# asharakeh/bayes-od-rc

Hardware: AMD Instinct MI355X
Metric: images/sec at N=10 MC samples, 512x512; per-anchor covariance latency (higher is better)
Workload: dtype bf16; 1 GPU; ResNet-50 RetinaNet + covar head, N=10 MC-dropout, 512x512, full BayesOD pipeline (forward+posterior+soft-NMS+cluster-fuse); global_batch=512, mc_samples=10, anchors=49104, parallelism=one GPU (no exchange; N > 1: image-sharded, one RCCL gather/step), visible_gpus=1, gpu_max_hw_queues=4

## Files before the change

### bayes-od-rc_amd/_lib.py

```python
import ctypes as C
import os

import numpy as np


_HERE = os.path.dirname(os.path.abspath(__file__))
LIB_PATH = os.path.join(_HERE, "lib", "libbayesod_hip.so")
if os.environ.get("BOD_LIB_OVERRIDE"):
    LIB_PATH = os.path.abspath(os.environ["BOD_LIB_OVERRIDE"])

BOD_OK, BOD_ERR_INVALID_ARG, BOD_ERR_HIP, BOD_ERR_OOM, BOD_ERR_NOT_READY, BOD_ERR_NO_DEVICE = range(6)
BOD_PARTS_COVARIANCE, BOD_PARTS_CLASS = 1, 2
BOD_VIEW_IDENTITY, BOD_VIEW_HFLIP = 0, 1


class BodConfig(C.Structure):
    _fields_ = [
        ("device", C.c_int32), ("image_h", C.c_int32), ("image_w", C.c_int32), ("batch", C.c_int32),
        ("mc_samples", C.c_int32), ("num_classes", C.c_int32), ("anchors_per_location", C.c_int32),
        ("min_level", C.c_int32), ("max_level", C.c_int32), ("dropout_rate", C.c_float),
        ("use_full_covar", C.c_int32), ("dirichlet_non_informative", C.c_int32),
        ("gaussian_isotropic", C.c_int32), ("isotropic_variance", C.c_float),
        ("ranking_method", C.c_int32), ("nms_max_output_size", C.c_int32),
        ("nms_iou_threshold", C.c_float), ("nms_soft_sigma", C.c_float), ("nms_variant", C.c_int32),
# ... 58 lines not shown
    "bod_get_raw": (C.c_int, [_H, _F, _F, _F]),
    "bod_set_raw": (C.c_int, [_H, _F, _F, _F]),
    "bod_get_pyramid": (C.c_int, [_H, C.c_int32, _F]),
    "bod_posterior": (C.c_int, [_H, C.c_uint64, C.c_uint32]),
    "bod_validation_post": (C.c_int, [_H]),
    "bod_get_num_kept": (C.c_int, [_H, _I]),
    "bod_get_posterior": (C.c_int, [_H, C.c_int32, _F, _F, _F, _F, _F, _I]),
    "bod_set_posterior": (C.c_int, [_H, C.c_int32, C.c_int32, _F, _F, _F, _F]),
    "bod_nms": (C.c_int, [_H]),
    "bod_get_nms": (C.c_int, [_H, C.c_int32, _I, _I]),
    "bod_set_nms": (C.c_int, [_H, C.c_int32, _I, C.c_int32]),
    "bod_get_iou_matrix": (C.c_int, [_H, C.c_int32, _F]),
    "bod_cluster_fuse": (C.c_int, [_H]),
    "bod_set_affinity": (C.c_int, [_H, C.c_int32, _F, C.c_int32, C.c_int32]),
    "bod_get_detections": (C.c_int, [_H, C.c_int32, _I, _F, _F, _F, _F]),
    "bod_get_detections_batch": (C.c_int, [_H, _I, _F, _F, _F, _F]),
    "bod_device_detections": (C.c_int, [_H, C.c_int32, C.POINTER(C.c_void_p)]),
    "bod_device_raw": (C.c_int, [_H, C.POINTER(C.c_void_p), C.c_int32]),
    "bod_infer": (C.c_int, [_H, C.c_void_p, C.c_int32, C.c_uint64, C.c_uint32]),
    "bod_infer_async": (C.c_int, [_H, C.c_void_p, C.c_int32, C.c_uint64, C.c_uint32, _I]),
    "bod_collect": (C.c_int, [_H, C.c_int32, _I, _F, _F, _F, _F]),
    "bod_upload_images": (C.c_int, [_H, _F]),
    "bod_upload_frames_u8": (C.c_int, [_H, C.POINTER(C.c_uint8), C.c_int32, C.c_int32, _F, C.c_int32]),
    "bod_upload_frames_u8_async": (C.c_int, [_H, C.POINTER(C.c_uint8), C.c_int32, C.c_int32, _F, C.c_int32, C.c_int32]),
    "bod_upload_frames_u8_ragged": (C.c_int, [_H, C.POINTER(C.c_uint8), _I, _F, C.c_int32]),
    "bod_upload_frames_u8_ragged_async": (C.c_int, [_H, C.POINTER(C.c_uint8), _I, _F, C.c_int32, C.c_int32]),
    "bod_upload_frames_u8_augmented": (C.c_int, [_H, C.POINTER(C.c_uint8), _I, _F, C.c_int32, C.POINTER(BodAugment)]),
    "bod_upload_frames_u8_augmented_async": (C.c_int, [_H, C.POINTER(C.c_uint8), _I, _F, C.c_int32, C.POINTER(BodAugment), C.c_int32]),
    "bod_augment_boxes": (C.c_int, [C.c_int32, _I, C.c_int32, C.c_int32, C.c_int32, C.POINTER(BodAugment), _I, _F, _F, C.c_int32,
                                    C.c_float, _I, _F, _F]),
    "bod_jpeg_info": (C.c_int, [C.c_char_p, C.c_int64, C.POINTER(BodJpegInfo)]),
    "bod_jpeg_entropy_decode": (C.c_int, [C.c_char_p, C.c_int64, C.POINTER(C.c_int16), C.c_int64, C.POINTER(C.c_uint16)]),
    "bod_jpeg_decode_rgb": (C.c_int, [C.c_int32, C.c_int32, C.POINTER(C.c_char_p), C.POINTER(C.c_int64), C.c_int32,
                                      C.POINTER(C.c_uint8), C.c_int64, _I]),
    "bod_upload_frames_jpeg": (C.c_int, [_H, C.POINTER(C.c_char_p), C.POINTER(C.c_int64), _F, C.c_int32, C.POINTER(BodAugment),
                                         C.c_int32, _I]),
    "bod_upload_frames_jpeg_async": (C.c_int, [_H, C.POINTER(C.c_char_p), C.POINTER(C.c_int64), _F, C.c_int32, C.POINTER(BodAugment),
                                               C.c_int32, _I, C.c_int32]),
    "bod_device_images_buffer": (C.c_void_p, [_H, C.c_int32]),
    "bod_device_images": (C.c_void_p, [_H]),
    "bod_synchronize": (C.c_int, [_H]),
    "bod_stage_conv_wgrad": (C.c_int, [C.c_int32, _F, C.c_int32, C.c_int32, C.c_int32, C.c_int32, _F, C.c_int32, C.c_int32,
                                       C.c_int32, C.c_int32, C.c_int32, C.c_int32, _F, _F]),
    "bod_stage_conv": (C.c_int, [C.c_int32, _F, C.c_int32, C.c_int32, C.c_int32, C.c_int32, _F, _F,
                                 C.c_int32, C.c_int32, C.c_int32, C.c_int32, C.c_int32, C.c_int32, _F,
                                 C.c_float, C.c_uint64, C.c_int32, C.c_uint32, C.c_int32, C.c_int32, _F]),
    "bod_loss_forward": (C.c_int, [C.c_int32, C.c_int32, C.c_int32, C.c_int32, _F, _F, _F, _F, _F, _F,
                                   C.POINTER(C.c_uint8), C.POINTER(C.c_uint8), C.c_int32, C.c_int32, C.c_float,
                                   C.POINTER(C.c_double)]),
    "bod_loss_forward_ex": (C.c_int, [C.c_int32, C.c_int32, C.c_int32, C.c_int32, _F, _F, _F, _F, _F, _F,
                                      C.POINTER(C.c_uint8), C.POINTER(C.c_uint8), C.c_int32, C.c_int32, C.c_float,
                                      C.POINTER(C.c_double), C.POINTER(BodLossOptions)]),
    "bod_set_loss_options": (C.c_int, [_H, C.POINTER(BodLossOptions)]),
    "bod_train_step": (C.c_int, [_H, C.c_void_p, C.c_int32, _F, _F, C.POINTER(C.c_uint8), C.POINTER(C.c_uint8), C.c_uint64, C.c_uint32,
                                 C.c_int32, C.c_float, C.c_float, C.c_float, C.c_float, C.c_float, C.c_int32, C.POINTER(C.c_double)]),
    "bod_train_step_boxes": (C.c_int, [_H, C.c_void_p, C.c_int32, _I, _F, _F, C.c_float, C.c_float, C.c_uint64, C.c_uint32,
                                       C.c_int32, C.c_float, C.c_float, C.c_float, C.c_float, C.c_float, C.c_int32, C.POINTER(C.c_double)]),
    "bod_train_get_targets": (C.c_int, [_H, _F, _F, C.POINTER(C.c_uint8), C.POINTER(C.c_uint8)]),
    "bod_train_gradients": (C.c_int, [_H, C.POINTER(C.c_void_p), C.POINTER(C.c_int64)]),
    "bod_train_apply": (C.c_int, [_H, C.c_float, C.POINTER(C.c_double)]),
    "bod_train_get": (C.c_int, [_H, C.c_char_p, C.c_int32, C.c_int32, _F, C.c_int64]),
    "bod_train_set": (C.c_int, [_H, C.c_char_p, C.c_int32, C.c_int32, _F, C.c_int64]),
    "bod_train_step_count": (C.c_int, [_H, C.POINTER(C.c_int64), C.c_int64]),
    "bod_loss_backward": (C.c_int, [C.c_int32, C.c_int32, C.c_int32, C.c_int32, _F, _F, _F, _F, _F, _F,
                                    C.POINTER(C.c_uint8), C.POINTER(C.c_uint8), C.c_int32, C.c_int32, C.c_float,
                                    C.c_float, C.c_float, C.POINTER(C.c_double), _F, _F, _F]),
    "bod_loss_backward_ex": (C.c_int, [C.c_int32, C.c_int32, C.c_int32, C.c_int32, _F, _F, _F, _F, _F, _F,
                                       C.POINTER(C.c_uint8), C.POINTER(C.c_uint8), C.c_int32, C.c_int32, C.c_float,
                                       C.c_float, C.c_float, C.POINTER(C.c_double), _F, _F, _F, C.POINTER(BodLossOptions)]),
    "bod_anchor_targets": (C.c_int, [C.c_int32, C.c_int32, _F, C.c_int32, _I, _F, _F, C.c_int32, C.c_float, C.c_float, _F, _F,
                                     C.POINTER(C.c_uint8), C.POINTER(C.c_uint8), _I, _F]),
    "bod_validation_losses_boxes": (C.c_int, [_H, _I, _F, _F, C.c_float, C.c_float, C.c_int32, C.c_int32, C.c_float, _D]),
    "bod_get_validation_detections_batch": (C.c_int, [_H, _I, _F, _F]),
    "bod_validate_boxes": (C.c_int, [_H, C.c_void_p, C.c_int32, _I, _F, _F, C.c_float, C.c_float, C.c_int32, C.c_int32, C.c_float, _D,
                                     _I, _F, _F]),
    "bod_pdq_corner_heatmaps": (C.c_int, [C.c_int32, C.c_int32, C.c_int32, C.c_int32, _D, _D, _I, _F]),
    "bod_pdq_frames": (C.c_int, [C.c_int32, C.c_int32, C.c_int32, C.c_int32, _I, _I, _I, _I, _D, _D, _D, _D, _F]),
    "bod_score_pairs": (C.c_int, [C.c_int32, C.c_int64, _D, _D, _D, C.c_int32, C.c_uint64, C.c_uint64, _D, _I]),
    "bod_bench_head_conv": (C.c_int, [_H, C.c_int32, C.c_int32, C.c_int32, C.POINTER(C.c_double), C.POINTER(C.c_double)]),
    "bod_profile_begin": (C.c_int, [_H]),
    "bod_profile_select": (C.c_int, [_H, C.c_int32]),
    "bod_plan_info": (C.c_int, [_H, C.POINTER(C.c_int32)]),
    "bod_plan_info_n": (C.c_int, [_H, C.POINTER(C.c_int32), C.c_int32]),
    "bod_stat_reset": (C.c_int, [_H]),
    "bod_stat_forward": (C.c_int, [_H, C.c_void_p, C.c_int32, C.c_uint64, C.c_uint32, C.c_int32]),
    "bod_stat_merge_from": (C.c_int, [_H, _H]),
    "bod_stat_merge": (C.c_int, [_H, C.POINTER(C.c_void_p), C.c_int32]),
    "bod_stat_device": (C.c_int, [_H, C.POINTER(C.c_void_p), _I]),
    "bod_stat_get": (C.c_int, [_H, _F, _F, _F, _I]),
    "bod_stat_set": (C.c_int, [_H, _F, _F, _F, C.c_int32]),
    "bod_stat_posterior": (C.c_int, [_H, C.c_uint64, C.c_uint32]),
    "bod_stat_forward_view": (C.c_int, [_H, C.c_void_p, C.c_int32, C.c_uint64, C.c_uint32, C.c_int32, C.c_int32]),
    "bod_stat_merge_view": (C.c_int, [_H, C.POINTER(C.c_void_p), C.c_int32, C.c_int32]),
    "bod_record_width": (C.c_int32, [_H]),
    "bod_get_posterior_parts": (C.c_int, [_H, C.c_int32, _F]),
    "bod_set_posterior_parts": (C.c_int, [_H, C.c_int32, C.c_int32, _F]),
    "bod_get_detection_parts": (C.c_int, [_H, C.c_int32, _F]),
    "bod_get_detection_parts_batch": (C.c_int, [_H, _F]),
    "bod_collect_parts": (C.c_int, [_H, C.c_int32, _F]),
    "bod_device_detection_parts": (C.c_int, [_H, C.c_int32, C.POINTER(C.c_void_p)]),
    "bod_get_posterior_class_parts": (C.c_int, [_H, C.c_int32, _F]),
    "bod_get_posterior_mean_probs": (C.c_int, [_H, C.c_int32, _F]),
    "bod_set_posterior_class_parts": (C.c_int, [_H, C.c_int32, C.c_int32, _F, _F]),
    "bod_get_detection_class_parts": (C.c_int, [_H, C.c_int32, _F]),
    "bod_get_detection_class_parts_batch": (C.c_int, [_H, _F]),
    "bod_collect_class_parts": (C.c_int, [_H, C.c_int32, _F]),
    "bod_device_detection_class_parts": (C.c_int, [_H, C.c_int32, C.POINTER(C.c_void_p)]),
    "bod_stat_get_entropy": (C.c_int, [_H, _F]),
    "bod_stat_set_entropy": (C.c_int, [_H, _F]),
    "bod_stat_device_entropy": (C.c_int, [_H, C.POINTER(C.c_void_p)]),
    "bod_stat_merge_entropy": (C.c_int, [_H, C.c_void_p, C.c_int32]),
    "bod_gather_detections": (C.c_int, [_H, C.c_int32, C.c_void_p, C.c_int32, C.c_int32, C.c_int32, C.c_void_p, C.POINTER(C.c_void_p)]),
    "bod_profile_end": (C.c_int, [_H, C.POINTER(C.c_double), C.POINTER(C.c_int64),
                                  C.POINTER(C.c_double), C.POINTER(C.c_double), C.POINTER(C.c_int64)]),
}

_lib = None


def load():
    global _lib
    if _lib is not None:
        return _lib
    if not os.path.exists(LIB_PATH):
        raise RuntimeError(
            "libbayesod_hip.so not found at %s -- build it with `python -c 'import __graft_entry__ as g; "
            "g.build()'` (there is no CPU fallback)" % LIB_PATH)
    lib = C.CDLL(LIB_PATH)
    for name, (res, args) in SIGNATURES.items():
        fn = getattr(lib, name)
        fn.restype = res
        fn.argtypes = args
    _lib = lib
    return lib


def fptr(a):
    return None if a is None else a.ctypes.data_as(_F)


def dptr(a):
    return None if a is None else a.ctypes.data_as(_D)


def iptr(a):
    return None if a is None else a.ctypes.data_as(_I)


def check(lib, handle, status):
    if status == BOD_OK:
        return
    msg = lib.bod_last_error(handle)
    msg = msg.decode() if msg else "status %d" % status
    if status in (BOD_ERR_INVALID_ARG, BOD_ERR_NOT_READY):
        raise ValueError(msg)
    if status == BOD_ERR_OOM:
        raise MemoryError(msg)
    raise RuntimeError(msg)


def as_f32(a):
    return np.ascontiguousarray(a, dtype=np.float32)
```

### bayes-od-rc_amd/csrc/engine.hip

```cpp
#include "../../include/bayesod.h"
#include "kernels.h"
#include "jpeg_entropy.h"

#include <algorithm>
#include <array>
#include <atomic>
#include <cmath>
#include <condition_variable>
#include <deque>
#include <functional>
#include <mutex>
#include <thread>
#include <tuple>
#include <type_traits>
#include <cstdarg>
#include <cstdio>
#include <cstring>
#include <map>
#include <memory>
#include <string>
#include <system_error>
#include <vector>
#include <dlfcn.h>

// ... 186 lines not shown
            }
}

}

struct JpegSlot {
    char* pinned = nullptr; size_t pinned_cap = 0;
    char* dev = nullptr; size_t dev_cap = 0;
    uint8_t* planes = nullptr; size_t planes_cap = 0;
    hipEvent_t copied = nullptr;
    int32_t n = 0;
    size_t stage_bytes = 0, coef_base = 0, plane_bytes = 0;
    int64_t rgb_bytes = 0;
    int32_t idct_wgs_per_frame = 0, color_wgs_per_frame = 0;
    void release() {
        if (pinned) hipHostFree(pinned);
        if (dev) hipFree(dev);
        if (planes) hipFree(planes);
        if (copied) hipEventDestroy(copied);
        *this = JpegSlot();
    }
};

struct bod_context {
    bod_config cfg{};
    std::string err;
    hipStream_t stream = nullptr;
    std::vector<void*> allocs;
    std::map<const void*, size_t> alloc_bytes;
    int64_t device_bytes = 0;
    struct TrainState* train = nullptr;
    struct ValState* val = nullptr;
    int32_t energy_samples = BOD_ENERGY_DEFAULT_SAMPLES;
    uint64_t loss_seed = 0; uint32_t loss_first_image_id = 0; int32_t loss_id_stride = 1;
    int32_t* energy_list = nullptr; float* energy_term = nullptr;

    int sh = 0, sw = 0, ph = 0, pw = 0;
    int ch[6] = {0}, cw[6] = {0};
    int nlev = 0; int lh[8] = {0}, lw[8] = {0};
    int64_t lvl_off[8] = {0};
    int64_t lvl_p0[8] = {0};
    int64_t Ppad = 0; int P = 0, A = 0;

    std::map<std::string, HostTensor> host_w;
    std::map<std::string, PackedConv> packed;
    float* stem_w = nullptr; float* stem_b = nullptr;
    bool weights_ready = false, anchors_ready = false, forward_done = false, posterior_done = false,
         nms_done = false, cluster_done = false;

    float* d_images = nullptr;
    float* splitk_partial = nullptr; size_t splitk_elems = 0;
    uint8_t* d_frames_u8 = nullptr; size_t frames_u8_cap = 0;
    float* d_images_b[2] = {nullptr, nullptr}; uint8_t* d_u8_b[2] = {nullptr, nullptr}; size_t u8_cap_b[2] = {0, 0};
    hipStream_t copy = nullptr;
    hipEvent_t ev_img_ready[2] = {nullptr, nullptr}, ev_img_free[2] = {nullptr, nullptr};
    bool img_ready_pending[2] = {false, false}, img_free_pending[2] = {false, false};
    int cur_img_buf = -1;
    struct RaggedTable { std::vector<char> host; char* dev = nullptr; };
    RaggedTable rag_sync, rag_b[2];
    RaggedTable aug_sync, aug_b[2];
    JpegSlot jpeg_slot[3];
    hipEvent_t ev_tab[2] = {nullptr, nullptr};
    const float* kscale_src[2] = {nullptr, nullptr};
    float* kscale_cur[2] = {nullptr, nullptr}; int kscale_i = 0;
    const float* kscale_now = nullptr;
    char* stem_out = nullptr;
    int es = 2;
    bool split = false;
    char* pyr_hx = nullptr;
    int pyr_fmt = 1;
    int plan_mx = 0;
    int mx = 0;
    Plane pyramid;
    char* head_act[3][2] = {{nullptr}};
    char* head_act_t[3][4] = {{nullptr}};
    float* raw[3] = {nullptr};
    float* agg[3] = {nullptr};
    bool agg_plan = false;
    bool plan_fused_out = false, plan_xreuse = false, plan_xreuse0 = false;
    bool raw_valid = false, agg_valid = false;
    bool plan_sparse = false;
    bool plan_halo = false;
    SparseTailArgs sparse{};
    int plan_tail_rows = 0;
    bool agg_sparse = false;
    float* stat_acc[3] = {nullptr};
    int stat_k = 0;
    hipEvent_t ev_stat = nullptr;
    float* d_mirror = nullptr;
    int mirror_sym = -1, mirror_bad_level = 0;
    bool keep_ready = false;
    uint64_t keep_seed = 0; uint32_t keep_first = 0;
    uint64_t last_seed = 0; uint32_t last_first_image = 0;
    int32_t last_sample_base = 0;
    std::map<std::string, RowEnt*> tables;
    struct XrTable { RowEnt* rows = nullptr; int2* ext = nullptr; int m = 0; };
    std::map<std::string, XrTable> xr_tables;
    std::vector<Op> ops;
    const float* cur_images = nullptr;

    float* d_anchors = nullptr;
    PostBuffers pb{};
    float* nms_scores = nullptr; int32_t* nms_begin = nullptr;
    int32_t* nms_sel_s[2] = {nullptr, nullptr}; int32_t* nms_nsel_s[2] = {nullptr, nullptr};
    float* out_scores_s[2] = {nullptr, nullptr}; float* out_means_s[2] = {nullptr, nullptr};
    float* out_covs_s[2] = {nullptr, nullptr}; float* out_counts_s[2] = {nullptr, nullptr};
    int32_t* nms_sel = nullptr; int32_t* nms_nsel = nullptr;
    float* out_scores = nullptr; float* out_means = nullptr; float* out_covs = nullptr; float* out_counts = nullptr;
    int slot = 0;
    float* parts = nullptr;
    float* out_parts_s[2] = {nullptr, nullptr}; float* out_parts = nullptr;
    std::vector<char> parts_ok, det_parts_ok[2];
    bool parts_staged[2] = {false, false};
    bool class_parts = false;
    float* ent = nullptr; float* stat_ent = nullptr; int stat_ent_k = 0;
    float* cparts = nullptr;
    float* out_cparts_s[2] = {nullptr, nullptr}; float* out_cparts = nullptr;
    std::vector<char> cparts_ok, det_cparts_ok[2];
    bool cparts_staged[2] = {false, false};
    hipStream_t side = nullptr;
    int overlap_mode = 0;
    int ov_front_slots = 0, ov_slots = 0;
    hipStream_t full = nullptr, front = nullptr, back = nullptr;
    hipEvent_t ev_front_done[2] = {nullptr, nullptr}, ev_l0_done[2] = {nullptr, nullptr}, ev_join = nullptr;
    bool l0_pending[2] = {false, false};
    bool ov_dirty = false;
    char* pyr_d[2] = {nullptr, nullptr};
    int fwd_parity = 0, pyr_last = 0;
    int first_head_op = 0;
    bool in_overlap_call = false;
    int n_cu = 256;
    hipEvent_t ev_posterior = nullptr; hipEvent_t ev_done[2] = {nullptr, nullptr};
    int dev_op_lo = 0, dev_op_hi = 1 << 30;
    hipStream_t done_stream[2] = {nullptr, nullptr};
    bool side_pending[2] = {false, false};
    char* host_stage[2] = {nullptr, nullptr};
    float* rec_send = nullptr; float* rec_recv = nullptr; size_t rec_recv_elems = 0;
    hipEvent_t ev_gather = nullptr; hipStream_t gather_stream = nullptr;
    void select_slot(int sidx) {
        slot = sidx;
        nms_sel = nms_sel_s[sidx]; nms_nsel = nms_nsel_s[sidx];
        out_scores = out_scores_s[sidx]; out_means = out_means_s[sidx];
        out_covs = out_covs_s[sidx]; out_counts = out_counts_s[sidx];
        out_parts = out_parts_s[sidx]; out_cparts = out_cparts_s[sidx];
    }
    float* iou_scratch = nullptr; int64_t iou_cap = 0;
    float* affinity = nullptr; int affinity_img = -1;

    bool profiling = false; int prof_which = 0;
    std::vector<std::pair<hipEvent_t, hipEvent_t>> ev_head, ev_post;
    double prof_flops = 0;

    bod_status fail(bod_status s, const char* fmt, ...) {
        char buf[1024];
        va_list ap; va_start(ap, fmt); vsnprintf(buf, sizeof buf, fmt, ap); va_end(ap);
        err = buf;
        return s;
    }
    template <typename T> bod_status dalloc(T** p, size_t n_elems, bool zero = true) {
        void* q = nullptr;
        const size_t bytes = std::max<size_t>(n_elems * sizeof(T), 256);
        hipError_t e = hipMalloc(&q, bytes);
        if (e != hipSuccess) return fail(BOD_ERR_OOM, "hipMalloc(%zu) failed: %s", bytes, hipGetErrorString(e));
        if (zero) {
            e = hipMemsetAsync(q, 0, bytes, stream);
            if (e != hipSuccess) return fail(BOD_ERR_HIP, "hipMemset: %s", hipGetErrorString(e));
        }
        allocs.push_back(q);
        alloc_bytes[q] = bytes;
        device_bytes += (int64_t)bytes;
        *p = reinterpret_cast<T*>(q);
        return BOD_OK;
    }
};

#define HIPCHK(h, expr)                                                                         \
    do {                                                                                        \
        hipError_t _e = (expr);                                                                 \
        if (_e != hipSuccess)                                                                   \
            return (h)->fail(BOD_ERR_HIP, "%s failed: %s (%s:%d)", #expr, hipGetErrorString(_e), \
                             __FILE__, __LINE__);                                               \
    } while (0)
#define BODCHK(expr) do { bod_status _s = (expr); if (_s != BOD_OK) return _s; } while (0)

namespace {

const char* kHeadPrefix[3] = {"pyramid_classification", "pyramid_regression", "pyramid_cov"};
const int kHeadConvs[3] = {4, 3, 4};

// ... 546 lines not shown
    if (xreuse0) BODCHK(make_xr_tiles(t1, &d1x, &dext1, &m1x));

    const bool mc = train_mode || std::max(N, c.mc_ensemble_size) > 1;
    const uint32_t thr = (uint32_t)std::floor((double)c.dropout_rate * 65536.0);
    const float dscale = (float)(1.0 / (1.0 - (double)c.dropout_rate));
    const int nheads = c.has_covar_head ? 3 : 2;
    bool fuse_out = (h->es == 2 || (h->split && xreuse)) && !train_mode;
    if (const char* e = getenv("BOD_FUSE_HEAD_OUTPUT")) fuse_out = fuse_out && atoi(e) != 0;
    {
        ConvArgs probe{};
        probe.M = B * N * h->P; probe.cout_pad = 256; probe.fan_count = 1; probe.flags = CONV_RELU;
        fuse_out = fuse_out && (mx_plan || conv_igemm_uses_full_cout_tile(probe));
    }
    bool agg = xreuse && fuse_out && N >= 2 && 256 / N >= 1 && 320 / N - 2 >= 1 && (c.mc_ensemble_size <= N || c.mc_statistics);
    if (const char* e = getenv("BOD_FUSE_AGGREGATION")) agg = agg && atoi(e) != 0;
    RowEnt* d2a = nullptr; int2* dexta = nullptr; int m2a = 0;
    if (agg) {
        std::vector<RowEnt> tiled;
        std::vector<ExtRow> ext;
        const int rc = xr_tile_rows_aggregated(t2, B, N, h->P, tiled, ext);
        if (rc == 1) return h->fail(BOD_ERR_INVALID_ARG, "aggregated tiling: no pixel fits a tile (N = %d)", N);
        if (rc == 2) return h->fail(BOD_ERR_INVALID_ARG, "aggregated tiling: extended rows out of order");
        m2a = (int)tiled.size();
        BODCHK(h->dalloc(&d2a, tiled.size(), false));
        BODCHK(h->dalloc(&dexta, ext.size(), false));
        HIPCHK(h, hipMemcpyAsync(d2a, tiled.data(), tiled.size() * sizeof(RowEnt), hipMemcpyHostToDevice, h->stream));
        HIPCHK(h, hipMemcpyAsync(dexta, ext.data(), ext.size() * sizeof(int2), hipMemcpyHostToDevice, h->stream));
        HIPCHK(h, hipStreamSynchronize(h->stream));
        const size_t BA = (size_t)B * h->A;
        BODCHK(h->dalloc(&h->agg[0], BA * c.num_classes));
        BODCHK(h->dalloc(&h->agg[1], BA * 16));
        if (c.has_covar_head) BODCHK(h->dalloc(&h->agg[2], BA * 10));
        if (h->class_parts) BODCHK(h->dalloc(&h->ent, BA));
    } else {
        BODCHK(ensure_raw(h));
    }
    if (c.mc_statistics) {
        const size_t BA = (size_t)B * h->A;
        const size_t per[3] = {(size_t)c.num_classes, 16, 10};
        for (int k = 0; k < (c.has_covar_head ? 3 : 2); ++k)
            if (!h->agg[k]) BODCHK(h->dalloc(&h->agg[k], BA * per[k]));
        if (h->class_parts && !h->ent) BODCHK(h->dalloc(&h->ent, BA));
        BODCHK(ensure_stat(h));
    }
    bool sparse = agg && h->es == 2 && !h->split && !mx_plan && !c.pipeline_overlap && !c.mc_statistics &&
                  h->A == h->P * c.anchors_per_location && h->P <= 65536;
    if (const char* e = getenv("BOD_SPARSE_TAIL")) sparse = sparse && atoi(e) != 0;
    bool halo = sparse && !train_mode;
    if (const char* e = getenv("BOD_SPARSE_HALO")) halo = halo && atoi(e) != 0;
    if (sparse) {
        SparseTailArgs& sa = h->sparse;
        const int tables = halo ? 2 : 1;
        sa.B = B; sa.N = N; sa.P = h->P; sa.apl = c.anchors_per_location; sa.Ppad = h->Ppad;
        sa.cap_tiles = B * (h->P / st_min_pixels(N) + 1);
        sa.tail_rows = 192;
        if (const char* e = getenv("BOD_SPARSE_TAIL_ROWS")) { if (atoi(e) == 256) sa.tail_rows = 256; }
        {
            ConvArgs probe{};
            probe.M = sa.cap_tiles * sa.tail_rows; probe.cout_pad = 256; probe.fan_count = 1; probe.flags = CONV_RELU;
            if (!conv_igemm_uses_full_cout_tile(probe)) sa.tail_rows = 256;
        }
        if (st_min_pixels(N, sa.tail_rows) != st_min_pixels(N))
            return h->fail(BOD_ERR_INVALID_ARG, "sparse tail: %d-row tiles change the tile bound at N = %d", sa.tail_rows, N);
        sa.lv.n = 5;
        {
            const PyramidGeometry pg = pyramid_geometry(h->lh, h->lw);
            for (int l = 0; l < 5; ++l) { sa.lv.lw[l] = pg.lw[l]; sa.lv.lh[l] = pg.lh[l]; sa.lv.p0[l] = (int32_t)pg.lvl_p0[l]; }
        }
        RowEnt* pix = nullptr;
        BODCHK(h->dalloc(&pix, (size_t)h->P, false));
        HIPCHK(h, hipMemcpyAsync(pix, t2.data(), (size_t)h->P * sizeof(RowEnt), hipMemcpyHostToDevice, h->stream));
        HIPCHK(h, hipStreamSynchronize(h->stream));
        sa.pix = pix;
        BODCHK(h->dalloc(&sa.rows, (size_t)sa.cap_tiles * sa.tail_rows, false));
        BODCHK(h->dalloc(&sa.ext, (size_t)sa.cap_tiles * XR_EXT_ROWS, false));
        if (halo) {
            BODCHK(h->dalloc(&sa.halo_rows, (size_t)sa.cap_tiles * 256, false));
            BODCHK(h->dalloc(&sa.halo_ext, (size_t)sa.cap_tiles * XR_EXT_ROWS, false));
        }
        BODCHK(h->dalloc(&sa.tile_count, 2));
        BODCHK(h->dalloc(&sa.runs, (size_t)tables * B * h->P, false));
        BODCHK(h->dalloc(&sa.chunks, (size_t)tables * B * h->P, false));
        BODCHK(h->dalloc(&sa.tiles, (size_t)tables * B * h->P, false));
    }
    h->plan_sparse = sparse;
    h->plan_halo = halo;
    h->plan_tail_rows = sparse ? h->sparse.tail_rows : 0;
    Op sparse_op; sparse_op.kind = Op::CONV; sparse_op.is_head3x3 = true; sparse_op.flavour = FLAVOUR_AGG;
    int sparse_groups = 0; PackedConv sparse_pc{};
    Op halo_op = sparse_op;
    int halo_groups = 0; PackedConv halo_pc{};
    h->agg_plan = agg; h->plan_fused_out = fuse_out; h->plan_xreuse = xreuse; h->plan_xreuse0 = xreuse0; h->plan_mx = mx_plan ? mxf : 0;
    int hfmt[3] = {mxf, mxf, mxf};
    if (mxf == 2) { const char* e = getenv("BOD_MX4_BOX_HX"); if (e && atoi(e) != 0) hfmt[1] = 1; }
    if (mxf == 1) { static const bool cls_h4 = [] { const char* e = getenv("BOD_MX_CLS_H4"); return !e || atoi(e) != 0; }(); if (cls_h4) hfmt[0] = 2; }
    const bool mixed = mx_plan && hfmt[0] != hfmt[1];
    const int pyr_fmt = mixed ? 1 : mxf;
    h->pyr_fmt = pyr_fmt;
    for (int layer = 0; layer < 4; ++layer)
    for (int fpass = 0; fpass < 2; ++fpass)
    for (int part = 0; part < 2; ++part)
    for (int flav = (agg && layer >= 2) ? FLAVOUR_RAW : FLAVOUR_BOTH; flav <= ((agg && layer >= 2) ? FLAVOUR_AGG : FLAVOUR_BOTH); ++flav) {
        const bool split_launch = agg && layer >= 2;
        if (fpass == 1 && (!mixed || layer == 0)) continue;
        const int lfmt = !mx_plan ? 0 : layer == 0 ? pyr_fmt : mixed ? (fpass == 0 ? 2 : 1) : mxf;
        if (!split_launch && part == 1) continue;
        if (split_launch && part == 0 && flav == FLAVOUR_AGG) continue;
        const bool both = split_launch && part == 0;
        Op op; op.kind = Op::CONV; op.is_head3x3 = true; op.flavour = both ? FLAVOUR_BOTH : flav;
        int g = 0; PackedConv pc0{};
        double fused_flops = 0;
        const bool both_flav = op.flavour == FLAVOUR_BOTH;
        ConvGroup raw_cg{}; PackedConv raw_pc{}; std::string raw_wname; bool has_raw = false;
        ConvGroup full_cg[3]{}; std::string full_wname[3]; PackedConv full_pc{}; int nfull = 0;
        for (int hd = 0; hd < nheads; ++hd) {
            if (layer >= kHeadConvs[hd]) continue;
            if (split_launch && (part == 1) != (layer == kHeadConvs[hd] - 1)) continue;
            if (mixed && layer > 0 && hfmt[hd] != lfmt) continue;
            PackedConv pc;
            BODCHK(pack_conv(h, std::string(kHeadPrefix[hd]) + "_" + std::to_string(layer), "", 128, &pc, (mx_plan && (layer > 0 || mx_l0)) ? lfmt : 0));
            if (pc.cin != 256 || pc.cout != 256 || pc.taps != 9)
                return h->fail(BOD_ERR_INVALID_ARG, "head conv %s_%d must be 3x3 256->256", kHeadPrefix[hd], layer);
            op.wname[g] = std::string(kHeadPrefix[hd]) + "_" + std::to_string(layer);
            ConvGroup cg{};
            cg.in = layer == 0 ? (mx_l0 ? h->pyr_hx : h->pyramid.d) : (train_mode ? h->head_act_t[hd][layer - 1] : h->head_act[hd][(layer + 1) & 1]);
            cg.w = pc.w; cg.bias = pc.bias;
            cg.out = train_mode ? h->head_act_t[hd][layer] : h->head_act[hd][layer & 1];
            cg.layer_id = hd * 4 + layer;
            cg.out_hx = (mx_plan && layer < kHeadConvs[hd] - 1) ? hfmt[hd] : 0;
            if (fuse_out && layer == kHeadConvs[hd] - 1) {
                PackedConv po;
                BODCHK(pack_conv(h, kHeadPrefix[hd], "", 32, &po));
                if (po.cin != 256 || po.cout != out_ch[hd] || po.taps != 1)
                    return h->fail(BOD_ERR_INVALID_ARG, "head output conv %s must be 1x1 256->%d (got %d->%d)", kHeadPrefix[hd], out_ch[hd], po.cin, po.cout);
                cg.w2 = po.w; cg.bias2 = po.bias; cg.out2 = h->raw[hd]; cg.cout2 = po.cout; cg.out2_cstride = out_ch[hd];
                op.head[g] = hd;
                if (flav == FLAVOUR_AGG) {
                    cg.out2 = nullptr;
                    cg.agg_kind = hd == 0 ? AGG_CLS : hd == 1 ? AGG_BOX : AGG_COV;
                    cg.agg_n = N; cg.agg_P = h->P; cg.agg_C = c.num_classes; cg.agg_out = h->agg[hd]; cg.anchors = h->d_anchors;
                    if (hd == 0 && h->class_parts) { cg.agg_kind = AGG_CLS_ENT; cg.out2 = h->ent; }
                }
                fused_flops += 2.0 * ((double)B * N * h->P) * 256.0 * out_ch[hd];
            }
            if (halo && both_flav && ((layer == 1 && hd == 1) || (layer == 2 && hd == 2))) {
                halo_op.conv.g[halo_groups] = cg;
                halo_op.wname[halo_groups] = op.wname[g];
                if (halo_groups++ == 0) halo_pc = pc;
                halo_op.flops += 2.0 * ((double)B * N * h->P) * 256.0 * 2304.0;
                raw_cg = cg; raw_pc = pc; raw_wname = op.wname[g]; has_raw = true;
                if (nfull == 0) full_pc = pc;
                full_cg[nfull] = cg; full_wname[nfull++] = op.wname[g];
                op.wname[g].clear();
                continue;
            }
            if (sparse && flav == FLAVOUR_AGG && hd != 0) {
                sparse_op.conv.g[sparse_groups] = cg;
                sparse_op.wname[sparse_groups] = op.wname[g];
                sparse_op.head[sparse_groups] = hd;
                if (sparse_groups++ == 0) sparse_pc = pc;
                sparse_op.flops += 2.0 * ((double)B * N * h->P) * 256.0 * 2304.0 + 2.0 * ((double)B * N * h->P) * 256.0 * out_ch[hd];
                fused_flops -= 2.0 * ((double)B * N * h->P) * 256.0 * out_ch[hd];
                op.head[g] = -1; op.wname[g].clear();
                continue;
            }
            op.conv.g[g] = cg;
// ... 60 lines not shown
        ConvArgs a = base_args(sparse_pc, sa.rows, sa.cap_tiles * sa.tail_rows, 256, 256);
        a.tile_rows = sa.tail_rows;
        for (int q = 0; q < sparse_groups; ++q) a.g[q] = sparse_op.conv.g[q];
        a.groups = sparse_groups;
        a.flags = CONV_RELU | (mc ? CONV_DROPOUT : 0);
        a.fan_count = 1; a.fan_stride = (int32_t)h->Ppad;
        a.drop_threshold = thr; a.drop_scale = dscale;
        a.ext = sa.ext; a.xreuse = 2; a.tile_count = sa.tile_count;
        sparse_op.conv = a;
        sparse_op.name = "head_tower_layer_3(sparse)";
        h->ops.push_back(sparse_op);
    }
    for (int hd = 0; hd < nheads && !fuse_out; ++hd) {
        PackedConv pc;
        BODCHK(pack_conv(h, kHeadPrefix[hd], "", 64, &pc));
        if (pc.cin != 256 || pc.cout != out_ch[hd] || pc.taps != 1)
            return h->fail(BOD_ERR_INVALID_ARG, "head output conv %s must be 1x1 256->%d (got %d->%d)", kHeadPrefix[hd], out_ch[hd], pc.cin, pc.cout);
        Op op; op.kind = Op::CONV;
        ConvArgs a = base_args(pc, d3, B * N * h->P, 256, out_ch[hd]);
        a.g[0] = ConvGroup{train_mode ? h->head_act_t[hd][kHeadConvs[hd] - 1] : h->head_act[hd][(kHeadConvs[hd] - 1) & 1], pc.w, pc.bias, h->raw[hd], nullptr, nullptr, 0, 0, nullptr, nullptr, nullptr, 0, 0};
        a.flags = CONV_OUT_F32;
        op.conv = a;
        op.flops = 2.0 * a.M * pc.cout * 256.0;
        op.name = kHeadPrefix[hd]; op.wname[0] = kHeadPrefix[hd];
        h->ops.push_back(op);
    }
    if (h->splitk_elems) {
        BODCHK(h->dalloc(&h->splitk_partial, h->splitk_elems));
        for (Op& o : h->ops) if (o.kind == Op::CONV && o.conv.ksplit > 1) o.conv.partial = h->splitk_partial;
    }
    if (h->split) for (Op& o : h->ops) if (o.kind == Op::CONV) to_split_args(&o.conv);
    h->first_head_op = (int)h->ops.size();
    for (size_t i = 0; i < h->ops.size(); ++i) if (h->ops[i].is_head3x3) { h->first_head_op = (int)i; break; }
    h->pyr_d[0] = h->pyramid.d;
    if (const char* e = getenv("BOD_DUMP_OPS")) if (atoi(e) != 0) {
        fprintf(stderr, "# ops: index name kind flavour M taps cin cout groups fan has_res fused_next flops bytes\n");
        for (size_t i = 0; i < h->ops.size(); ++i) {
            const Op& o = h->ops[i];
            const ConvArgs& a = o.conv;
            double bytes = 0;
            if (o.kind == Op::STEM)
                bytes = (double)B * c.image_h * c.image_w * 3 * 4 + (double)B * h->ph * h->pw * 64 * h->es;
            if (o.kind == Op::CONV) {
                const double es = (a.flags & CONV_OUT_F32) ? 4.0 : (double)h->es;
                for (int g = 0; g < a.groups; ++g) {
                    bytes += (double)a.M * a.cin * h->es;
                    bytes += (double)a.M * std::max(1, a.fan_count) * a.cout_valid * es;
                    if (a.g[g].res) bytes += (double)a.M * a.cout_valid * h->es;
                    if (a.g[g].ch_w3) bytes += (double)a.M * (a.cin == 128 ? 128 : 64) * h->es;
                    bytes += (double)a.taps * a.cin * a.cout_pad * h->es;
                }
            }
            fprintf(stderr, "# op %zu %s %d %d %d %d %d %d %d %d %d %d %.6g %.6g\n", i, o.name.c_str(), (int)o.kind, o.flavour, a.M, a.taps, a.cin,
                    a.cout_valid, a.groups, a.fan_count, o.kind == Op::CONV && a.g[0].res ? 1 : 0, o.kind == Op::CONV && a.g[0].ch_w3 ? 1 : 0, o.flops, bytes);
        }
    }
    if (h->overlap_mode) BODCHK(h->dalloc(&h->pyr_d[1], (size_t)B * h->Ppad * 256 * h->es));
    return BOD_OK;
}

bod_status alloc_post(bod_context* h) {
    const bod_config& c = h->cfg;
    const size_t BA = (size_t)c.batch * h->A;
    const int nblocks = (h->A + 255) / 256;
    PostBuffers& p = h->pb;
    BODCHK(h->dalloc(&p.keep, BA));
    BODCHK(h->dalloc(&p.d_counts, BA * c.num_classes));
    BODCHK(h->dalloc(&p.block_counts, (size_t)c.batch * nblocks));
    BODCHK(h->dalloc(&p.num_kept, (size_t)c.batch));
    BODCHK(h->dalloc(&p.counts, BA * c.num_classes));
    BODCHK(h->dalloc(&p.score, BA * c.num_classes));
    BODCHK(h->dalloc(&p.means, BA * 4));
    BODCHK(h->dalloc(&p.covs, BA * 16));
    BODCHK(h->dalloc(&p.ranking, BA));
    BODCHK(h->dalloc(&p.corners, BA * 4));
    BODCHK(h->dalloc(&p.anchor_index, BA));
    BODCHK(h->dalloc(&h->d_anchors, (size_t)h->A * 4));
    const size_t BApad = (size_t)h->cfg.batch * ((h->A + 511) & ~(size_t)511);
    BODCHK(h->dalloc(&h->nms_scores, BApad));
    BODCHK(h->dalloc(&h->nms_begin, BApad));
    const size_t BK = (size_t)c.batch * c.nms_max_output_size;
    for (int sidx = 0; sidx < 2; ++sidx) {
        BODCHK(h->dalloc(&h->nms_sel_s[sidx], BK));
        BODCHK(h->dalloc(&h->nms_nsel_s[sidx], (size_t)c.batch));
        BODCHK(h->dalloc(&h->out_scores_s[sidx], BK * c.num_classes));
        BODCHK(h->dalloc(&h->out_means_s[sidx], BK * 4));
        BODCHK(h->dalloc(&h->out_covs_s[sidx], BK * 16));
        BODCHK(h->dalloc(&h->out_counts_s[sidx], BK * c.num_classes));
        if (c.covariance_parts & BOD_PARTS_COVARIANCE) BODCHK(h->dalloc(&h->out_parts_s[sidx], BK * 48));
        if (h->class_parts) BODCHK(h->dalloc(&h->out_cparts_s[sidx], BK * 4));
        const size_t stage_bytes = ((size_t)c.batch + BK * (2 * (size_t)c.num_classes + 20 + ((c.covariance_parts & BOD_PARTS_COVARIANCE) ? 48 : 0) +
                                                            (h->class_parts ? 4 : 0))) * 4;
        if (hipHostMalloc(reinterpret_cast<void**>(&h->host_stage[sidx]), stage_bytes, hipHostMallocDefault) != hipSuccess)
            return h->fail(BOD_ERR_OOM, "pinned host staging buffer (%zu bytes)", stage_bytes);
    }
    if (c.covariance_parts & BOD_PARTS_COVARIANCE) {
        BODCHK(h->dalloc(&h->parts, BA * BOD_PARTS_TRI));
        h->parts_ok.assign((size_t)c.batch, 0);
        for (int sidx = 0; sidx < 2; ++sidx) h->det_parts_ok[sidx].assign((size_t)c.batch, 0);
    }
    if (h->class_parts) {
        BODCHK(h->dalloc(&h->cparts, BA * (3 + (size_t)c.num_classes)));
        h->cparts_ok.assign((size_t)c.batch, 0);
        for (int sidx = 0; sidx < 2; ++sidx) h->det_cparts_ok[sidx].assign((size_t)c.batch, 0);
    }
    h->select_slot(0);
    BODCHK(h->dalloc(&h->d_images, (size_t)c.batch * c.image_h * c.image_w * 3));
    h->d_images_b[0] = h->d_images;
    return BOD_OK;
}

PostCfg post_cfg(bod_context* h, uint64_t seed, uint32_t first_image) {
    const bod_config& c = h->cfg;
    PostCfg p{};
    p.B = c.batch; p.N = c.mc_samples; p.A = h->A; p.C = c.num_classes; p.draws = c.num_categorical_draws;
    p.use_full_covar = c.use_full_covar; p.has_covar = c.has_covar_head; p.dirichlet = c.dirichlet_non_informative;
    p.gaussian_iso = c.gaussian_isotropic; p.ranking_method = c.ranking_method; p.iso_var = c.isotropic_variance;
    p.kitti_sh = c.kitti_scale_h; p.kitti_sw = c.kitti_scale_w;
    p.kitti_frame = c.kitti_scale_h > 0.f ? h->kscale_now : nullptr;
    p.seed_lo = (uint32_t)seed; p.seed_hi = (uint32_t)(seed >> 32); p.image_base = first_image;
    return p;
}

struct Markers {
    bool on = false;
    int (*push)(const char*) = nullptr;
    int (*pop)() = nullptr;
    Markers() {
        const char* e = getenv("BOD_ROCTX");
        if (!e || !atoi(e)) return;
        void* lib = dlopen("librocprofiler-sdk-roctx.so", RTLD_NOW | RTLD_GLOBAL);
        if (!lib) lib = dlopen("libroctx64.so", RTLD_NOW | RTLD_GLOBAL);
        if (!lib) { fprintf(stderr, "bayesod: BOD_ROCTX=1 but no roctx library could be opened (%s)\n", dlerror()); return; }
        push = reinterpret_cast<int (*)(const char*)>(dlsym(lib, "roctxRangePushA"));
        pop = reinterpret_cast<int (*)()>(dlsym(lib, "roctxRangePop"));
        on = push && pop;
    }
};
static Markers& markers() { static Markers m; return m; }
struct MarkerRange {
    bool on;
    explicit MarkerRange(const char* name) : on(markers().on) { if (on) markers().push(name); }
    ~MarkerRange() { if (on) markers().pop(); }
    MarkerRange(const MarkerRange&) = delete;
    MarkerRange& operator=(const MarkerRange&) = delete;
};
static std::string op_stage(const std::string& name) {
    if (name.rfind("conv1", 0) == 0 || name.rfind("pool1", 0) == 0) return "bod:stem";
    if (name.rfind("res", 0) == 0 && name.size() > 3) return "bod:" + name.substr(0, 4);
    if (name.rfind("head_tower_layer_", 0) == 0) return "bod:" + name.substr(0, name.find('(') == std::string::npos ? name.size() : name.find('('));
    if (name.rfind("pyramid_", 0) == 0) return "bod:head_outputs";
    return "bod:fpn";
}

bod_status mark_images_consumed(bod_context* h, hipStream_t st = nullptr) {
    if (h->cur_img_buf >= 0 && h->copy) {
        HIPCHK(h, hipEventRecord(h->ev_img_free[h->cur_img_buf], st ? st : h->stream));
        h->img_free_pending[h->cur_img_buf] = true;
    }
    return BOD_OK;
}

bod_status join_overlap(bod_context* h) {
    if (!h->ov_dirty) return BOD_OK;
    HIPCHK(h, hipStreamSynchronize(h->front));
    HIPCHK(h, hipStreamSynchronize(h->back));
    h->ov_dirty = false;
    return BOD_OK;
}

bod_status run_forward(bod_context* h, const float* dev_images, uint64_t seed, uint32_t first_image, int flavour = FLAVOUR_RAW,
                       bool only_flavoured = false, bool overlapped = false) {
    const bod_config& c = h->cfg;
    if (flavour == FLAVOUR_RAW && !only_flavoured) BODCHK(ensure_raw(h));
    const bool ov = overlapped && h->overlap_mode != 0 && !only_flavoured;
    hipStream_t fs = ov ? h->front : h->stream;
    int par = 0;
    if (ov) {
        par = h->fwd_parity; h->fwd_parity ^= 1;
        if (h->l0_pending[par]) { HIPCHK(h, hipStreamWaitEvent(fs, h->ev_l0_done[par], 0)); h->l0_pending[par] = false; }
    }
    if (!only_flavoured) { h->pyr_last = par; h->keep_ready = false; }
    const int cus_front = h->n_cu;
    const int cus_back = h->n_cu;
    static const int trace_call = getenv("BOD_TRACE_OPS") ? atoi(getenv("BOD_TRACE_OPS")) : 0;
    static int call_no = 0;
    const bool trace = trace_call > 0 && ++call_no == trace_call && !ov;
    std::vector<hipEvent_t> tev;
    if (trace) {
        tev.resize(h->ops.size() + 1);
        for (hipEvent_t& e : tev) HIPCHK(h, hipEventCreate(&e));
        HIPCHK(h, hipEventRecord(tev[0], h->stream));
    }
    size_t op_i = 0;
    bool stem_pool_fused = false;
    std::string cur_stage;
    struct StageCloser { std::string& s; ~StageCloser() { if (!s.empty()) markers().pop(); } } stage_closer{cur_stage};
    for (Op& op : h->ops) {
        if (trace && op_i > 0) HIPCHK(h, hipEventRecord(tev[op_i], h->stream));
        const bool is_front = (int)op_i < h->first_head_op;
        const bool first_back = (int)op_i == h->first_head_op;
        hipStream_t st = is_front ? fs : h->stream;
        ++op_i;
        if ((op.flavour != FLAVOUR_BOTH && op.flavour != flavour) || (only_flavoured && op.flavour == FLAVOUR_BOTH)) continue;
        if (op.raw_use == (only_flavoured ? Op::RAW_FORWARD : Op::RAW_RERUN)) continue;
        if ((int)op_i - 1 < h->dev_op_lo || (int)op_i - 1 >= h->dev_op_hi) continue;
        if (ov && first_back) {
            HIPCHK(h, hipEventRecord(h->ev_front_done[par], fs));
            HIPCHK(h, hipStreamWaitEvent(h->stream, h->ev_front_done[par], 0));
        }
        if (markers().on) {
            std::string st = op_stage(op.name);
            if (st != cur_stage) {
                if (!cur_stage.empty()) markers().pop();
                markers().push(st.c_str());
                cur_stage.swap(st);
            }
        }
        switch (op.kind) {
            case Op::STEM: {
                const Op* pool = op_i < h->ops.size() && h->ops[op_i].kind == Op::POOL ? &h->ops[op_i] : nullptr;
                static const bool split_fused = [] { const char* e = getenv("BOD_STEM_SPLIT_FUSED"); return !e || atoi(e) != 0; }();
                stem_pool_fused = pool && !h->train && (h->split ? split_fused : h->es == 2) && !trace &&
                                  stem_pool_fused_applies(dev_images, c.batch, c.image_w, h->sw, is_front ? cus_front : cus_back);
                if (stem_pool_fused)
                    HIPCHK(h, launch_stem_pool_fused(dev_images, h->stem_w, h->stem_b, pool->conv.g[0].out, h->split ? 1 : 0, c.batch, c.image_h,
                                                     c.image_w, h->sh, h->sw, h->ph, h->pw, h->pw + 2, (h->ph + 2) * (h->pw + 2), st));
                else
                HIPCHK(h, launch_stem_conv(dev_images, h->stem_w, h->stem_b, h->stem_out, h->es == 4, c.batch, c.image_h,
                                           c.image_w, h->sh, h->sw, st));
                if (!h->train) BODCHK(mark_images_consumed(h, st));
                break;
            }
            case Op::KEEP: {
                for (int sidx = 0; sidx < 2; ++sidx)
                    if (h->side_pending[sidx]) HIPCHK(h, hipStreamWaitEvent(st, h->ev_done[sidx], 0));
                PostCfg pc = post_cfg(h, seed, first_image);
                pc.aggregated = 1;
                PostBuffers pb = h->pb;
                pb.agg_cls = h->agg[0];
                HIPCHK(h, launch_posterior_keep(pc, pb, st));
                SparseTailArgs sa = h->sparse;
                sa.keep = h->pb.keep;
                HIPCHK(h, launch_sparse_tail_rows(sa, st));
                static const bool sparse_stats = [] { const char* e = getenv("BOD_SPARSE_STATS"); return e && atoi(e) != 0; }();
                if (sparse_stats) {
                    HIPCHK(h, hipStreamSynchronize(st));
                    int32_t cnt[2] = {0, 0};
                    HIPCHK(h, hipMemcpy(cnt, sa.tile_count, sizeof cnt, hipMemcpyDeviceToHost));
                    const int R = sa.tail_rows;
                    long valid = 0, full = 0;
                    if (cnt[0] > 0 && cnt[0] <= sa.cap_tiles) {
                        std::vector<int32_t> off((size_t)cnt[0] * R);
                        HIPCHK(h, hipMemcpy2D(off.data(), sizeof(int32_t), &sa.rows[0].out_off, sizeof(RowEnt), sizeof(int32_t), off.size(), hipMemcpyDeviceToHost));
                        for (int t = 0; t < cnt[0]; ++t) {
                            int v = 0;
                            for (int r = 0; r < R; ++r) v += off[(size_t)t * R + r] >= 0 ? 1 : 0;
                            valid += v;
                            full += v == R ? 1 : 0;
                        }
                    }
                    const long dense = ((long)sa.B * sa.N * sa.P + 255) / 256;
                    std::fprintf(stderr, "BOD_SPARSE_STATS: tail %d tiles of %d rows, %.1f valid rows per tile (%ld rows = %.3f of the dense launch's), %ld tiles with all %d rows valid; "
                                 "halo %d tiles of 256 rows; dense plain tiles %ld; capacity %d tiles\n", (int)cnt[0], R,
                                 cnt[0] > 0 ? (double)valid / cnt[0] : 0.0, valid, (double)valid / ((double)sa.B * sa.N * sa.P), full, R, (int)cnt[1], dense, (int)sa.cap_tiles);
                }
                h->keep_ready = true; h->keep_seed = seed; h->keep_first = first_image;
                break;
            }
            case Op::POOL:
                if (stem_pool_fused) break;
                HIPCHK(h, launch_stem_pool(h->stem_out, op.conv.g[0].out, h->split ? 2 : (h->es == 4 ? 1 : 0), c.batch,
                                           h->sh, h->sw, h->ph, h->pw, h->pw + 2, (h->ph + 2) * (h->pw + 2), st));
                break;
            case Op::CONV: {
                if (op.hx_pyramid) HIPCHK(h, launch_pairs_to_hx(h->pyramid.d, h->pyr_hx, (long)c.batch * h->Ppad, 256, st, h->pyr_fmt));
                op.conv.seed_lo = (uint32_t)seed; op.conv.seed_hi = (uint32_t)(seed >> 32);
                op.conv.image_base = first_image;
                op.conv.sample_base = (uint32_t)c.mc_sample_base;
                op.conv.dyn_rng = train_dyn_rng(h);
                const bool is_tower = op.conv.xreuse != 0 && op.conv.fan_count <= 1;
                const bool timed = h->profiling && op.is_head3x3 && (h->prof_which == 0 || (h->prof_which == 1) == is_tower);
                hipEvent_t e0 = nullptr, e1 = nullptr;
                if (timed) {
                    HIPCHK(h, hipEventCreate(&e0)); HIPCHK(h, hipEventCreate(&e1));
                    HIPCHK(h, hipEventRecord(e0, st));
                }
                op.conv.n_cu = is_front ? cus_front : cus_back;
                if (par != 0) {
                    ConvArgs a = op.conv;
                    for (int g = 0; g < a.groups; ++g) {
                        if (a.g[g].in == h->pyr_d[0]) a.g[g].in = h->pyr_d[1];
                        if (a.g[g].out == h->pyr_d[0]) a.g[g].out = h->pyr_d[1];
                    }
                    HIPCHK(h, (h->es == 4 && !h->split) ? launch_conv_igemm_f32(a, st) : launch_conv_igemm(a, st));
                } else
                HIPCHK(h, (h->es == 4 && !h->split) ? launch_conv_igemm_f32(op.conv, st) : launch_conv_igemm(op.conv, st));
                if (timed) {
                    HIPCHK(h, hipEventRecord(e1, st));
                    h->ev_head.emplace_back(e0, e1);
                    h->prof_flops += op.flops;
                }
                if (ov && first_back) {
                    HIPCHK(h, hipEventRecord(h->ev_l0_done[par], h->stream));
                    h->l0_pending[par] = true;
                }
                break;
            }
        }
    }
    if (trace) {
        HIPCHK(h, hipEventRecord(tev[h->ops.size()], h->stream));
        HIPCHK(h, hipStreamSynchronize(h->stream));
        fprintf(stderr, "# op trace: name kind M taps cin cout_pad groups fan ms TFLOP/s\n");
        for (size_t i = 0; i < h->ops.size(); ++i) {
            float ms = 0.f;
            HIPCHK(h, hipEventElapsedTime(&ms, tev[i], tev[i + 1]));
            const Op& o = h->ops[i];
            fprintf(stderr, "%-28s %d %8d %2d %5d %5d %d %2d %9.4f %8.1f\n", o.name.c_str(), (int)o.kind, o.conv.M, o.conv.taps,
                    o.conv.cin, o.conv.cout_pad, o.conv.groups, o.conv.fan_count, ms, o.flops / (ms * 1e-3) / 1e12);
        }
        for (hipEvent_t& e : tev) hipEventDestroy(e);
    }
    h->forward_done = true; h->posterior_done = h->nms_done = h->cluster_done = false; h->affinity_img = -1;
    h->last_seed = seed; h->last_first_image = first_image;
    if (!only_flavoured) h->last_sample_base = c.mc_sample_base;
    if (flavour == FLAVOUR_AGG) { h->agg_valid = true; h->raw_valid = false; h->agg_sparse = h->plan_sparse; }
// ... 1375 lines not shown
        if (!h->det_cparts_ok[h->slot][img]) return h->fail(BOD_ERR_NOT_READY, "bod_get_detection_class_parts_batch: image %d was fused without its posterior's class parts (bod_set_posterior_class_parts)", img);
    const size_t B = (size_t)h->cfg.batch, K = (size_t)h->cfg.nms_max_output_size;
    std::vector<int32_t> num(B);
    HIPCHK(h, hipMemcpyAsync(num.data(), h->nms_nsel, B * 4, hipMemcpyDeviceToHost, h->stream));
    BODCHK(d2h(h, rows, h->out_cparts, B * K * 4));
    HIPCHK(h, hipStreamSynchronize(h->stream));
    for (size_t b = 0; rows && b < B; ++b)
        for (size_t k = (size_t)std::max(num[b], 0); k < K; ++k)
            for (int q = 0; q < 4; ++q) rows[(b * K + k) * 4 + q] = 0.f;
    return BOD_OK;
}

bod_status bod_device_detection_class_parts(bod_handle h, int32_t sidx, void** p) {
    BODCHK(class_parts_handle(h, "bod_device_detection_class_parts"));
    if (!p || sidx < 0 || sidx > 1) return h->fail(BOD_ERR_INVALID_ARG, "bod_device_detection_class_parts: slot %d / NULL", sidx);
    *p = h->out_cparts_s[sidx];
    return BOD_OK;
}

bod_status bod_device_raw(bod_handle h, void** p, int32_t mark_ready) {
    if (!h || !p) return BOD_ERR_INVALID_ARG;
    BODCHK(join_overlap(h));
    HIPCHK(h, hipSetDevice(h->cfg.device));
    if (mark_ready) BODCHK(ensure_raw(h)); else BODCHK(materialise_raw(h));
    p[0] = h->raw[0]; p[1] = h->raw[1]; p[2] = h->cfg.has_covar_head ? h->raw[2] : nullptr;
    if (mark_ready) { h->kscale_now = nullptr; h->forward_done = true; h->posterior_done = h->nms_done = h->cluster_done = false; h->affinity_img = -1; h->raw_valid = true; h->agg_valid = false; }
    return BOD_OK;
}

bod_status bod_device_detections(bod_handle h, int32_t sidx, void** p) {
    if (!h || !p || sidx < 0 || sidx > 1) return BOD_ERR_INVALID_ARG;
    p[0] = h->nms_nsel_s[sidx]; p[1] = h->out_scores_s[sidx]; p[2] = h->out_means_s[sidx];
    p[3] = h->out_covs_s[sidx]; p[4] = h->out_counts_s[sidx];
    return BOD_OK;
}

bod_status bod_infer(bod_handle h, const float* images, int32_t on_device, uint64_t seed, uint32_t first_image_id) {
    MarkerRange mr_api("bod:infer");
    if (!h) return BOD_ERR_INVALID_ARG;
    BODCHK(join_overlap(h));
    if (!h->weights_ready) return h->fail(BOD_ERR_NOT_READY, "weights not finalized");
    if (h->cfg.mc_samples < 2) return h->fail(BOD_ERR_INVALID_ARG, "bayes_od needs mc_samples >= 2 (sample covariance divides by N-1)");
    HIPCHK(h, hipSetDevice(h->cfg.device));
    const float* dev = nullptr;
    BODCHK(stage_images(h, images, on_device, &dev));
    h->cur_images = dev;
    BODCHK(run_forward(h, dev, seed, first_image_id, infer_flavour(h)));
    BODCHK(run_posterior(h, seed, first_image_id));
    BODCHK(run_nms(h, h->stream));
    return run_cluster(h, h->stream);
}

bod_status bod_infer_async(bod_handle h, const float* images, int32_t on_device, uint64_t seed, uint32_t first_image_id, int32_t* slot_out) {
    MarkerRange mr_api("bod:infer_async");
    if (!h || !slot_out) return BOD_ERR_INVALID_ARG;
    if (!h->weights_ready) return h->fail(BOD_ERR_NOT_READY, "weights not finalized");
    if (h->cfg.mc_samples < 2) return h->fail(BOD_ERR_INVALID_ARG, "bayes_od needs mc_samples >= 2 (sample covariance divides by N-1)");
    HIPCHK(h, hipSetDevice(h->cfg.device));
    const int sidx = h->slot ^ 1;
    if (h->side_pending[sidx])
        return h->fail(BOD_ERR_NOT_READY, "slot %d still holds uncollected detections: call bod_collect first", sidx);
    const bool ov = h->overlap_mode != 0;
    struct MainStream { bod_context* h; ~MainStream() { h->stream = h->full; h->in_overlap_call = false; } } restore_main{h};
    if (ov) {
        HIPCHK(h, hipEventRecord(h->ev_join, h->full));
        HIPCHK(h, hipStreamWaitEvent(h->front, h->ev_join, 0));
        HIPCHK(h, hipStreamWaitEvent(h->back, h->ev_join, 0));
        h->stream = h->back; h->in_overlap_call = true; h->ov_dirty = true;
    }
    const float* dev = nullptr;
    BODCHK(stage_images(h, images, on_device, &dev, ov ? h->front : h->stream));
    h->cur_images = dev;
    BODCHK(run_forward(h, dev, seed, first_image_id, infer_flavour(h), false, ov));
    BODCHK(run_posterior(h, seed, first_image_id));
    HIPCHK(h, hipEventRecord(h->ev_posterior, h->stream));
    h->select_slot(sidx);
    static const bool side_on = [] { const char* e = getenv("BOD_SIDE_STREAM"); return e && atoi(e) != 0; }();
    hipStream_t sd = side_on ? h->side : h->stream;
    if (side_on) HIPCHK(h, hipStreamWaitEvent(h->side, h->ev_posterior, 0));
    BODCHK(run_nms(h, sd));
    BODCHK(run_cluster(h, sd));
    {
        const size_t B = (size_t)h->cfg.batch, BK = B * h->cfg.nms_max_output_size, C = h->cfg.num_classes;
        char* hs = h->host_stage[sidx];
        HIPCHK(h, hipMemcpyAsync(hs, h->nms_nsel_s[sidx], B * 4, hipMemcpyDeviceToHost, sd)); hs += B * 4;
        HIPCHK(h, hipMemcpyAsync(hs, h->out_scores_s[sidx], BK * C * 4, hipMemcpyDeviceToHost, sd)); hs += BK * C * 4;
        HIPCHK(h, hipMemcpyAsync(hs, h->out_means_s[sidx], BK * 16, hipMemcpyDeviceToHost, sd)); hs += BK * 16;
        HIPCHK(h, hipMemcpyAsync(hs, h->out_covs_s[sidx], BK * 64, hipMemcpyDeviceToHost, sd)); hs += BK * 64;
        HIPCHK(h, hipMemcpyAsync(hs, h->out_counts_s[sidx], BK * C * 4, hipMemcpyDeviceToHost, sd)); hs += BK * C * 4;
        if (h->parts) { HIPCHK(h, hipMemcpyAsync(hs, h->out_parts_s[sidx], BK * 48 * 4, hipMemcpyDeviceToHost, sd)); h->parts_staged[sidx] = true; hs += BK * 48 * 4; }
        if (h->cparts) { HIPCHK(h, hipMemcpyAsync(hs, h->out_cparts_s[sidx], BK * 4 * 4, hipMemcpyDeviceToHost, sd)); h->cparts_staged[sidx] = true; }
    }
    HIPCHK(h, hipEventRecord(h->ev_done[sidx], sd));
    h->done_stream[sidx] = sd;
    h->side_pending[sidx] = true;
    *slot_out = sidx;
    return BOD_OK;
}

bod_status bod_collect(bod_handle h, int32_t sidx, int32_t* num, float* scores, float* means, float* covs, float* counts) {
    MarkerRange mr_api("bod:collect");
    if (!h) return BOD_ERR_INVALID_ARG;
    if (sidx < 0 || sidx > 1 || !h->side_pending[sidx]) return h->fail(BOD_ERR_NOT_READY, "slot %d has no pending batch", sidx);
    const size_t B = (size_t)h->cfg.batch, BK = B * h->cfg.nms_max_output_size, C = h->cfg.num_classes;
    HIPCHK(h, hipEventSynchronize(h->ev_done[sidx]));
    const char* hs = h->host_stage[sidx];
    if (num) std::memcpy(num, hs, B * 4);
    hs += B * 4;
    if (scores) std::memcpy(scores, hs, BK * C * 4);
    hs += BK * C * 4;
    if (means) std::memcpy(means, hs, BK * 16);
    hs += BK * 16;
    if (covs) std::memcpy(covs, hs, BK * 64);
    hs += BK * 64;
    if (counts) std::memcpy(counts, hs, BK * C * 4);
    h->side_pending[sidx] = false;
    return BOD_OK;
}

bod_status bod_collect_parts(bod_handle h, int32_t sidx, float* parts) {
    BODCHK(parts_handle(h, "bod_collect_parts"));
    if (sidx < 0 || sidx > 1 || !h->parts_staged[sidx]) return h->fail(BOD_ERR_NOT_READY, "bod_collect_parts: slot %d holds no batch of bod_infer_async", sidx);
    const size_t B = (size_t)h->cfg.batch, BK = B * h->cfg.nms_max_output_size, C = h->cfg.num_classes;
    HIPCHK(h, hipEventSynchronize(h->ev_done[sidx]));
    if (parts) std::memcpy(parts, h->host_stage[sidx] + (B + BK * (2 * C + 20)) * 4, BK * 48 * 4);
    return BOD_OK;
}

bod_status bod_collect_class_parts(bod_handle h, int32_t sidx, float* rows) {
    BODCHK(class_parts_handle(h, "bod_collect_class_parts"));
    if (sidx < 0 || sidx > 1 || !h->cparts_staged[sidx]) return h->fail(BOD_ERR_NOT_READY, "bod_collect_class_parts: slot %d holds no batch of bod_infer_async", sidx);
    const size_t B = (size_t)h->cfg.batch, K = (size_t)h->cfg.nms_max_output_size, BK = B * K, C = h->cfg.num_classes;
    HIPCHK(h, hipEventSynchronize(h->ev_done[sidx]));
    if (!rows) return BOD_OK;
    std::memcpy(rows, h->host_stage[sidx] + (B + BK * (2 * C + 20 + (h->parts ? 48 : 0))) * 4, BK * 4 * 4);
    const int32_t* num = reinterpret_cast<const int32_t*>(h->host_stage[sidx]);
    for (size_t b = 0; b < B; ++b)
        for (size_t k = (size_t)std::max(num[b], 0); k < K; ++k)
            for (int q = 0; q < 4; ++q) rows[(b * K + k) * 4 + q] = 0.f;
    return BOD_OK;
}

bod_status bod_stage_conv(int32_t device, const float* x, int32_t B, int32_t H, int32_t W, int32_t Cin,
                          const float* w, const float* bias, int32_t KH, int32_t KW, int32_t Cout,
                          int32_t stride, int32_t same_padding, int32_t relu, const float* residual,
                          float dropout_rate, uint64_t seed, int32_t layer_id, uint32_t image_id,
                          int32_t round_output_bf16, int32_t precision, float* out) {
    bod_context ctx;
    bod_context* h = &ctx;
    const int mxfmt = precision == BOD_PRECISION_F16MX ? 1 : precision == BOD_PRECISION_F16MX4 ? 2 : 0;
    const bool mxp = mxfmt != 0;
    const int mx_mode = mxp ? round_output_bf16 : 0;
    const bool f32 = precision == BOD_PRECISION_FP32, x3 = precision == BOD_PRECISION_BF16X3 || mxp;
    if (mxp) round_output_bf16 = 1;
    h->es = (f32 || x3) ? 4 : 2;
    h->split = x3; h->mx = mxfmt;
    auto done = [&](bod_status s) {
        if (s != BOD_OK) g_create_error = h->err;
        if (h->stream) hipStreamSynchronize(h->stream);
        for (void* p : h->allocs) hipFree(p);
        if (h->stream) hipStreamDestroy(h->stream);
        h->allocs.clear(); h->stream = nullptr;
        return s;
    };
    if (!x || !w || !out || B < 1 || H < 1 || W < 1 || KH < 1 || KW < 1 || stride < 1 || stride > 2)
        return done(h->fail(BOD_ERR_INVALID_ARG, "bod_stage_conv: bad argument"));
    if (precision != BOD_PRECISION_BF16 && !f32 && !x3) return done(h->fail(BOD_ERR_INVALID_ARG, "bod_stage_conv: bad precision"));
    if (mxp && (KH != 3 || KW != 3 || stride != 1 || !same_padding || Cin != 256 || Cout != 256 || residual || mx_mode < 0 || mx_mode > 2))
        return done(h->fail(BOD_ERR_INVALID_ARG, "bod_stage_conv: BOD_PRECISION_F16MX / F16MX4 run a head-tower layer (3x3, stride 1, SAME, 256 -> 256, no residual), round_output_bf16 in 0..2"));
    if (f32 && round_output_bf16) return done(h->fail(BOD_ERR_INVALID_ARG, "bod_stage_conv: round_output_bf16 is meaningless in fp32 precision"));
    if (Cin % 64 != 0 || ((round_output_bf16 || (dropout_rate > 0.f && !f32)) && Cout % 4 != 0))
        return done(h->fail(BOD_ERR_INVALID_ARG, "bod_stage_conv: Cin must be a multiple of 64 (and Cout of 4 for bf16 output); got %d, %d", Cin, Cout));
    if (KH > 3 || KW > 3) return done(h->fail(BOD_ERR_INVALID_ARG, "bod_stage_conv: kernel larger than 3x3 needs a wider zero border"));
    int ndev = 0;
    if (hipGetDeviceCount(&ndev) != hipSuccess || device < 0 || device >= ndev)
        return done(h->fail(BOD_ERR_NO_DEVICE, "no HIP device %d: libbayesod_hip has no CPU fallback", device));
    if (hipSetDevice(device) != hipSuccess || hipStreamCreateWithFlags(&h->stream, hipStreamNonBlocking) != hipSuccess)
        return done(h->fail(BOD_ERR_HIP, "cannot set up device %d", device));
    h->cfg.batch = B;
    int OH, OW, oy = 1, ox = 1;
    if (same_padding) {
        OH = (H + stride - 1) / stride; OW = (W + stride - 1) / stride;
        oy = 1 - same_pad_before(H, KH, stride); ox = 1 - same_pad_before(W, KW, stride);
    } else {
        OH = (H - KH) / stride + 1; OW = (W - KW) / stride + 1;
    }
    if (OH < 1 || OW < 1) return done(h->fail(BOD_ERR_INVALID_ARG, "bod_stage_conv: empty output"));
    auto run = [&]() -> bod_status {
        Plane in, res;
        BODCHK(new_plane(h, &in, B, H, W, Cin));
        auto put_split = [](std::vector<uint16_t>& dst, size_t pix_slot0, int c, float v) {
            const uint16_t hi = f2bf(v);
            const size_t slot = pix_slot0 + (size_t)(c >> 5) * 64 + (c & 31);
            dst[slot] = hi; dst[slot + 32] = f2bf(v - bf2f(hi));
        };
        std::vector<uint16_t> hx(f32 ? 0 : (size_t)B * in.bstride * Cin * (x3 ? 2 : 1), 0);
        std::vector<float> hx32(f32 ? (size_t)B * in.bstride * Cin : 0, 0.f);
        const bool hx_in = mxp && mx_mode != 2;
        for (int b = 0; b < B && hx_in; ++b)
            for (int y = 0; y < H; ++y)
                for (int xx = 0; xx < W; ++xx) {
                    const size_t pix = (size_t)b * in.bstride + (size_t)(y + 1) * in.pitch + (xx + 1);
                    (mxfmt == 2 ? pack_h4_row : pack_hx_row)(x + (((size_t)b * H + y) * W + xx) * Cin, Cin, reinterpret_cast<uint8_t*>(hx.data()) + pix * Cin * 4, false);
                }
        for (int b = 0; b < B && !hx_in; ++b)
            for (int y = 0; y < H; ++y)
                for (int xx = 0; xx < W; ++xx)
                    for (int c = 0; c < Cin; ++c) {
                        const size_t pix = (size_t)b * in.bstride + (size_t)(y + 1) * in.pitch + (xx + 1);
                        const size_t di = pix * Cin + c;
                        const float v = x[(((size_t)b * H + y) * W + xx) * Cin + c];
                        if (f32) hx32[di] = v; else if (x3) put_split(hx, pix * 2 * Cin, c, v); else hx[di] = f2bf(v);
                    }
        HIPCHK(h, hipMemcpyAsync(in.d, f32 ? (const void*)hx32.data() : (const void*)hx.data(),
                                 (size_t)B * in.bstride * Cin * h->es, hipMemcpyHostToDevice, h->stream));
        HIPCHK(h, hipStreamSynchronize(h->stream));
        if (residual) {
            BODCHK(new_plane(h, &res, B, OH, OW, Cout));
// ... 578 lines not shown
    static const bool side_on = [] { const char* e = getenv("BOD_SIDE_STREAM"); return e && atoi(e) != 0; }();
    hipStream_t st = (slot >= 0 && slot <= 1 && !side_on && h->done_stream[slot]) ? h->done_stream[slot] : h->side;
    if (slot < 0) {
        if (!h->cluster_done) return h->fail(BOD_ERR_NOT_READY, "bod_gather_detections: bod_cluster_fuse has not run");
        BODCHK(join_overlap(h));
        sidx = h->slot;
        st = h->stream;
    } else if (slot > 1 || !h->side_pending[slot]) {
        return h->fail(BOD_ERR_NOT_READY, "bod_gather_detections: slot %d has no pending batch", slot);
    }
    for (int img = 0; h->parts && img < B; ++img)
        if (!h->det_parts_ok[sidx][img]) return h->fail(BOD_ERR_NOT_READY, "bod_gather_detections: image %d was fused without its posterior's parts (bod_set_posterior_parts)", img);
    for (int img = 0; h->cparts && img < B; ++img)
        if (!h->det_cparts_ok[sidx][img]) return h->fail(BOD_ERR_NOT_READY, "bod_gather_detections: image %d was fused without its posterior's class parts (bod_set_posterior_class_parts)", img);
    if (!h->rec_send && hipMalloc(reinterpret_cast<void**>(&h->rec_send), block * 4) != hipSuccess)
        return h->fail(BOD_ERR_OOM, "bod_gather_detections: %zu bytes", block * 4);
    if (h->ev_gather && h->gather_stream && h->gather_stream != st) HIPCHK(h, hipStreamWaitEvent(st, h->ev_gather, 0));
    if (slot >= 0) HIPCHK(h, hipStreamWaitEvent(st, h->ev_done[slot], 0));
    if (h->cparts)
        HIPCHK(h, launch_pack_records_class(h->nms_nsel_s[sidx], h->out_scores_s[sidx], h->out_means_s[sidx], h->out_covs_s[sidx],
                                            h->out_counts_s[sidx], h->out_parts_s[sidx], h->out_cparts_s[sidx], h->rec_send, B, K, C, st));
    else if (h->parts)
        HIPCHK(h, launch_pack_records_parts(h->nms_nsel_s[sidx], h->out_scores_s[sidx], h->out_means_s[sidx], h->out_covs_s[sidx],
                                            h->out_counts_s[sidx], h->out_parts_s[sidx], h->rec_send, B, K, C, st));
    else
        HIPCHK(h, launch_pack_records(h->nms_nsel_s[sidx], h->out_scores_s[sidx], h->out_means_s[sidx], h->out_covs_s[sidx],
                                      h->out_counts_s[sidx], h->rec_send, B, K, C, st));
    float* recv = nullptr;
    if (rank == root) {
        if (world == 1 && !nccl_comm) recv = h->rec_send;
        else {
            if (h->rec_recv_elems < block * world) {
                if (h->rec_recv && h->rec_recv != h->rec_send) hipFree(h->rec_recv);
                h->rec_recv = nullptr; h->rec_recv_elems = 0;
                if (hipMalloc(reinterpret_cast<void**>(&h->rec_recv), block * world * 4) != hipSuccess)
                    return h->fail(BOD_ERR_OOM, "bod_gather_detections: %zu bytes", block * world * 4);
                h->rec_recv_elems = block * world;
            }
            recv = h->rec_recv;
        }
    }
    if (nccl_comm) {
        if (!rccl().load()) return h->fail(BOD_ERR_NOT_READY, "bod_gather_detections: librccl.so (ncclGather) could not be opened");
        const int rc = rccl().gather(h->rec_send, recv, block,  7, root, nccl_comm, st);
        if (rc != 0) return h->fail(BOD_ERR_HIP, "ncclGather: %s", rccl().errstr ? rccl().errstr(rc) : "error");
    }
    if (!h->ev_gather) HIPCHK(h, hipEventCreateWithFlags(&h->ev_gather, hipEventDisableTiming));
    if (rank == root && gathered_host) {
        HIPCHK(h, hipMemcpyAsync(gathered_host, recv, block * world * 4, hipMemcpyDeviceToHost, st));
        HIPCHK(h, hipEventRecord(h->ev_gather, st)); h->gather_stream = st;
        HIPCHK(h, hipEventSynchronize(h->ev_gather));
    } else {
        HIPCHK(h, hipEventRecord(h->ev_gather, st)); h->gather_stream = st;
    }
    if (!(rank == root && gathered_host) && slot >= 0) {
        HIPCHK(h, hipEventRecord(h->ev_done[slot], st));
    }
    if (gathered_device) *gathered_device = recv;
    return BOD_OK;
}

bod_status bod_plan_info(bod_handle h, int32_t* info8) {
    if (!h || !info8) return BOD_ERR_INVALID_ARG;
    if (!h->weights_ready) return h->fail(BOD_ERR_NOT_READY, "bod_plan_info: the plan is built by bod_finalize_weights");
    for (int i = 0; i < 8; ++i) info8[i] = 0;
    info8[0] = h->agg_plan; info8[1] = h->plan_fused_out; info8[2] = h->plan_xreuse; info8[3] = h->plan_xreuse0;
    info8[4] = (int32_t)h->ops.size();
    for (const Op& o : h->ops) if (o.kind == Op::CONV && !o.is_head3x3 && o.conv.xreuse) ++info8[5];
    info8[6] = h->plan_mx;
    info8[7] = h->plan_sparse;
    return BOD_OK;
}

bod_status bod_plan_info_n(bod_handle h, int32_t* info, int32_t n) {
    if (!h || !info || n < 0) return BOD_ERR_INVALID_ARG;
    int32_t all[10];
    BODCHK(bod_plan_info(h, all));
    all[8] = h->plan_halo;
    all[9] = h->plan_tail_rows;
    for (int i = 0; i < n && i < 10; ++i) info[i] = all[i];
    return BOD_OK;
}

static bod_status stat_handle(bod_handle h, const char* who) {
    if (!h->cfg.mc_statistics) return h->fail(BOD_ERR_INVALID_ARG, "%s: the handle was not created with mc_statistics = 1", who);
    BODCHK(join_overlap(h));
    HIPCHK(h, hipSetDevice(h->cfg.device));
    return ensure_stat(h);
}

static bod_status stat_view_ready(bod_handle h, const char* who, int32_t view) {
    if (view != BOD_VIEW_IDENTITY && view != BOD_VIEW_HFLIP)
        return h->fail(BOD_ERR_INVALID_ARG, "%s: view must be BOD_VIEW_IDENTITY (0) or BOD_VIEW_HFLIP (1), got %d", who, view);
    if (view == BOD_VIEW_IDENTITY) return BOD_OK;
    if (!h->anchors_ready) return h->fail(BOD_ERR_NOT_READY, "%s: bod_set_anchors has not been called (a mirrored view maps every anchor to its partner)", who);
    const bod_config& c = h->cfg;
    const int K = c.anchors_per_location;
    if (h->mirror_sym < 0) {
        std::vector<float> an((size_t)h->A * 4);
        HIPCHK(h, hipMemcpyAsync(an.data(), h->d_anchors, an.size() * 4, hipMemcpyDeviceToHost, h->stream));
        HIPCHK(h, hipStreamSynchronize(h->stream));
        const float fw = (float)c.image_w;
        int bad = -1;
        for (int l = 0; l < h->nlev && bad < 0; ++l) {
            const size_t off = (size_t)h->lvl_p0[l] * K;
            const int W = h->lw[l];
            for (int y = 0; y < h->lh[l] && bad < 0; ++y)
                for (int x = 0; x < W && bad < 0; ++x)
                    for (int k = 0; k < K; ++k) {
                        const float* s = &an[(off + ((size_t)y * W + x) * K + k) * 4];
                        const float* p = &an[(off + ((size_t)y * W + (W - 1 - x)) * K + k) * 4];
                        const float want[4] = {s[0], fw - s[1], s[2], s[3]};
                        if (memcmp(p, want, 16) != 0) { bad = l; break; }
                    }
        }
        h->mirror_sym = bad < 0; h->mirror_bad_level = bad < 0 ? 0 : c.min_level + bad;
    }
    if (!h->mirror_sym)
        return h->fail(BOD_ERR_INVALID_ARG, "%s: the anchors of pyramid level %d are not mirror-symmetric about image_w / 2 for a %dx%d image "
                       "(BOD_VIEW_HFLIP needs image_w to be a multiple of 2^max_level = %d)", who, h->mirror_bad_level, c.image_h, c.image_w,
                       1 << c.max_level);
    return BOD_OK;
}

static bod_status stat_fold(bod_handle h, const char* who, const float* cls, const float* box, const float* cov, int kb, int32_t view = BOD_VIEW_IDENTITY) {
    if (kb < 1) return h->fail(BOD_ERR_INVALID_ARG, "%s: a record of %d samples", who, kb);
    if (h->stat_k > (1 << 24) - kb) return h->fail(BOD_ERR_INVALID_ARG, "%s: more than 2^24 samples in one accumulator", who);
    if (h->class_parts && h->stat_ent_k != h->stat_k)
        return h->fail(BOD_ERR_NOT_READY, "%s: ent_sum holds %d of the record's %d samples (bod_stat_merge_entropy / bod_stat_set_entropy has not followed)", who, h->stat_ent_k, h->stat_k);
    StatMergeArgs m{};
    m.BA = (int64_t)h->cfg.batch * h->A; m.C = h->cfg.num_classes; m.ka = h->stat_k; m.kb = kb;
    m.acc_cls = h->stat_acc[0]; m.acc_box = h->stat_acc[1]; m.acc_cov = h->stat_acc[2];
    m.src_cls = cls; m.src_box = box; m.src_cov = h->cfg.has_covar_head ? cov : nullptr;
    if (!cls || !box || (h->cfg.has_covar_head && !cov)) return h->fail(BOD_ERR_INVALID_ARG, "%s: NULL statistics array", who);
    if (cls == m.acc_cls || box == m.acc_box) return h->fail(BOD_ERR_INVALID_ARG, "%s: the source is the accumulator itself", who);
    if (((uintptr_t)cls | (uintptr_t)box | (uintptr_t)m.src_cov) & 15u) return h->fail(BOD_ERR_INVALID_ARG, "%s: statistics arrays must be 16-byte aligned", who);
    if (view == BOD_VIEW_HFLIP) {
        StatMirrorArgs mm{};
        mm.m = m; mm.A = h->A; mm.K = h->cfg.anchors_per_location; mm.nlev = h->nlev;
        for (int l = 0; l < h->nlev; ++l) { mm.lvl_off[l] = (int32_t)h->lvl_p0[l] * mm.K; mm.lvl_w[l] = h->lw[l]; }
        mm.lvl_off[h->nlev] = h->A;
        mm.u_flip = (float)(h->cfg.image_w - 1);
        HIPCHK(h, launch_stat_merge_mirror(mm, h->stream));
    } else {
        HIPCHK(h, launch_stat_merge(m, h->stream));
    }
    h->stat_k += kb;
    return BOD_OK;
}

static bod_status stat_fold_entropy(bod_handle h, const char* who, const float* ent, int32_t view = BOD_VIEW_IDENTITY) {
    if (!ent) return h->fail(BOD_ERR_INVALID_ARG, "%s: ent_sum is NULL", who);
    if (ent == h->stat_ent) return h->fail(BOD_ERR_INVALID_ARG, "%s: the source is the accumulator itself", who);
    if ((uintptr_t)ent & 15u) return h->fail(BOD_ERR_INVALID_ARG, "%s: ent_sum must be 16-byte aligned", who);
    if (h->stat_ent_k >= h->stat_k) return h->fail(BOD_ERR_NOT_READY, "%s: ent_sum already holds the record's %d samples (fold the three arrays first)", who, h->stat_k);
    const int64_t BA = (int64_t)h->cfg.batch * h->A;
    if (view == BOD_VIEW_HFLIP) {
        StatMirrorArgs mm{};
        mm.A = h->A; mm.K = h->cfg.anchors_per_location; mm.nlev = h->nlev;
        for (int l = 0; l < h->nlev; ++l) { mm.lvl_off[l] = (int32_t)h->lvl_p0[l] * mm.K; mm.lvl_w[l] = h->lw[l]; }
        mm.lvl_off[h->nlev] = h->A;
        HIPCHK(h, launch_stat_merge_entropy(h->stat_ent, ent, BA, h->stat_ent_k == 0, &mm, h->stream));
    } else {
        HIPCHK(h, launch_stat_merge_entropy(h->stat_ent, ent, BA, h->stat_ent_k == 0, nullptr, h->stream));
    }
    h->stat_ent_k = h->stat_k;
// ... 228 lines not shown
```

### bayes-od-rc_amd/csrc/kernels.h

```cpp
#pragma once
#include <hip/hip_runtime.h>
#include <stdint.h>
#include "plan_tables.h"
#include "sparse_tables.h"


struct ConvGroup {
    const void* in;
    const void* w;
    const float* bias;
    void* out;
    const void* res;
    void* out_relu;
    int32_t in_coff;
    int32_t layer_id;
    const void* w2;
    const float* bias2;
    float* out2;
    int32_t cout2;
    int32_t out2_cstride;
    int32_t agg_kind;
    int32_t agg_n;
    int32_t agg_P;
    int32_t agg_C;
// ... 41 lines not shown
    int32_t n_cu;
    int32_t stagger_ticks;
    int32_t fan_chunk;
    int32_t mx;
    int32_t mx_loader;
    int32_t tile_rows;
    const int32_t* tile_count;
};

struct PerDeviceOnce {
    bool done[64] = {false};
    bool* slot() { int d = 0; if (hipGetDevice(&d) != hipSuccess || d < 0 || d >= 64) d = 0; return &done[d]; }
};

int device_cu_count();
inline int launch_cus(const ConvArgs& a) { return a.n_cu > 0 ? a.n_cu : device_cu_count(); }
hipError_t launch_conv_igemm(const ConvArgs& a, hipStream_t s);
bool conv_igemm_uses_full_cout_tile(const ConvArgs& a);
bool conv_igemm_uses_big_tile(const ConvArgs& a);
void conv_igemm_phase_cycles(unsigned long long* out16, bool reset);
hipError_t launch_conv_igemm_f32(const ConvArgs& a, hipStream_t s);
hipError_t launch_pairs_to_hx(const void* in, void* out, long npix, int C, hipStream_t s, int fmt = 1);

hipError_t launch_stem_conv(const float* img, const float* w, const float* bias, void* out, int out_f32,
                            int B, int H, int W, int oh, int ow, hipStream_t s);
bool stem_pool_fused_applies(const float* img, int B, int W, int ow, int n_cu);
hipError_t launch_stem_pool_fused(const float* img, const float* w, const float* bias, void* pooled, int split, int B, int H, int W, int oh,
                                  int ow, int ph, int pw, int pool_pitch, int pool_plane, hipStream_t s);
hipError_t launch_stem_pool(const void* in, void* out, int mode, int B, int ih, int iw, int oh, int ow,
                            int out_pitch, int out_plane, hipStream_t s);

struct PostCfg {
    int32_t B, N, A, C, draws;
    int32_t use_full_covar, has_covar, dirichlet, gaussian_iso, ranking_method;
    float iso_var;
    float kitti_sh, kitti_sw;
    const float* kitti_frame;
    uint32_t seed_lo, seed_hi, image_base;
    int32_t aggregated;
};

struct PostBuffers {
    const float* cls;
    const float* box;
    const float* cov;
    const float* anchors;
    const float* agg_cls;
    const float* agg_box;
    const float* agg_cov;
    uint8_t* keep;
    float* d_counts;
    int32_t* block_counts;
    int32_t* num_kept;
    float* counts;
    float* score;
    float* means;
    float* covs;
    float* ranking;
    float* corners;
    int32_t* anchor_index;
};

hipError_t launch_posterior(const PostCfg& c, const PostBuffers& b, hipStream_t s);
hipError_t launch_posterior_keep(const PostCfg& c, const PostBuffers& b, hipStream_t s);
hipError_t launch_posterior_fuse(const PostCfg& c, const PostBuffers& b, hipStream_t s);

struct SparseTailArgs {
    const uint8_t* keep;
    const RowEnt* pix;
    RowEnt* rows;
    int2* ext;
    RowEnt* halo_rows;
    int2* halo_ext;
    int32_t* tile_count;
    int2* runs;
    StQuad* chunks;
    StQuad* tiles;
    int32_t B, N, P, apl, cap_tiles;
    int32_t tail_rows;
    int64_t Ppad;
    SparseLevels lv;
};
hipError_t launch_sparse_tail_rows(const SparseTailArgs& a, hipStream_t s);
hipError_t launch_joint_entropy_rank(const PostCfg& c, const PostBuffers& b, hipStream_t s);
hipError_t launch_validation_post(const PostCfg& c, const PostBuffers& b, hipStream_t s);

struct NmsArgs {
    int32_t B, A;
    const int32_t* num_kept;
    const float* corners;
    const float* ranking;
    float* work_scores;
    int32_t* work_begin;
    int32_t* selected;
    int32_t* num_selected;
    int32_t max_out;
    float iou_thr, sigma;
    int32_t variant;
};
hipError_t launch_nms(const NmsArgs& a, hipStream_t s);

struct ValGatherArgs {
    int32_t B, A, C, max_out;
    const int32_t* num_kept;
    const int32_t* selected;
    const int32_t* num_selected;
    const float* score;
    const float* corners;
    float* out_scores;
    float* out_corners;
    int32_t* out_num;
};
hipError_t launch_validation_gather(const ValGatherArgs& a, hipStream_t s);

struct ClusterArgs {
    int32_t B, A, C, max_out;
    const int32_t* num_kept;
    const int32_t* selected;
    const int32_t* num_selected;
    const float* corners;
    const float* counts;
    const float* means;
    const float* covs;
    float thr;
    const float* affinity; int32_t affinity_img;
    float* out_scores; float* out_means; float* out_covs; float* out_counts;
};
hipError_t launch_cluster_fuse(const ClusterArgs& a, hipStream_t s);
hipError_t launch_iou_matrix(const float* corners, int M, float* out, hipStream_t s);
#define BOD_PARTS_TRI 30
hipError_t launch_posterior_parts(const PostCfg& c, const PostBuffers& b, float* parts, hipStream_t s);
hipError_t launch_cluster_parts(const ClusterArgs& a, const float* parts, float* out_parts, hipStream_t s);
#define BOD_LOG_SDEN(x) (__builtin_amdgcn_logf(x) * 0.693147180559945f)
hipError_t launch_posterior_class_parts(const PostCfg& c, const PostBuffers& b, const float* ent_sum, float* cparts, hipStream_t s);
hipError_t launch_cluster_class_parts(const ClusterArgs& a, const float* cparts, float* out_cparts, hipStream_t s);
hipError_t launch_pack_records(const int32_t* num, const float* scores, const float* means, const float* covs, const float* counts,
                               float* rec, int B, int K, int C, hipStream_t s);
hipError_t launch_pack_records_parts(const int32_t* num, const float* scores, const float* means, const float* covs, const float* counts,
                                     const float* parts, float* rec, int B, int K, int C, hipStream_t s);
hipError_t launch_pack_records_class(const int32_t* num, const float* scores, const float* means, const float* covs, const float* counts,
                                     const float* parts, const float* cparts, float* rec, int B, int K, int C, hipStream_t s);

struct PreprocArgs {
    const uint8_t* src;
    float* dst;
    int32_t B, sh, sw;
    int32_t rh, rw;
    int32_t H, W;
    int32_t crop_y, crop_x, pad_y, pad_x, vis_h, vis_w;
    int32_t resize;
    float scale_y, scale_x;
    float mean[3];
};
hipError_t launch_preprocess(const PreprocArgs& a, hipStream_t s);

struct PreprocFrame {
    int64_t offset;
    int32_t sh, sw, rh, rw;
    float scale_y, scale_x;
    int32_t crop_y, crop_x, pad_y, pad_x, vis_h, vis_w;
};
struct PreprocRaggedArgs {
    const uint8_t* src;
    float* dst;
    const PreprocFrame* frames;
    int32_t B, H, W;
// ... 192 lines not shown
```

### bayes-od-rc_amd/csrc/post_kernels.hip

```cpp
#include "kernels.h"
#include "philox.h"
#include <algorithm>
#include <math.h>

#define POST_BLOCK 256
#define MAXC 16

struct Mat4 { float m[4][4]; };

__device__ __forceinline__ Mat4 inv_spd4_once(const Mat4& a) {
    float g[4][4];
#pragma unroll
    for (int i = 0; i < 4; ++i)
#pragma unroll
        for (int j = 0; j < 4; ++j) g[i][j] = 0.f;
#pragma unroll
    for (int j = 0; j < 4; ++j) {
        float d = a.m[j][j];
#pragma unroll
        for (int k = 0; k < j; ++k) d -= g[j][k] * g[j][k];
        const float dj = sqrtf(d);
        g[j][j] = dj;
        const float inv = 1.0f / dj;
#pragma unroll
        for (int i = j + 1; i < 4; ++i) {
            float s = a.m[i][j];
#pragma unroll
            for (int k = 0; k < j; ++k) s -= g[i][k] * g[j][k];
            g[i][j] = s * inv;
        }
    }
    float h[4][4];
#pragma unroll
    for (int i = 0; i < 4; ++i)
#pragma unroll
        for (int j = 0; j < 4; ++j) h[i][j] = 0.f;
#pragma unroll
    for (int j = 0; j < 4; ++j) {
        h[j][j] = 1.0f / g[j][j];
#pragma unroll
        for (int i = j + 1; i < 4; ++i) {
            float s = 0.f;
#pragma unroll
            for (int k = j; k < i; ++k) s += g[i][k] * h[k][j];
            h[i][j] = -s / g[i][i];
        }
    }
    Mat4 r;
#pragma unroll
    for (int i = 0; i < 4; ++i)
#pragma unroll
        for (int j = 0; j <= i; ++j) {
            float s = 0.f;
#pragma unroll
            for (int k = i; k < 4; ++k) s += h[k][i] * h[k][j];
            r.m[i][j] = s;
            r.m[j][i] = s;
        }
    return r;
}

__device__ __forceinline__ Mat4 inv_spd4(const Mat4& a) { return inv_spd4_once(a); }

__device__ __forceinline__ void decode_box(const float4 anc, const float4 t, float o[4]) {
    o[0] = anc.z * t.x / 10.0f + anc.x;
    o[1] = anc.w * t.y / 10.0f + anc.y;
    o[2] = anc.z * fminf(fmaxf(expf(t.z / 5.0f), 1e-4f), 1e4f);
    o[3] = anc.w * fminf(fmaxf(expf(t.w / 5.0f), 1e-4f), 1e4f);
}

template <int C>
__global__ __launch_bounds__(POST_BLOCK) void post_sample_kernel(PostCfg c, PostBuffers pb, int nblocks) {
    const int a = blockIdx.x * POST_BLOCK + threadIdx.x;
    const int b = blockIdx.y;
    bool keep = false;
    if (a < c.A) {
        float mp[C];
#pragma unroll
        for (int j = 0; j < C; ++j) mp[j] = 0.f;
        if (c.aggregated) {
            const float* l = pb.agg_cls + ((size_t)b * c.A + a) * C;
#pragma unroll
            for (int j = 0; j < C; ++j) mp[j] = l[j];
        }
        for (int n = 0; n < (c.aggregated ? 0 : c.N); ++n) {
            const float* l = pb.cls + (((size_t)b * c.N + n) * c.A + a) * C;
            float v[C];
            if (C % 4 == 0) {
#pragma unroll
                for (int q = 0; q < C / 4; ++q) {
                    const float4 t = reinterpret_cast<const float4*>(l)[q];
                    v[4 * q] = t.x; v[4 * q + 1] = t.y; v[4 * q + 2] = t.z; v[4 * q + 3] = t.w;
                }
            } else {
#pragma unroll
                for (int j = 0; j < C; ++j) v[j] = l[j];
            }
            float mx = v[0];
#pragma unroll
            for (int j = 1; j < C; ++j) mx = fmaxf(mx, v[j]);
            float s = 0.f;
#pragma unroll
            for (int j = 0; j < C; ++j) { v[j] = expf(v[j] - mx); s += v[j]; }
#pragma unroll
            for (int j = 0; j < C; ++j) mp[j] += v[j] / s;
        }
        float cdf[C];
        float accum = 0.f;
#pragma unroll
        for (int j = 0; j < C; ++j) { mp[j] = mp[j] / (float)c.N; accum += mp[j]; cdf[j] = accum; }
        const float total = cdf[C - 1];
        int cnt[C];
#pragma unroll
        for (int j = 0; j < C; ++j) cnt[j] = 0;
        const int groups = (c.draws + 3) / 4;
        for (int g = 0; g < groups; ++g) {
            const Philox4 r = philox4x32_10((uint32_t)a, (uint32_t)g, BOD_CAT_TAG, c.image_base + b,
                                            c.seed_lo, c.seed_hi);
            const uint32_t w[4] = {r.x, r.y, r.z, r.w};
#pragma unroll
            for (int q = 0; q < 4; ++q) {
                if (4 * g + q < c.draws) {
                    const float t = (float)(w[q] >> 8) * 5.9604644775390625e-8f * total;
                    int k = 0;
#pragma unroll
                    for (int j = 0; j < C; ++j) k += (cdf[j] <= t) ? 1 : 0;
                    k = k < C - 1 ? k : C - 1;
#pragma unroll
                    for (int j = 0; j < C; ++j) cnt[j] += (j == k) ? 1 : 0;
                }
            }
        }
        int best = 0, bestc = cnt[0];
#pragma unroll
        for (int j = 1; j < C; ++j)
            if (cnt[j] > bestc) { bestc = cnt[j]; best = j; }
        keep = best != C - 1;
        pb.keep[(size_t)b * c.A + a] = keep ? 1 : 0;
        float* dc = pb.d_counts + ((size_t)b * c.A + a) * C;
#pragma unroll
        for (int j = 0; j < C; ++j) dc[j] = (float)cnt[j];
    }
    const int n = __syncthreads_count(keep ? 1 : 0);
    if (threadIdx.x == 0) pb.block_counts[(size_t)b * nblocks + blockIdx.x] = n;
}

__global__ __launch_bounds__(POST_BLOCK) void post_scan_kernel(PostBuffers pb, int nblocks) {
    __shared__ int part[POST_BLOCK];
    const int b = blockIdx.x, tid = threadIdx.x;
    int* bc = pb.block_counts + (size_t)b * nblocks;
    const int per = (nblocks + POST_BLOCK - 1) / POST_BLOCK;
    int local = 0;
    for (int i = 0; i < per; ++i) {
        const int idx = tid * per + i;
        if (idx < nblocks) local += bc[idx];
    }
    part[tid] = local;
    __syncthreads();
    if (tid == 0) {
        int run = 0;
        for (int i = 0; i < POST_BLOCK; ++i) { const int t = part[i]; part[i] = run; run += t; }
        pb.num_kept[b] = run;
    }
    __syncthreads();
    int run = part[tid];
    for (int i = 0; i < per; ++i) {
        const int idx = tid * per + i;
        if (idx < nblocks) { const int t = bc[idx]; bc[idx] = run; run += t; }
    }
}

__global__ __launch_bounds__(POST_BLOCK) void post_compact_kernel(PostCfg c, PostBuffers pb, int nblocks) {
    __shared__ int wave_off[POST_BLOCK / 64 + 1];
    const int tid = threadIdx.x, lane = tid & 63, wave = tid >> 6;
    const int a = blockIdx.x * POST_BLOCK + tid;
    const int b = blockIdx.y;
    const bool keep = (a < c.A) && pb.keep[(size_t)b * c.A + a];
    const unsigned long long bal = __ballot(keep);
    const int before = __popcll(bal & ((1ull << lane) - 1ull));
    if (lane == 0) wave_off[wave + 1] = __popcll(bal);
    if (tid == 0) wave_off[0] = 0;
    __syncthreads();
    if (tid == 0)
        for (int w = 1; w <= POST_BLOCK / 64; ++w) wave_off[w] += wave_off[w - 1];
    __syncthreads();
    if (!keep) return;
    const int slot = pb.block_counts[(size_t)b * nblocks + blockIdx.x] + wave_off[wave] + before;
    pb.anchor_index[(size_t)b * c.A + slot] = a;
}

#if defined(BOD_POST_SELFCHECK)
#define POST_FUSE_INLINE __noinline__
#if BOD_POST_SELFCHECK == 2
struct FuseIn { float4 anc, ab[4]; float2 cv[5]; float dc[8]; };
#define POST_FUSE_OUT , float* __restrict__ out20, const FuseIn& fin
#else
#define POST_FUSE_OUT , float* __restrict__ out20
#endif
struct SelfcheckRec { uint32_t hw_id, xcc_id, image, slot, lane, elem; float first, second; };
__device__ unsigned int g_selfcheck_count;
__device__ unsigned long long g_selfcheck_waves;
__device__ SelfcheckRec g_selfcheck_recs[4096];
#else
#define POST_FUSE_INLINE __forceinline__
#define POST_FUSE_OUT
#endif
template <int C>
__device__ POST_FUSE_INLINE void post_fuse_anchor(const PostCfg& c, const PostBuffers& pb, const int b, const int slot POST_FUSE_OUT) {
    const size_t o = (size_t)b * c.A + slot;
#if defined(BOD_POST_SELFCHECK) && BOD_POST_SELFCHECK == 2
    const int a = 0; (void)a; (void)o;
    const float4 anc = fin.anc;
#else
    const int a = pb.anchor_index[o];

    const float4 anc = reinterpret_cast<const float4*>(pb.anchors)[a];
#endif
    float mu[4] = {0.f, 0.f, 0.f, 0.f};
    Mat4 epi;
#pragma unroll
    for (int i = 0; i < 4; ++i)
#pragma unroll
        for (int j = 0; j < 4; ++j) epi.m[i][j] = 0.f;
    const int n_raw = c.aggregated ? 0 : c.N;
// ... 181 lines not shown
    }
#endif
#if defined(BOD_POST_SELFCHECK)
#pragma unroll
    for (int i = 0; i < 4; ++i) {
        out20[i] = pm[i];
#pragma unroll
        for (int j = 0; j < 4; ++j) out20[4 + i * 4 + j] = pcov.m[i][j];
    }
#endif
#if defined(BOD_POST_SELFCHECK) && BOD_POST_SELFCHECK == 2
    out20[0] += best * 0.f;
    return;
#else
    pb.ranking[o] = best;
    pb.corners[o * 4 + 0] = pm[0] - pm[2] / 2.0f;
    pb.corners[o * 4 + 1] = pm[1] - pm[3] / 2.0f;
    pb.corners[o * 4 + 2] = pm[0] + pm[2] / 2.0f;
    pb.corners[o * 4 + 3] = pm[1] + pm[3] / 2.0f;
#endif
}

#define POST_FUSE_BLOCKS 8
template <int C>
__global__ __launch_bounds__(POST_BLOCK) void post_fuse_kernel(PostCfg c, PostBuffers pb, int nblocks) {
    const int b = blockIdx.y;
    const int m = pb.num_kept[b];
#if defined(BOD_POST_SELFCHECK)
    for (int slot = blockIdx.x * POST_BLOCK + threadIdx.x; slot < m; slot += gridDim.x * POST_BLOCK) {
        float r1[20], r2[20];
#if BOD_POST_SELFCHECK == 2
        FuseIn fin;
        {
            const size_t o = (size_t)b * c.A + slot;
            const int a = pb.anchor_index[o];
            fin.anc = reinterpret_cast<const float4*>(pb.anchors)[a];
            for (int q = 0; q < 4; ++q) fin.ab[q] = (reinterpret_cast<const float4*>(pb.agg_box) + ((size_t)b * c.A + a) * 4)[q];
            for (int q = 0; q < 5; ++q) fin.cv[q] = reinterpret_cast<const float2*>(pb.agg_cov + ((size_t)b * c.A + a) * 10)[q];
            for (int q = 0; q < 8; ++q) fin.dc[q] = q < C ? pb.d_counts[((size_t)b * c.A + a) * C + q] : 0.f;
        }
        asm volatile("s_waitcnt vmcnt(0) lgkmcnt(0)" ::: "memory");
        post_fuse_anchor<C>(c, pb, b, slot, r1, fin);
        post_fuse_anchor<C>(c, pb, b, slot, r2, fin);
#else
        post_fuse_anchor<C>(c, pb, b, slot, r1);
        post_fuse_anchor<C>(c, pb, b, slot, r2);
#endif
        if ((threadIdx.x & 63) == 0) atomicAdd(&g_selfcheck_waves, 1ull);
        int bad = -1;
        for (int i = 19; i >= 0; --i) if (__float_as_uint(r1[i]) != __float_as_uint(r2[i])) bad = i;
        if (bad >= 0) {
            const unsigned int k = atomicAdd(&g_selfcheck_count, 1u);
            if (k < 4096u) {
                SelfcheckRec r;
                r.hw_id = __builtin_amdgcn_s_getreg((31 << 11) | 4);
                r.xcc_id = __builtin_amdgcn_s_getreg((31 << 11) | 20);
                r.image = (uint32_t)b; r.slot = (uint32_t)slot; r.lane = threadIdx.x & 63; r.elem = (uint32_t)bad;
                r.first = r1[bad]; r.second = r2[bad];
                g_selfcheck_recs[k] = r;
            }
        }
    }
#else
    for (int slot = blockIdx.x * POST_BLOCK + threadIdx.x; slot < m; slot += gridDim.x * POST_BLOCK) post_fuse_anchor<C>(c, pb, b, slot);
#endif
}
#if defined(BOD_POST_SELFCHECK)
extern "C" int bod_debug_selfcheck_read(unsigned int* count, unsigned long long* waves, void* recs, int max) {
    unsigned int n = 0;
    if (hipMemcpyFromSymbol(&n, HIP_SYMBOL(g_selfcheck_count), 4) != hipSuccess) return 1;
    if (hipMemcpyFromSymbol(waves, HIP_SYMBOL(g_selfcheck_waves), 8) != hipSuccess) return 1;
    const unsigned int m = n < (unsigned)max ? n : (unsigned)max;
    if (m && hipMemcpyFromSymbol(recs, HIP_SYMBOL(g_selfcheck_recs), (size_t)(m < 4096u ? m : 4096u) * sizeof(SelfcheckRec)) != hipSuccess) return 1;
    const unsigned int z = 0; const unsigned long long z8 = 0;
    if (hipMemcpyToSymbol(HIP_SYMBOL(g_selfcheck_count), &z, 4) != hipSuccess || hipMemcpyToSymbol(HIP_SYMBOL(g_selfcheck_waves), &z8, 8) != hipSuccess) return 1;
    *count = n;
    return 0;
}
#endif

hipError_t launch_posterior_keep(const PostCfg& c, const PostBuffers& b, hipStream_t s) {
    const int nblocks = (c.A + POST_BLOCK - 1) / POST_BLOCK;
    dim3 grid(nblocks, c.B);
    if (c.C == 8) hipLaunchKernelGGL(post_sample_kernel<8>, grid, dim3(POST_BLOCK), 0, s, c, b, nblocks);
    else if (c.C == 4) hipLaunchKernelGGL(post_sample_kernel<4>, grid, dim3(POST_BLOCK), 0, s, c, b, nblocks);
    else return hipErrorInvalidValue;
    hipLaunchKernelGGL(post_scan_kernel, dim3(c.B), dim3(POST_BLOCK), 0, s, b, nblocks);
    return hipGetLastError();
}

hipError_t launch_posterior_fuse(const PostCfg& c, const PostBuffers& b, hipStream_t s) {
    const int nblocks = (c.A + POST_BLOCK - 1) / POST_BLOCK;
    dim3 grid(nblocks, c.B);
    if (c.C != 8 && c.C != 4) return hipErrorInvalidValue;
    hipLaunchKernelGGL(post_compact_kernel, grid, dim3(POST_BLOCK), 0, s, c, b, nblocks);
    if (c.C == 8) hipLaunchKernelGGL(post_fuse_kernel<8>, dim3(std::min(nblocks, POST_FUSE_BLOCKS), c.B), dim3(POST_BLOCK), 0, s, c, b, nblocks);
    else hipLaunchKernelGGL(post_fuse_kernel<4>, dim3(std::min(nblocks, POST_FUSE_BLOCKS), c.B), dim3(POST_BLOCK), 0, s, c, b, nblocks);
    return hipGetLastError();
}

hipError_t launch_posterior(const PostCfg& c, const PostBuffers& b, hipStream_t s) {
    const hipError_t e = launch_posterior_keep(c, b, s);
    return e != hipSuccess ? e : launch_posterior_fuse(c, b, s);
}

__device__ __forceinline__ void parts_congruence(const Mat4& g, const Mat4& x, const float sc[4], float* __restrict__ out) {
    Mat4 t;
#pragma unroll
    for (int i = 0; i < 4; ++i)
#pragma unroll
        for (int j = 0; j < 4; ++j) {
            float s = 0.f;
#pragma unroll
            for (int k = 0; k < 4; ++k) s += g.m[i][k] * x.m[k][j];
            t.m[i][j] = s;
        }
    int q = 0;
#pragma unroll
    for (int i = 0; i < 4; ++i)
#pragma unroll
        for (int j = 0; j <= i; ++j) {
            float s = 0.f;
#pragma unroll
            for (int k = 0; k < 4; ++k) s += t.m[i][k] * g.m[j][k];
            out[q++] = sc[i] * s * sc[j];
        }
}

__global__ __launch_bounds__(POST_BLOCK) void post_parts_kernel(PostCfg c, PostBuffers pb, float* __restrict__ parts) {
    const int b = blockIdx.y;
    const int m = pb.num_kept[b];
    for (int slot = blockIdx.x * POST_BLOCK + threadIdx.x; slot < m; slot += gridDim.x * POST_BLOCK) {
        const size_t o = (size_t)b * c.A + slot;
        const int a = pb.anchor_index[o];
        const float4 anc = reinterpret_cast<const float4*>(pb.anchors)[a];
        float mu[4] = {0.f, 0.f, 0.f, 0.f};
        Mat4 epi;
#pragma unroll
        for (int i = 0; i < 4; ++i)
#pragma unroll
            for (int j = 0; j < 4; ++j) epi.m[i][j] = 0.f;
        const int n_raw = c.aggregated ? 0 : c.N;
        if (c.aggregated) {
            const float4* ab = reinterpret_cast<const float4*>(pb.agg_box) + ((size_t)b * c.A + a) * 4;
            const float4 q0 = ab[1], q1 = ab[2], q2 = ab[3];
            epi.m[0][0] = q0.x; epi.m[1][0] = q0.y; epi.m[1][1] = q0.z; epi.m[2][0] = q0.w;
            epi.m[2][1] = q1.x; epi.m[2][2] = q1.y; epi.m[3][0] = q1.z; epi.m[3][1] = q1.w;
            epi.m[3][2] = q2.x; epi.m[3][3] = q2.y;
        }
        for (int n = 0; n < n_raw; ++n) {
            const float4 t = reinterpret_cast<const float4*>(pb.box)[((size_t)b * c.N + n) * c.A + a];
            float bx[4];
            decode_box(anc, t, bx);
#pragma unroll
            for (int i = 0; i < 4; ++i) mu[i] += bx[i];
        }
        if (!c.aggregated) {
#pragma unroll
            for (int i = 0; i < 4; ++i) mu[i] = mu[i] / (float)c.N;
        }
        for (int n = 0; n < n_raw; ++n) {
            const float4 t = reinterpret_cast<const float4*>(pb.box)[((size_t)b * c.N + n) * c.A + a];
            float bx[4];
            decode_box(anc, t, bx);
#pragma unroll
            for (int i = 0; i < 4; ++i) bx[i] -= mu[i];
#pragma unroll
            for (int i = 0; i < 4; ++i)
#pragma unroll
// ... 102 lines not shown
            parts_congruence(g, al, sc, out + 10);
        } else {
#pragma unroll
            for (int q = 0; q < 10; ++q) out[10 + q] = 0.f;
        }
        int q = 0;
#pragma unroll
        for (int i = 0; i < 4; ++i)
#pragma unroll
            for (int j = 0; j <= i; ++j) out[20 + q++] = sc[i] * pp.m[i][j] * sc[j];
    }
}

hipError_t launch_posterior_parts(const PostCfg& c, const PostBuffers& b, float* parts, hipStream_t s) {
    if (!parts) return hipErrorInvalidValue;
    const int nblocks = (c.A + POST_BLOCK - 1) / POST_BLOCK;
    hipLaunchKernelGGL(post_parts_kernel, dim3(std::min(nblocks, POST_FUSE_BLOCKS), c.B), dim3(POST_BLOCK), 0, s, c, b, parts);
    return hipGetLastError();
}

template <int C>
__global__ __launch_bounds__(POST_BLOCK) void post_class_parts_kernel(PostCfg c, PostBuffers pb, const float* __restrict__ ent_sum,
                                                                      float* __restrict__ cparts) {
    const int b = blockIdx.y;
    const int m = pb.num_kept[b];
    for (int slot = blockIdx.x * POST_BLOCK + threadIdx.x; slot < m; slot += gridDim.x * POST_BLOCK) {
        const size_t o = (size_t)b * c.A + slot;
        const int a = pb.anchor_index[o];
        float mp[C];
        float ent = 0.f;
#pragma unroll
        for (int j = 0; j < C; ++j) mp[j] = 0.f;
        if (c.aggregated) {
            const float4* l = reinterpret_cast<const float4*>(pb.agg_cls + ((size_t)b * c.A + a) * C);
#pragma unroll
            for (int k = 0; k < C / 4; ++k) {
                const float4 t = l[k];
                mp[4 * k] = t.x; mp[4 * k + 1] = t.y; mp[4 * k + 2] = t.z; mp[4 * k + 3] = t.w;
            }
            ent = ent_sum[(size_t)b * c.A + a];
        }
        for (int n = 0; n < (c.aggregated ? 0 : c.N); ++n) {
            const float* l = pb.cls + (((size_t)b * c.N + n) * c.A + a) * C;
            float v[C];
#pragma unroll
            for (int k = 0; k < C / 4; ++k) {
                const float4 t = reinterpret_cast<const float4*>(l)[k];
                v[4 * k] = t.x; v[4 * k + 1] = t.y; v[4 * k + 2] = t.z; v[4 * k + 3] = t.w;
            }
            float mx = v[0];
#pragma unroll
            for (int j = 1; j < C; ++j) mx = fmaxf(mx, v[j]);
            float sden = 0.f, dot = 0.f;
#pragma unroll
            for (int j = 0; j < C; ++j) { const float d = v[j] - mx; v[j] = expf(d); sden += v[j]; dot += v[j] * d; }
            ent += BOD_LOG_SDEN(sden) - dot / sden;
#pragma unroll
            for (int j = 0; j < C; ++j) mp[j] += v[j] / sden;
        }
        const float fk = (float)c.N;
        float total = 0.f;
#pragma unroll
        for (int j = 0; j < C; ++j) {
            mp[j] = mp[j] / fk;
            if (mp[j] > 0.f) total -= mp[j] * logf(mp[j]);
        }
        const float ale = ent / fk;
        float* out = cparts + o * (3 + C);
        out[0] = total; out[1] = ale; out[2] = fmaxf(total - ale, 0.f);
#pragma unroll
        for (int j = 0; j < C; ++j) out[3 + j] = mp[j];
    }
}

hipError_t launch_posterior_class_parts(const PostCfg& c, const PostBuffers& b, const float* ent_sum, float* cparts, hipStream_t s) {
    if (!cparts || (c.aggregated && !ent_sum) || (c.C != 4 && c.C != 8)) return hipErrorInvalidValue;
    const int nblocks = (c.A + POST_BLOCK - 1) / POST_BLOCK;
    const dim3 grid(std::min(nblocks, POST_FUSE_BLOCKS), c.B);
    if (c.C == 8) hipLaunchKernelGGL(post_class_parts_kernel<8>, grid, dim3(POST_BLOCK), 0, s, c, b, ent_sum, cparts);
    else hipLaunchKernelGGL(post_class_parts_kernel<4>, grid, dim3(POST_BLOCK), 0, s, c, b, ent_sum, cparts);
    return hipGetLastError();
}

__global__ __launch_bounds__(256) void sparse_tail_rows_kernel(SparseTailArgs a) {
    extern __shared__ uint8_t s_flag[];
    __shared__ int s_cnt[2][256];
    __shared__ int s_nrun[2], s_nchunk[2], s_ntile[2], s_base[2];
    const int b = blockIdx.x, tid = threadIdx.x, N = a.N, P = a.P, B = a.B;
    const int T = a.halo_rows ? 2 : 1;
    const SparseLevels& lv = a.lv;
    const uint8_t* keep = a.keep + (size_t)b * P * a.apl;
    for (int p = tid; p < P; p += blockDim.x) {
        uint8_t f = 0;
        for (int k = 0; k < a.apl; ++k) f |= keep[(size_t)p * a.apl + k];
        s_flag[p] = f ? ST_KEPT : 0;
    }
    __syncthreads();
    for (int p = tid; p < P; p += blockDim.x) if (st_member(s_flag, lv, p, ST_KEPT)) s_flag[p] |= ST_TAIL;
    if (T == 2) {
        __syncthreads();
        for (int p = tid; p < P; p += blockDim.x) if (st_dilated(s_flag, lv, p)) s_flag[p] |= ST_DIL;
        __syncthreads();
        for (int p = tid; p < P; p += blockDim.x) if (st_member(s_flag, lv, p, ST_DIL)) s_flag[p] |= ST_HALO;
    }
    __syncthreads();
    const int share = (P + 255) / 256, q0 = min(P, tid * share), q1 = min(P, q0 + share);
    int cnt[2] = {0, 0};
    for (int t = 0; t < T; ++t) {
        const uint8_t bit = t == 0 ? ST_TAIL : ST_HALO;
        for (int p = q0; p < q1; ++p) cnt[t] += st_run_edge(s_flag, lv, p, bit) & 1;
        s_cnt[t][tid] = cnt[t];
    }
    __syncthreads();
    for (int d = 1; d < 256; d <<= 1) {
        int v[2] = {0, 0};
        for (int t = 0; t < T; ++t) v[t] = tid >= d ? s_cnt[t][tid - d] : 0;
        __syncthreads();
        for (int t = 0; t < T; ++t) s_cnt[t][tid] += v[t];
        __syncthreads();
    }
    for (int t = 0; t < T; ++t) {
        const uint8_t bit = t == 0 ? ST_TAIL : ST_HALO;
        int2* runs = a.runs + ((size_t)t * B + b) * P;
        int r = s_cnt[t][tid] - cnt[t];
        for (int p = q0; p < q1; ++p) {
            const int edge = st_run_edge(s_flag, lv, p, bit);
            if (edge & 1) runs[r++].x = p;
            if (edge & 2) runs[r - 1].y = p;
        }
        if (tid == 255) s_nrun[t] = s_cnt[t][255];
    }
    __syncthreads();
    const int wave = tid >> 6, lane = tid & 63;
    if (wave < T) {
        const int t = wave;
        const int2* runs = a.runs + ((size_t)t * B + b) * P;
        StQuad* chunks = a.chunks + ((size_t)t * B + b) * P;
        StQuad* tiles = a.tiles + ((size_t)t * B + b) * P;
        const int nrun = s_nrun[t];
        const int R = t == 0 ? a.tail_rows : 256;
        StPack st{0, 0, 0, 0, 0, 0};
        for (int r0 = 0; r0 < nrun; r0 += 64) {
            const int2 mine = r0 + lane < nrun ? runs[r0 + lane] : make_int2(0, 0);
            const int n = min(64, nrun - r0);
            for (int j = 0; j < n; ++j) {
                const int p = __shfl(mine.x, j), q = __shfl(mine.y, j);
                st_pack_run(st, p, q - p + 1, N, chunks, tiles, lane == 0, R);
            }
        }
        st_pack_close(st, tiles, lane == 0);
        if (lane == 0) {
            s_nchunk[t] = st.nchunk; s_ntile[t] = st.ntile;
            s_base[t] = atomicAdd(a.tile_count + t, st.ntile);
        }
    }
    __syncthreads();
    const RowEnt invalid = st_invalid_row(a.pix[0]);
    for (int t = 0; t < T; ++t) {
        const int nchunk = s_nchunk[t], ntile = s_ntile[t], base = s_base[t];
        const int R = t == 0 ? a.tail_rows : 256;
        if (base + ntile > a.cap_tiles) continue;
        RowEnt* rows = t == 0 ? a.rows : a.halo_rows;
        ExtRow* ext = reinterpret_cast<ExtRow*>(t == 0 ? a.ext : a.halo_ext);
        const StQuad* chunks = a.chunks + ((size_t)t * B + b) * P;
        const StQuad* tiles = a.tiles + ((size_t)t * B + b) * P;
        for (int i = tid; i < nchunk * N; i += blockDim.x) {
            const int ci = i / N, n = i - ci * N;
            const StQuad c = chunks[ci];
            st_write_piece(c, n, b, base + c.y, a.pix, N, P, a.Ppad, rows, ext, R);
        }
        for (int i = tid; i < ntile * R; i += blockDim.x) {
            const int tt = i / R, r = i - tt * R;
            if (st_pad_row(tiles[tt], r, N)) rows[(size_t)(base + tt) * R + r] = invalid;
        }
        for (int i = tid; i < ntile * XR_EXT_ROWS; i += blockDim.x) {
            const int tt = i / XR_EXT_ROWS, r = i - tt * XR_EXT_ROWS;
            const StQuad ti = tiles[tt];
            if (r >= ti.z) ext[(size_t)(base + tt) * XR_EXT_ROWS + r] = st_pad_ext(ti, b, a.pix, N, P, a.Ppad);
        }
    }
}

hipError_t launch_sparse_tail_rows(const SparseTailArgs& a, hipStream_t s) {
    if (a.B <= 0 || a.P <= 0 || a.N < 1 || 256 / a.N < 1 || XR_EXT_ROWS / a.N - 2 < 1 || a.P > 65536 || a.lv.n < 1 || a.lv.n > 5)
        return hipErrorInvalidValue;
    if ((a.tail_rows != 192 && a.tail_rows != 256) || a.tail_rows / a.N < 1) return hipErrorInvalidValue;
    hipError_t e = hipMemsetAsync(a.tile_count, 0, 2 * sizeof(int32_t), s);
    if (e != hipSuccess) return e;
    hipLaunchKernelGGL(sparse_tail_rows_kernel, dim3(a.B), dim3(256), (size_t)a.P, s, a);
    return hipGetLastError();
}

template <int C>
__global__ __launch_bounds__(POST_BLOCK) void val_flag_kernel(PostCfg c, PostBuffers pb, int nblocks) {
    const int a = blockIdx.x * POST_BLOCK + threadIdx.x;
    const int b = blockIdx.y;
    bool keep = false;
    if (a < c.A) {
        const float* l = pb.cls + (((size_t)b * c.N) * c.A + a) * C;
        float v[C];
#pragma unroll
        for (int j = 0; j < C; ++j) v[j] = l[j];
        float mx = v[0];
#pragma unroll
        for (int j = 1; j < C; ++j) mx = fmaxf(mx, v[j]);
        float s = 0.f;
#pragma unroll
        for (int j = 0; j < C; ++j) { v[j] = expf(v[j] - mx); s += v[j]; }
        int best = 0; float bestp = v[0] / s;
        float* dc = pb.d_counts + ((size_t)b * c.A + a) * C;
#pragma unroll
        for (int j = 0; j < C; ++j) {
            const float pj = v[j] / s;
            dc[j] = pj;
            if (j > 0 && pj > bestp) { bestp = pj; best = j; }
        }
        keep = best != C - 1;
        pb.keep[(size_t)b * c.A + a] = keep ? 1 : 0;
    }
    const int n = __syncthreads_count(keep ? 1 : 0);
    if (threadIdx.x == 0) pb.block_counts[(size_t)b * nblocks + blockIdx.x] = n;
}

template <int C>
__global__ __launch_bounds__(POST_BLOCK) void val_fuse_kernel(PostCfg c, PostBuffers pb, int nblocks) {
    __shared__ int wave_off[POST_BLOCK / 64 + 1];
    const int tid = threadIdx.x, lane = tid & 63, wave = tid >> 6;
    const int a = blockIdx.x * POST_BLOCK + tid;
    const int b = blockIdx.y;
    const bool keep = (a < c.A) && pb.keep[(size_t)b * c.A + a];
    const unsigned long long bal = __ballot(keep);
    const int before = __popcll(bal & ((1ull << lane) - 1ull));
    if (lane == 0) wave_off[wave + 1] = __popcll(bal);
    if (tid == 0) wave_off[0] = 0;
    __syncthreads();
    if (tid == 0)
        for (int w = 1; w <= POST_BLOCK / 64; ++w) wave_off[w] += wave_off[w - 1];
    __syncthreads();
    if (!keep) return;
    const int slot = pb.block_counts[(size_t)b * nblocks + blockIdx.x] + wave_off[wave] + before;
    const size_t o = (size_t)b * c.A + slot;
    const float4 anc = reinterpret_cast<const float4*>(pb.anchors)[a];
    const float4 t = reinterpret_cast<const float4*>(pb.box)[((size_t)b * c.N) * c.A + a];
    float bx[4];
    decode_box(anc, t, bx);
    const float* dc = pb.d_counts + ((size_t)b * c.A + a) * C;
    float top = dc[0];
#pragma unroll
    for (int j = 0; j < C; ++j) { pb.counts[o * C + j] = dc[j]; pb.score[o * C + j] = dc[j]; top = fmaxf(top, dc[j]); }
#pragma unroll
    for (int i = 0; i < 4; ++i) pb.means[o * 4 + i] = bx[i];
#pragma unroll
    for (int i = 0; i < 16; ++i) pb.covs[o * 16 + i] = 0.f;
    pb.ranking[o] = top;
    reinterpret_cast<float4*>(pb.corners)[o] = make_float4(bx[0] - bx[2] / 2.0f, bx[1] - bx[3] / 2.0f, bx[0] + bx[2] / 2.0f, bx[1] + bx[3] / 2.0f);
    pb.anchor_index[o] = a;
}

hipError_t launch_validation_post(const PostCfg& c, const PostBuffers& b, hipStream_t s) {
    const int nblocks = (c.A + POST_BLOCK - 1) / POST_BLOCK;
    dim3 grid(nblocks, c.B);
    if (c.C == 8) {
        hipLaunchKernelGGL(val_flag_kernel<8>, grid, dim3(POST_BLOCK), 0, s, c, b, nblocks);
        hipLaunchKernelGGL(post_scan_kernel, dim3(c.B), dim3(POST_BLOCK), 0, s, b, nblocks);
        hipLaunchKernelGGL(val_fuse_kernel<8>, grid, dim3(POST_BLOCK), 0, s, c, b, nblocks);
    } else if (c.C == 4) {
        hipLaunchKernelGGL(val_flag_kernel<4>, grid, dim3(POST_BLOCK), 0, s, c, b, nblocks);
        hipLaunchKernelGGL(post_scan_kernel, dim3(c.B), dim3(POST_BLOCK), 0, s, b, nblocks);
        hipLaunchKernelGGL(val_fuse_kernel<4>, grid, dim3(POST_BLOCK), 0, s, c, b, nblocks);
    } else {
        return hipErrorInvalidValue;
    }
// ... 355 lines not shown
            for (int o = 32; o > 0; o >>= 1) {
                const float ok = __shfl_xor(bk, o, 64);
                const int oi = __shfl_xor(bi, o, 64);
                if (oi != 0x7fffffff && (bi == 0x7fffffff || ok < bk || (ok == bk && oi < bi))) { bk = ok; bi = oi; }
            }
            if (lane == 0) { top_kl[wave * 3 + r] = bk; top_ix[wave * 3 + r] = bi; }
            if (bi != 0x7fffffff && ci == bi) ++p;
        }
    }
    __syncthreads();
#pragma unroll
    for (int q = 0; q < 10; ++q) psum[q] = (red[q] + red[16 + q]) + (red[32 + q] + red[48 + q]);
#pragma unroll
    for (int q = 0; q < 4; ++q) pmsum[q] = (red[10 + q] + red[26 + q]) + (red[42 + q] + red[58 + q]);
    const int total = (int)((red[14] + red[30]) + (red[46] + red[62]));
    if (total <= 3) {
        __syncthreads();
#pragma unroll
        for (int j = 0; j < C; ++j) {
            const float r0 = wsum(ssum[j]), r1 = wsum(csum[j]);
            if (lane == 0) { red[wave * 16 + j] = r0; red[64 + wave * 16 + j] = r1; }
        }
        __syncthreads();
#pragma unroll
        for (int j = 0; j < C; ++j) {
            ssum[j] = (red[j] + red[16 + j]) + (red[32 + j] + red[48 + j]);
            csum[j] = (red[64 + j] + red[80 + j]) + (red[96 + j] + red[112 + j]);
        }
    }
    if (tid != 0) return;
    const size_t ob = (size_t)b * a.max_out + k;
    Mat4 ps;
    {
        int t = 0;
#pragma unroll
        for (int r = 0; r < 4; ++r)
#pragma unroll
            for (int q = 0; q <= r; ++q) { ps.m[r][q] = psum[t]; ps.m[q][r] = psum[t]; ++t; }
    }
    const Mat4 fc = inv_spd4(ps);
#pragma unroll
    for (int r = 0; r < 4; ++r) {
        float s = 0.f;
#pragma unroll
        for (int q = 0; q < 4; ++q) s += fc.m[r][q] * pmsum[q];
        a.out_means[ob * 4 + r] = s;
#pragma unroll
        for (int q = 0; q < 4; ++q) a.out_covs[ob * 16 + r * 4 + q] = fc.m[r][q] * 70.0f;
    }
    if (total > 3) {
        float bk[3] = {INFINITY, INFINITY, INFINITY};
        int bx[3] = {0x7fffffff, 0x7fffffff, 0x7fffffff};
        for (int t = 0; t < 4 * 3; ++t) {
            const float kl = top_kl[t]; const int ix = top_ix[t];
            if (ix == 0x7fffffff) continue;
            if (kl < bk[2] || (kl == bk[2] && ix < bx[2])) {
                bk[2] = kl; bx[2] = ix;
                if (bk[2] < bk[1] || (bk[2] == bk[1] && bx[2] < bx[1])) {
                    float f = bk[1]; bk[1] = bk[2]; bk[2] = f; int g = bx[1]; bx[1] = bx[2]; bx[2] = g;
                    if (bk[1] < bk[0] || (bk[1] == bk[0] && bx[1] < bx[0])) {
                        f = bk[0]; bk[0] = bk[1]; bk[1] = f; g = bx[0]; bx[0] = bx[1]; bx[1] = g;
                    }
                }
            }
        }
#pragma unroll
        for (int j = 0; j < C; ++j) { ssum[j] = 0.f; csum[j] = 0.f; }
        for (int t = 0; t < 3; ++t) {
            float row[C], rs = 0.f;
#pragma unroll
            for (int j = 0; j < C; ++j) { row[j] = a.counts[(base + bx[t]) * C + j]; rs += row[j]; }
#pragma unroll
            for (int j = 0; j < C; ++j) { ssum[j] += row[j] / rs; csum[j] += row[j]; }
        }
    }
    const float denom = (float)(total > 3 ? 3 : total);
#pragma unroll
    for (int j = 0; j < C; ++j) {
        a.out_scores[ob * C + j] = ssum[j] / denom;
        a.out_counts[ob * C + j] = csum[j];
    }
}

hipError_t launch_cluster_fuse(const ClusterArgs& a, hipStream_t s) {
    dim3 grid(a.max_out, a.B);
    if (a.C == 8) hipLaunchKernelGGL(cluster_fuse_kernel<8>, grid, dim3(CL_BLOCK), 0, s, a);
    else if (a.C == 4) hipLaunchKernelGGL(cluster_fuse_kernel<4>, grid, dim3(CL_BLOCK), 0, s, a);
    else return hipErrorInvalidValue;
    return hipGetLastError();
}

__global__ __launch_bounds__(CL_BLOCK) void cluster_parts_kernel(ClusterArgs a, const float* __restrict__ parts, float* __restrict__ out_parts) {
    __shared__ float red[4 * 40];
    const int k = blockIdx.x, b = blockIdx.y, tid = threadIdx.x;
    if (k >= a.num_selected[b]) return;
    const int M = a.num_kept[b];
    const int centre = a.selected[(size_t)b * a.max_out + k];
    const size_t base = (size_t)b * a.A;
    const float4* boxes = reinterpret_cast<const float4*>(a.corners) + base;
    const float4 cbox = boxes[centre];
    float acc[40];
#pragma unroll
    for (int q = 0; q < 40; ++q) acc[q] = 0.f;
    const float* aff = (a.affinity && b == a.affinity_img) ? a.affinity + (size_t)k * a.A : nullptr;
    for (int i = tid; i < M; i += CL_BLOCK) {
        if (!((aff ? aff[i] : iou_plus1(boxes[i], cbox)) > a.thr)) continue;
        Mat4 cv;
#pragma unroll
        for (int r = 0; r < 4; ++r)
#pragma unroll
            for (int q = 0; q < 4; ++q) cv.m[r][q] = a.covs[(base + i) * 16 + r * 4 + q];
        const Mat4 pr = inv_spd4(cv);
        {
            int t = 0;
#pragma unroll
            for (int r = 0; r < 4; ++r)
#pragma unroll
                for (int q = 0; q <= r; ++q) acc[30 + t++] += pr.m[r][q];
        }
        const float* x = parts + (base + i) * BOD_PARTS_TRI;
        const float one[4] = {1.f, 1.f, 1.f, 1.f};
#pragma unroll
        for (int part = 0; part < 3; ++part) {
            Mat4 xm;
            int t = 0;
#pragma unroll
            for (int r = 0; r < 4; ++r)
#pragma unroll
                for (int q = 0; q <= r; ++q) { xm.m[r][q] = x[part * 10 + t]; xm.m[q][r] = xm.m[r][q]; ++t; }
            float pxp[10];
            parts_congruence(pr, xm, one, pxp);
#pragma unroll
            for (int q = 0; q < 10; ++q) acc[part * 10 + q] += pxp[q];
        }
    }
    const int wave = tid >> 6, lane = tid & 63;
#pragma unroll
    for (int q = 0; q < 40; ++q) {
        float v = acc[q];
#pragma unroll
        for (int o = 32; o > 0; o >>= 1) v += __shfl_xor(v, o, 64);
        if (lane == 0) red[wave * 40 + q] = v;
    }
    __syncthreads();
    if (tid != 0) return;
#pragma unroll
    for (int q = 0; q < 40; ++q) acc[q] = (red[q] + red[40 + q]) + (red[80 + q] + red[120 + q]);
    Mat4 ps;
    {
        int t = 0;
#pragma unroll
        for (int r = 0; r < 4; ++r)
#pragma unroll
            for (int q = 0; q <= r; ++q) { ps.m[r][q] = acc[30 + t]; ps.m[q][r] = acc[30 + t]; ++t; }
    }
    const Mat4 fc = inv_spd4(ps);
    const float one[4] = {1.f, 1.f, 1.f, 1.f};
    float* out = out_parts + ((size_t)b * a.max_out + k) * 48;
#pragma unroll
    for (int part = 0; part < 3; ++part) {
        Mat4 sm;
        int t = 0;
#pragma unroll
        for (int r = 0; r < 4; ++r)
#pragma unroll
            for (int q = 0; q <= r; ++q) { sm.m[r][q] = acc[part * 10 + t]; sm.m[q][r] = sm.m[r][q]; ++t; }
        float fsf[10];
        parts_congruence(fc, sm, one, fsf);
        t = 0;
#pragma unroll
        for (int r = 0; r < 4; ++r)
// ... 263 lines not shown
```

### bayes-od-rc_amd/engine.py

```python
import ctypes as C

import numpy as np

from . import _lib
from ._lib import BodConfig, BodSizes, as_f32, fptr, iptr

_KINDS = {"kernel": 0, "bias": 1, "gamma": 2, "beta": 3, "mean": 4, "var": 5}
PRECISIONS = {"bf16": 0, "fp32": 1, "bf16x3": 2, "f16mx": 3, "f16mx4": 4}
VIEWS = {"identity": _lib.BOD_VIEW_IDENTITY, "hflip": _lib.BOD_VIEW_HFLIP}


def make_config(image_hw, batch=1, mc_samples=10, num_classes=8, anchors_per_location=9, device=0,
                dropout_rate=0.3, use_full_covar=True, bayes_od_config=None, nms_config=None,
                has_covar_head=True, dataset_name='bdd', orig_size=None, nms_variant='A',
                num_categorical_draws=30, layers=(3, 4, 5, 6, 7), precision='bf16', mc_sample_base=0,
                mc_ensemble_size=0, training=False, backbone_depth=50, pipeline_overlap=False, mc_statistics=False,
                covariance_parts=False, class_parts=False):
    bo = bayes_od_config or {'ranking_method': 'score', 'dirichlet_prior': {'type': 'non_informative'},
                             'gaussian_prior': {'type': 'isotropic', 'isotropic_variance': 100000.0}}
    nms = nms_config or {'max_output_size': 100, 'iou_threshold': 0.5, 'soft_nms_sigma': 0.5}
    cfg = BodConfig()
    cfg.device = int(device)
    cfg.image_h, cfg.image_w = int(image_hw[0]), int(image_hw[1])
    cfg.batch, cfg.mc_samples = int(batch), int(mc_samples)
# ... 593 lines not shown
            self._chk(self.lib.bod_stat_merge(self.h, p, int(samples)))
        else:
            self._chk(self.lib.bod_stat_merge_view(self.h, p, int(samples), v))
        if len(ptrs) > 3 and ptrs[3]:
            self.stat_merge_entropy(ptrs[3], view=v)

    def stat_merge_entropy(self, ptr, view=0):
        self._chk(self.lib.bod_stat_merge_entropy(self.h, C.c_void_p(int(ptr)), self._view(view)))

    def stat_device_entropy_pointer(self):
        p = C.c_void_p(0)
        self._chk(self.lib.bod_stat_device_entropy(self.h, C.byref(p)))
        return int(p.value or 0)

    def get_entropy(self):
        ent = np.empty((self.B, self.A), np.float32)
        self._chk(self.lib.bod_stat_get_entropy(self.h, fptr(ent)))
        return ent

    def set_entropy(self, ent_sum):
        ent = as_f32(ent_sum)
        if ent.shape != (self.B, self.A):
            raise ValueError("ent_sum of shape %s, expected %s" % (ent.shape, (self.B, self.A)))
        self._chk(self.lib.bod_stat_set_entropy(self.h, fptr(ent)))

    def stat_device_pointers(self):
        ptrs = (C.c_void_p * 3)()
        self._chk(self.lib.bod_stat_device(self.h, ptrs, None))
        return [ptrs[i] for i in range(3)]

    @property
    def stat_samples(self):
        k = C.c_int32(0)
        self._chk(self.lib.bod_stat_device(self.h, None, C.byref(k)))
        return int(k.value)

    def get_statistics(self):
        n = (self.B, self.A)
        cls = np.empty(n + (self.Ccls,), np.float32)
        box = np.empty(n + (16,), np.float32)
        cov = np.empty(n + (10,), np.float32) if self.cfg.has_covar_head else None
        k = C.c_int32(0)
        self._chk(self.lib.bod_stat_get(self.h, fptr(cls), fptr(box), fptr(cov), C.byref(k)))
        return cls, box, cov, int(k.value)

    def set_statistics(self, cls_sum, box_moments, cov_sum=None, samples=0):
        n = (self.B, self.A)
        arrs = []
        for a, w in ((cls_sum, self.Ccls), (box_moments, 16), (cov_sum, 10)):
            a = as_f32(a) if a is not None else None
            if a is not None and a.shape != n + (w,):
                raise ValueError("statistics array of shape %s, expected %s" % (a.shape, n + (w,)))
            arrs.append(a)
        self._chk(self.lib.bod_stat_set(self.h, fptr(arrs[0]), fptr(arrs[1]), fptr(arrs[2]), int(samples)))

    def stat_posterior(self, seed=0, first_image_id=0):
        self._chk(self.lib.bod_stat_posterior(self.h, seed, first_image_id))

    def bench_head_conv(self, layer=1, variant=0, iters=10):
        ms, fl = C.c_double(0), C.c_double(0)
        self._chk(self.lib.bod_bench_head_conv(self.h, layer, variant, iters, C.byref(ms), C.byref(fl)))
        return ms.value, fl.value

    def gather_detections(self, slot=-1, comm=None, world=1, rank=0, root=0, want_host=True):
        w = int(self.lib.bod_record_width(self.h))
        out = None
        dev = C.c_void_p(0)
        if rank == root and want_host:
            out = np.empty((world, self.B, self.K, w), np.float32)
        self._chk(self.lib.bod_gather_detections(self.h, int(slot), C.c_void_p(int(comm) if comm else 0), int(world), int(rank), int(root),
                                                 out.ctypes.data if out is not None else None,
                                                 C.byref(dev) if rank == root else None))
        if rank == root and not want_host:
            return int(dev.value or 0), (world, self.B, self.K, w)
        return out

    def plan_info(self):
        info = (C.c_int32 * 10)()
        self._chk(self.lib.bod_plan_info_n(self.h, info, 10))
        return {"aggregating": bool(info[0]), "fused_head_outputs": bool(info[1]), "row_reuse": bool(info[2]),
                "fan_out_row_reuse": bool(info[3]), "ops": int(info[4]), "plane_row_reuse_layers": int(info[5]), "tower_mx": bool(info[6]), "tower_mx_format": int(info[6]),
                "sparse_tail": bool(info[7]), "sparse_halo": bool(info[8]), "sparse_tail_rows": int(info[9])}

    @property
    def aggregating(self):
        return self.plan_info()["aggregating"]

    def profile_begin(self, which=None):
        if which is not None:
            self._chk(self.lib.bod_profile_select(self.h, int(which)))
        self._chk(self.lib.bod_profile_begin(self.h))

    def profile_end(self):
        hm, pm, fl = C.c_double(0), C.c_double(0), C.c_double(0)
        hl, pl = C.c_int64(0), C.c_int64(0)
        self._chk(self.lib.bod_profile_end(self.h, C.byref(hm), C.byref(hl), C.byref(fl), C.byref(pm), C.byref(pl)))
        return {"head_conv_ms": hm.value, "head_conv_launches": hl.value, "head_conv_flops": fl.value,
                "posterior_ms": pm.value, "posterior_launches": pl.value}


def pack_ragged(frames, batch=None):
    frames = list(frames)
    if batch is not None and len(frames) != int(batch):
        raise ValueError("expected %d frames, got %d" % (int(batch), len(frames)))
    if not frames:
        raise ValueError("no frames to pack")
    for i, f in enumerate(frames):
        if not isinstance(f, np.ndarray) or f.dtype != np.uint8 or f.ndim != 3 or f.shape[2] != 3 or f.shape[0] < 1 or f.shape[1] < 1:
            raise ValueError("frame %d: expected a uint8 array of shape (h, w, 3), got %s %s" %
                             (i, getattr(f, "dtype", type(f).__name__), getattr(f, "shape", "")))
    sizes = np.asarray([f.shape[:2] for f in frames], np.int32)
    buf = np.empty(3 * int(np.sum(sizes[:, 0].astype(np.int64) * sizes[:, 1])), np.uint8)
    off = 0
    for f in frames:
        buf[off:off + f.size] = f.reshape(-1)
        off += f.size
    return buf, sizes


AUGMENT_DTYPE = np.dtype([("flip", "<i4"), ("scale", "<f4"), ("off_y", "<f4"), ("off_x", "<f4"), ("gain", "<f4"), ("bias", "<f4")])
AUGMENT_IDENTITY = {"flip": 0, "scale": 1.0, "off_y": 0.5, "off_x": 0.5, "gain": 1.0, "bias": 0.0}
AUGMENT_DEFAULTS = {"flip_probability": 0.5, "scale_range": [0.8, 1.25], "random_placement": True, "gain_range": [0.8, 1.2],
                    "bias_range": [-20.0, 20.0], "min_visible": 0.25}


def augment_records(aug, batch=None):
    if isinstance(aug, np.ndarray):
        if aug.dtype != AUGMENT_DTYPE:
            raise ValueError("augmentation records must have dtype AUGMENT_DTYPE, got %s" % (aug.dtype,))
        rec = np.ascontiguousarray(aug).reshape(-1)
    else:
        rec = np.empty(len(aug), AUGMENT_DTYPE)
        for i, d in enumerate(aug):
            unknown = set(d) - set(AUGMENT_IDENTITY)
            if unknown:
                raise ValueError("frame %d: unknown augmentation field(s) %s" % (i, sorted(unknown)))
            rec[i] = tuple(d.get(k, v) for k, v in AUGMENT_IDENTITY.items())
    if batch is not None and rec.shape[0] != int(batch):
        raise ValueError("expected %d augmentation records, got %d" % (int(batch), rec.shape[0]))
    return rec


def augment_config(cfg=None):
    out = dict(AUGMENT_DEFAULTS)
    unknown = set(cfg or {}) - set(out)
    if unknown:
        raise ValueError("unknown augmentation setting(s) %s (known: %s)" % (sorted(unknown), sorted(out)))
    out.update(cfg or {})
    return out


def _f32_in(x, lo, hi):
    v = np.float32(x)
    if float(v) > hi:
        v = np.nextafter(v, np.float32(-np.inf))
    elif float(v) < lo:
        v = np.nextafter(v, np.float32(np.inf))
    return v


def draw_augmentation(cfg, seed, image_ids):
    cfg = augment_config(cfg)
    ids = [int(i) for i in np.asarray(image_ids).reshape(-1)]
    rec = np.empty(len(ids), AUGMENT_DTYPE)
    (s_lo, s_hi), (g_lo, g_hi), (b_lo, b_hi) = cfg["scale_range"], cfg["gain_range"], cfg["bias_range"]
    if not (0.0 < s_lo <= s_hi) or g_lo > g_hi or b_lo > b_hi or not (0.0 <= cfg["flip_probability"] <= 1.0):
# ... 235 lines not shown
```

### include/bayesod.h

```cpp
#ifndef BAYESOD_H
#define BAYESOD_H

#include <stdint.h>

#ifdef __cplusplus
extern "C" {
#endif

typedef struct bod_context* bod_handle;

typedef enum {
    BOD_OK = 0,
    BOD_ERR_INVALID_ARG = 1,
    BOD_ERR_HIP = 2,
    BOD_ERR_OOM = 3,
    BOD_ERR_NOT_READY = 4,
    BOD_ERR_NO_DEVICE = 5
} bod_status;

enum { BOD_RANK_SCORE = 0, BOD_RANK_JOINT_ENTROPY = 1 };
enum { BOD_NMS_VARIANT_A = 0, BOD_NMS_VARIANT_B = 1 };
enum { BOD_HEAD_CLS = 0, BOD_HEAD_REG = 1, BOD_HEAD_COV = 2 };
enum { BOD_PRECISION_BF16 = 0, BOD_PRECISION_FP32 = 1, BOD_PRECISION_BF16X3 = 2, BOD_PRECISION_F16MX = 3, BOD_PRECISION_F16MX4 = 4 };

// ... 171 lines not shown
                            const float* covar_params, const float* anchors, const uint8_t* positive_mask,
                            const uint8_t* negative_mask, int32_t do_classification, int32_t reg_kind,
                            float label_smoothing, double* out4);

#define BOD_LOSS_ONE_IMAGE_ID 1
typedef struct {
    int32_t energy_samples;
    uint64_t seed;
    uint32_t first_image_id;
    int32_t reserved[4];
} bod_loss_options;
bod_status bod_loss_forward_ex(int32_t device, int32_t B, int32_t A, int32_t C, const float* cls,
                               const float* cls_targets, const float* box, const float* box_targets,
                               const float* covar_params, const float* anchors, const uint8_t* positive_mask,
                               const uint8_t* negative_mask, int32_t do_classification, int32_t reg_kind,
                               float label_smoothing, double* out4, const bod_loss_options* options);
bod_status bod_set_loss_options(bod_handle h, const bod_loss_options* options);

bod_status bod_anchor_targets(int32_t device, int32_t A, const float* anchors_vuhw, int32_t B, const int32_t* num_gt,
                              const float* gt_boxes_vuvu, const float* gt_classes, int32_t C, float min_positive_iou,
                              float max_negative_iou, float* cls_targets, float* box_targets, uint8_t* positive_mask,
                              uint8_t* negative_mask, int32_t* best_gt, float* best_iou);

bod_status bod_validation_losses_boxes(bod_handle h, const int32_t* num_gt, const float* gt_boxes_vuvu, const float* gt_classes,
                                       float min_positive_iou, float max_negative_iou, int32_t do_classification,
                                       int32_t reg_kind, float label_smoothing, double* sums4);
bod_status bod_get_validation_detections_batch(bod_handle h, int32_t* num_detections, float* scores, float* corners);
bod_status bod_validate_boxes(bod_handle h, const float* images, int32_t images_on_device, const int32_t* num_gt,
                              const float* gt_boxes_vuvu, const float* gt_classes, float min_positive_iou,
                              float max_negative_iou, int32_t do_classification, int32_t reg_kind, float label_smoothing,
                              double* sums4, int32_t* num_detections, float* scores, float* corners);

bod_status bod_loss_backward(int32_t device, int32_t B, int32_t A, int32_t C, const float* cls,
                             const float* cls_targets, const float* box, const float* box_targets,
                             const float* covar_params, const float* anchors, const uint8_t* positive_mask,
                             const uint8_t* negative_mask, int32_t do_cls, int32_t reg_kind, float label_smoothing,
                             float w_cls, float w_reg, double* out4, float* dcls, float* dbox, float* dcov);
bod_status bod_loss_backward_ex(int32_t device, int32_t B, int32_t A, int32_t C, const float* cls,
                                const float* cls_targets, const float* box, const float* box_targets,
                                const float* covar_params, const float* anchors, const uint8_t* positive_mask,
                                const uint8_t* negative_mask, int32_t do_cls, int32_t reg_kind, float label_smoothing,
                                float w_cls, float w_reg, double* out4, float* dcls, float* dbox, float* dcov,
                                const bod_loss_options* options);

bod_status bod_pdq_corner_heatmaps(int32_t device, int32_t img_h, int32_t img_w, int32_t n, const double* means_yx,
                                   const double* covs_yx, int32_t* rois, float* heatmaps);
bod_status bod_pdq_frames(int32_t device, int32_t img_h, int32_t img_w, int32_t num_frames, const int32_t* num_gt,
                          const int32_t* gt_boxes, const int32_t* num_det, const int32_t* det_boxes,
                          const double* det_corner_covs, double* fg_loss, double* bg_loss, double* det_bg_loss,
                          float* heatmaps);

bod_status bod_score_pairs(int32_t device, int64_t n, const double* means, const double* covs, const double* targets,
                           int32_t num_samples, uint64_t seed, uint64_t first_row_id, double* out, int32_t* status);

bod_status bod_bench_head_conv(bod_handle h, int32_t layer, int32_t variant, int32_t iters,
                               double* mean_ms, double* flops_per_launch);

bod_status bod_profile_begin(bod_handle h);
bod_status bod_profile_select(bod_handle h, int32_t which);
bod_status bod_profile_end(bod_handle h, double* head_conv_ms, int64_t* head_conv_launches,
                           double* head_conv_flops, double* posterior_ms, int64_t* posterior_launches);

int32_t bod_record_width(bod_handle h);
bod_status bod_gather_detections(bod_handle h, int32_t slot, void* nccl_comm, int32_t world, int32_t rank, int32_t root,
                                 float* gathered_host, float** gathered_device);

bod_status bod_get_posterior_parts(bod_handle h, int32_t image_index, float* parts);
bod_status bod_set_posterior_parts(bod_handle h, int32_t image_index, int32_t m, const float* parts);
bod_status bod_get_detection_parts(bod_handle h, int32_t image_index, float* parts);
bod_status bod_get_detection_parts_batch(bod_handle h, float* parts);
bod_status bod_collect_parts(bod_handle h, int32_t slot, float* parts);
bod_status bod_device_detection_parts(bod_handle h, int32_t slot, void** ptr);

bod_status bod_get_posterior_class_parts(bod_handle h, int32_t image_index, float* rows);
bod_status bod_get_posterior_mean_probs(bod_handle h, int32_t image_index, float* mean_probs);
bod_status bod_set_posterior_class_parts(bod_handle h, int32_t image_index, int32_t m, const float* mean_probs, const float* rows);
bod_status bod_get_detection_class_parts(bod_handle h, int32_t image_index, float* rows);
bod_status bod_get_detection_class_parts_batch(bod_handle h, float* rows);
bod_status bod_collect_class_parts(bod_handle h, int32_t slot, float* rows);
bod_status bod_device_detection_class_parts(bod_handle h, int32_t slot, void** ptr);

bod_status bod_plan_info(bod_handle h, int32_t* info8);
bod_status bod_plan_info_n(bod_handle h, int32_t* info, int32_t n);

bod_status bod_stat_reset(bod_handle h);
bod_status bod_stat_forward(bod_handle h, const float* images, int32_t images_on_device, uint64_t seed, uint32_t first_image_id,
                            int32_t sample_base);
bod_status bod_stat_merge_from(bod_handle dst, bod_handle src);
bod_status bod_stat_merge(bod_handle h, const void* const* ptrs3, int32_t samples);
bod_status bod_stat_device(bod_handle h, void** ptrs3, int32_t* samples);
bod_status bod_stat_get(bod_handle h, float* cls_sum, float* box_moments, float* cov_sum, int32_t* samples);
bod_status bod_stat_set(bod_handle h, const float* cls_sum, const float* box_moments, const float* cov_sum, int32_t samples);
bod_status bod_stat_posterior(bod_handle h, uint64_t seed, uint32_t first_image_id);

enum { BOD_VIEW_IDENTITY = 0, BOD_VIEW_HFLIP = 1 };
bod_status bod_stat_forward_view(bod_handle h, const float* images, int32_t images_on_device, uint64_t seed, uint32_t first_image_id,
                                 int32_t sample_base, int32_t view);
bod_status bod_stat_merge_view(bod_handle h, const void* const* ptrs3, int32_t samples, int32_t view);

bod_status bod_stat_get_entropy(bod_handle h, float* ent_sum);
bod_status bod_stat_set_entropy(bod_handle h, const float* ent_sum);
bod_status bod_stat_device_entropy(bod_handle h, void** ptr);
bod_status bod_stat_merge_entropy(bod_handle h, const void* ent_sum, int32_t view);

#ifdef __cplusplus
}
#endif
#endif
```

### include/bayesod_cdef.h

```cpp
typedef struct bod_context* bod_handle;
typedef enum {
    BOD_OK = 0,
    BOD_ERR_INVALID_ARG = 1,
    BOD_ERR_HIP = 2,
    BOD_ERR_OOM = 3,
    BOD_ERR_NOT_READY = 4,
    BOD_ERR_NO_DEVICE = 5
} bod_status;
enum { BOD_RANK_SCORE = 0, BOD_RANK_JOINT_ENTROPY = 1 };
enum { BOD_NMS_VARIANT_A = 0, BOD_NMS_VARIANT_B = 1 };
enum { BOD_HEAD_CLS = 0, BOD_HEAD_REG = 1, BOD_HEAD_COV = 2 };
enum { BOD_PRECISION_BF16 = 0, BOD_PRECISION_FP32 = 1, BOD_PRECISION_BF16X3 = 2, BOD_PRECISION_F16MX = 3, BOD_PRECISION_F16MX4 = 4 };
typedef struct {
    int32_t device;
    int32_t image_h, image_w;
    int32_t batch;
    int32_t mc_samples;
    int32_t num_classes;
    int32_t anchors_per_location;
    int32_t min_level, max_level;
    float   dropout_rate;
    int32_t use_full_covar;
    int32_t dirichlet_non_informative;
    int32_t gaussian_isotropic;
// ... 129 lines not shown
                                const float* gt_boxes_vuvu, const float* gt_classes, float min_positive_iou,
                                float max_negative_iou, uint64_t seed, uint32_t first_image_id, int32_t reg_kind,
                                float label_smoothing, float w_cls, float w_reg, float l2_rate, float learning_rate,
                                int32_t apply_update, double* out6);
bod_status bod_train_get_targets(bod_handle h, float* cls_targets, float* box_targets, uint8_t* positive_mask,
                                 uint8_t* negative_mask);
bod_status bod_train_gradients(bod_handle h, void** device_ptr, int64_t* count);
bod_status bod_train_apply(bod_handle h, float learning_rate, double* grad_norm);
bod_status bod_train_get(bod_handle h, const char* layer, int32_t kind, int32_t what, float* out, int64_t n);
bod_status bod_train_set(bod_handle h, const char* layer, int32_t kind, int32_t what, const float* data, int64_t n);
bod_status bod_train_step_count(bod_handle h, int64_t* get, int64_t set);
bod_status bod_loss_forward(int32_t device, int32_t B, int32_t A, int32_t C, const float* cls,
                            const float* cls_targets, const float* box, const float* box_targets,
                            const float* covar_params, const float* anchors, const uint8_t* positive_mask,
                            const uint8_t* negative_mask, int32_t do_classification, int32_t reg_kind,
                            float label_smoothing, double* out4);
typedef struct {
    int32_t energy_samples;
    uint64_t seed;
    uint32_t first_image_id;
    int32_t reserved[4];
} bod_loss_options;
bod_status bod_loss_forward_ex(int32_t device, int32_t B, int32_t A, int32_t C, const float* cls,
                               const float* cls_targets, const float* box, const float* box_targets,
                               const float* covar_params, const float* anchors, const uint8_t* positive_mask,
                               const uint8_t* negative_mask, int32_t do_classification, int32_t reg_kind,
                               float label_smoothing, double* out4, const bod_loss_options* options);
bod_status bod_set_loss_options(bod_handle h, const bod_loss_options* options);
bod_status bod_anchor_targets(int32_t device, int32_t A, const float* anchors_vuhw, int32_t B, const int32_t* num_gt,
                              const float* gt_boxes_vuvu, const float* gt_classes, int32_t C, float min_positive_iou,
                              float max_negative_iou, float* cls_targets, float* box_targets, uint8_t* positive_mask,
                              uint8_t* negative_mask, int32_t* best_gt, float* best_iou);
bod_status bod_validation_losses_boxes(bod_handle h, const int32_t* num_gt, const float* gt_boxes_vuvu, const float* gt_classes,
                                       float min_positive_iou, float max_negative_iou, int32_t do_classification,
                                       int32_t reg_kind, float label_smoothing, double* sums4);
bod_status bod_get_validation_detections_batch(bod_handle h, int32_t* num_detections, float* scores, float* corners);
bod_status bod_validate_boxes(bod_handle h, const float* images, int32_t images_on_device, const int32_t* num_gt,
                              const float* gt_boxes_vuvu, const float* gt_classes, float min_positive_iou,
                              float max_negative_iou, int32_t do_classification, int32_t reg_kind, float label_smoothing,
                              double* sums4, int32_t* num_detections, float* scores, float* corners);
bod_status bod_loss_backward(int32_t device, int32_t B, int32_t A, int32_t C, const float* cls,
                             const float* cls_targets, const float* box, const float* box_targets,
                             const float* covar_params, const float* anchors, const uint8_t* positive_mask,
                             const uint8_t* negative_mask, int32_t do_cls, int32_t reg_kind, float label_smoothing,
                             float w_cls, float w_reg, double* out4, float* dcls, float* dbox, float* dcov);
bod_status bod_loss_backward_ex(int32_t device, int32_t B, int32_t A, int32_t C, const float* cls,
                                const float* cls_targets, const float* box, const float* box_targets,
                                const float* covar_params, const float* anchors, const uint8_t* positive_mask,
                                const uint8_t* negative_mask, int32_t do_cls, int32_t reg_kind, float label_smoothing,
                                float w_cls, float w_reg, double* out4, float* dcls, float* dbox, float* dcov,
                                const bod_loss_options* options);
bod_status bod_pdq_corner_heatmaps(int32_t device, int32_t img_h, int32_t img_w, int32_t n, const double* means_yx,
                                   const double* covs_yx, int32_t* rois, float* heatmaps);
bod_status bod_pdq_frames(int32_t device, int32_t img_h, int32_t img_w, int32_t num_frames, const int32_t* num_gt,
                          const int32_t* gt_boxes, const int32_t* num_det, const int32_t* det_boxes,
                          const double* det_corner_covs, double* fg_loss, double* bg_loss, double* det_bg_loss,
                          float* heatmaps);
bod_status bod_score_pairs(int32_t device, int64_t n, const double* means, const double* covs, const double* targets,
                           int32_t num_samples, uint64_t seed, uint64_t first_row_id, double* out, int32_t* status);
bod_status bod_bench_head_conv(bod_handle h, int32_t layer, int32_t variant, int32_t iters,
                               double* mean_ms, double* flops_per_launch);
bod_status bod_profile_begin(bod_handle h);
bod_status bod_profile_select(bod_handle h, int32_t which);
bod_status bod_profile_end(bod_handle h, double* head_conv_ms, int64_t* head_conv_launches,
                           double* head_conv_flops, double* posterior_ms, int64_t* posterior_launches);
int32_t bod_record_width(bod_handle h);
bod_status bod_gather_detections(bod_handle h, int32_t slot, void* nccl_comm, int32_t world, int32_t rank, int32_t root,
                                 float* gathered_host, float** gathered_device);
bod_status bod_get_posterior_parts(bod_handle h, int32_t image_index, float* parts);
bod_status bod_set_posterior_parts(bod_handle h, int32_t image_index, int32_t m, const float* parts);
bod_status bod_get_detection_parts(bod_handle h, int32_t image_index, float* parts);
bod_status bod_get_detection_parts_batch(bod_handle h, float* parts);
bod_status bod_collect_parts(bod_handle h, int32_t slot, float* parts);
bod_status bod_device_detection_parts(bod_handle h, int32_t slot, void** ptr);
bod_status bod_get_posterior_class_parts(bod_handle h, int32_t image_index, float* rows);
bod_status bod_get_posterior_mean_probs(bod_handle h, int32_t image_index, float* mean_probs);
bod_status bod_set_posterior_class_parts(bod_handle h, int32_t image_index, int32_t m, const float* mean_probs, const float* rows);
bod_status bod_get_detection_class_parts(bod_handle h, int32_t image_index, float* rows);
bod_status bod_get_detection_class_parts_batch(bod_handle h, float* rows);
bod_status bod_collect_class_parts(bod_handle h, int32_t slot, float* rows);
bod_status bod_device_detection_class_parts(bod_handle h, int32_t slot, void** ptr);
bod_status bod_plan_info(bod_handle h, int32_t* info8);
bod_status bod_plan_info_n(bod_handle h, int32_t* info, int32_t n);
bod_status bod_stat_reset(bod_handle h);
bod_status bod_stat_forward(bod_handle h, const float* images, int32_t images_on_device, uint64_t seed, uint32_t first_image_id,
                            int32_t sample_base);
bod_status bod_stat_merge_from(bod_handle dst, bod_handle src);
bod_status bod_stat_merge(bod_handle h, const void* const* ptrs3, int32_t samples);
bod_status bod_stat_device(bod_handle h, void** ptrs3, int32_t* samples);
bod_status bod_stat_get(bod_handle h, float* cls_sum, float* box_moments, float* cov_sum, int32_t* samples);
bod_status bod_stat_set(bod_handle h, const float* cls_sum, const float* box_moments, const float* cov_sum, int32_t samples);
bod_status bod_stat_posterior(bod_handle h, uint64_t seed, uint32_t first_image_id);
enum { BOD_VIEW_IDENTITY = 0, BOD_VIEW_HFLIP = 1 };
bod_status bod_stat_forward_view(bod_handle h, const float* images, int32_t images_on_device, uint64_t seed, uint32_t first_image_id,
                                 int32_t sample_base, int32_t view);
bod_status bod_stat_merge_view(bod_handle h, const void* const* ptrs3, int32_t samples, int32_t view);
bod_status bod_stat_get_entropy(bod_handle h, float* ent_sum);
bod_status bod_stat_set_entropy(bod_handle h, const float* ent_sum);
bod_status bod_stat_device_entropy(bod_handle h, void** ptr);
bod_status bod_stat_merge_entropy(bod_handle h, const void* ent_sum, int32_t view);
```

Measured before the change: 2273 images/sec.

## Coalesce output staging, pack posterior draws, split sparse rows, wave-level cluster fuse

```diff
diff --git a/bayes-od-rc_amd/_lib.py b/bayes-od-rc_amd/_lib.py
--- a/bayes-od-rc_amd/_lib.py
+++ b/bayes-od-rc_amd/_lib.py
@@ -164,6 +164,8 @@
     "bod_profile_select": (C.c_int, [_H, C.c_int32]),
     "bod_plan_info": (C.c_int, [_H, C.POINTER(C.c_int32)]),
     "bod_plan_info_n": (C.c_int, [_H, C.POINTER(C.c_int32), C.c_int32]),
+    "bod_get_sparse_table": (C.c_int, [_H, C.c_int32, C.c_int32, C.POINTER(C.c_int32), C.POINTER(C.c_int32), C.POINTER(C.c_int32),
+                                       C.POINTER(C.c_int32)]),
     "bod_stat_reset": (C.c_int, [_H]),
     "bod_stat_forward": (C.c_int, [_H, C.c_void_p, C.c_int32, C.c_uint64, C.c_uint32, C.c_int32]),
     "bod_stat_merge_from": (C.c_int, [_H, _H]),
diff --git a/bayes-od-rc_amd/csrc/engine.hip b/bayes-od-rc_amd/csrc/engine.hip
--- a/bayes-od-rc_amd/csrc/engine.hip
+++ b/bayes-od-rc_amd/csrc/engine.hip
@@ -292,6 +292,7 @@
     bool plan_sparse = false;
     bool plan_halo = false;
     SparseTailArgs sparse{};
+    StQuad* sparse_hdr = nullptr; int sparse_img_tiles = 0;
     int plan_tail_rows = 0;
     bool agg_sparse = false;
     float* stat_acc[3] = {nullptr};
@@ -315,6 +316,8 @@
     int32_t* nms_sel_s[2] = {nullptr, nullptr}; int32_t* nms_nsel_s[2] = {nullptr, nullptr};
     float* out_scores_s[2] = {nullptr, nullptr}; float* out_means_s[2] = {nullptr, nullptr};
     float* out_covs_s[2] = {nullptr, nullptr}; float* out_counts_s[2] = {nullptr, nullptr};
+    float* records_s[2] = {nullptr, nullptr}; size_t records_bytes = 0;
+    size_t stage_num() const { return ((size_t)cfg.batch + 63) & ~(size_t)63; }
     int32_t* nms_sel = nullptr; int32_t* nms_nsel = nullptr;
     float* out_scores = nullptr; float* out_means = nullptr; float* out_covs = nullptr; float* out_counts = nullptr;
     int slot = 0;
@@ -1027,6 +1030,8 @@
         BODCHK(h->dalloc(&sa.runs, (size_t)tables * B * h->P, false));
         BODCHK(h->dalloc(&sa.chunks, (size_t)tables * B * h->P, false));
         BODCHK(h->dalloc(&sa.tiles, (size_t)tables * B * h->P, false));
+        BODCHK(h->dalloc(&h->sparse_hdr, (size_t)tables * B));
+        h->sparse_img_tiles = h->P / st_min_pixels(N) + 1;
     }
     h->plan_sparse = sparse;
     h->plan_halo = halo;
@@ -1253,15 +1258,19 @@
     const size_t BK = (size_t)c.batch * c.nms_max_output_size;
     for (int sidx = 0; sidx < 2; ++sidx) {
         BODCHK(h->dalloc(&h->nms_sel_s[sidx], BK));
-        BODCHK(h->dalloc(&h->nms_nsel_s[sidx], (size_t)c.batch));
-        BODCHK(h->dalloc(&h->out_scores_s[sidx], BK * c.num_classes));
-        BODCHK(h->dalloc(&h->out_means_s[sidx], BK * 4));
-        BODCHK(h->dalloc(&h->out_covs_s[sidx], BK * 16));
-        BODCHK(h->dalloc(&h->out_counts_s[sidx], BK * c.num_classes));
-        if (c.covariance_parts & BOD_PARTS_COVARIANCE) BODCHK(h->dalloc(&h->out_parts_s[sidx], BK * 48));
-        if (h->class_parts) BODCHK(h->dalloc(&h->out_cparts_s[sidx], BK * 4));
-        const size_t stage_bytes = ((size_t)c.batch + BK * (2 * (size_t)c.num_classes + 20 + ((c.covariance_parts & BOD_PARTS_COVARIANCE) ? 48 : 0) +
-                                                            (h->class_parts ? 4 : 0))) * 4;
+        const size_t stage_elems = h->stage_num() + BK * (2 * (size_t)c.num_classes + 20 + ((c.covariance_parts & BOD_PARTS_COVARIANCE) ? 48 : 0) +
+                                                          (h->class_parts ? 4 : 0));
+        const size_t stage_bytes = stage_elems * 4;
+        float* rec = nullptr;
+        BODCHK(h->dalloc(&rec, stage_elems));
+        h->records_s[sidx] = rec; h->records_bytes = stage_bytes;
+        h->nms_nsel_s[sidx] = reinterpret_cast<int32_t*>(rec); rec += h->stage_num();
+        h->out_scores_s[sidx] = rec; rec += BK * c.num_classes;
+        h->out_means_s[sidx] = rec; rec += BK * 4;
+        h->out_covs_s[sidx] = rec; rec += BK * 16;
+        h->out_counts_s[sidx] = rec; rec += BK * c.num_classes;
+        if (c.covariance_parts & BOD_PARTS_COVARIANCE) { h->out_parts_s[sidx] = rec; rec += BK * 48; }
+        if (h->class_parts) h->out_cparts_s[sidx] = rec;
         if (hipHostMalloc(reinterpret_cast<void**>(&h->host_stage[sidx]), stage_bytes, hipHostMallocDefault) != hipSuccess)
             return h->fail(BOD_ERR_OOM, "pinned host staging buffer (%zu bytes)", stage_bytes);
     }
@@ -1413,7 +1422,9 @@
                 HIPCHK(h, launch_posterior_keep(pc, pb, st));
                 SparseTailArgs sa = h->sparse;
                 sa.keep = h->pb.keep;
-                HIPCHK(h, launch_sparse_tail_rows(sa, st));
+                const char* split_env = getenv("BOD_SPARSE_ROWS_SPLIT");
+                if (!split_env || atoi(split_env) != 0) HIPCHK(h, launch_sparse_tail_rows_split(sa, h->sparse_hdr, h->sparse_img_tiles, st));
+                else HIPCHK(h, launch_sparse_tail_rows(sa, st));
                 static const bool sparse_stats = [] { const char* e = getenv("BOD_SPARSE_STATS"); return e && atoi(e) != 0; }();
                 if (sparse_stats) {
                     HIPCHK(h, hipStreamSynchronize(st));
@@ -2955,14 +2966,21 @@
     BODCHK(run_cluster(h, sd));
     {
         const size_t B = (size_t)h->cfg.batch, BK = B * h->cfg.nms_max_output_size, C = h->cfg.num_classes;
-        char* hs = h->host_stage[sidx];
-        HIPCHK(h, hipMemcpyAsync(hs, h->nms_nsel_s[sidx], B * 4, hipMemcpyDeviceToHost, sd)); hs += B * 4;
-        HIPCHK(h, hipMemcpyAsync(hs, h->out_scores_s[sidx], BK * C * 4, hipMemcpyDeviceToHost, sd)); hs += BK * C * 4;
-        HIPCHK(h, hipMemcpyAsync(hs, h->out_means_s[sidx], BK * 16, hipMemcpyDeviceToHost, sd)); hs += BK * 16;
-        HIPCHK(h, hipMemcpyAsync(hs, h->out_covs_s[sidx], BK * 64, hipMemcpyDeviceToHost, sd)); hs += BK * 64;
-        HIPCHK(h, hipMemcpyAsync(hs, h->out_counts_s[sidx], BK * C * 4, hipMemcpyDeviceToHost, sd)); hs += BK * C * 4;
-        if (h->parts) { HIPCHK(h, hipMemcpyAsync(hs, h->out_parts_s[sidx], BK * 48 * 4, hipMemcpyDeviceToHost, sd)); h->parts_staged[sidx] = true; hs += BK * 48 * 4; }
-        if (h->cparts) { HIPCHK(h, hipMemcpyAsync(hs, h->out_cparts_s[sidx], BK * 4 * 4, hipMemcpyDeviceToHost, sd)); h->cparts_staged[sidx] = true; }
+        const char* e = getenv("BOD_COLLECT_COPIES");
+        if (!e || atoi(e) != 5) {
+            HIPCHK(h, hipMemcpyAsync(h->host_stage[sidx], h->records_s[sidx], h->records_bytes, hipMemcpyDeviceToHost, sd));
+        } else {
+            char* hs = h->host_stage[sidx];
+            HIPCHK(h, hipMemcpyAsync(hs, h->nms_nsel_s[sidx], B * 4, hipMemcpyDeviceToHost, sd)); hs += h->stage_num() * 4;
+            HIPCHK(h, hipMemcpyAsync(hs, h->out_scores_s[sidx], BK * C * 4, hipMemcpyDeviceToHost, sd)); hs += BK * C * 4;
+            HIPCHK(h, hipMemcpyAsync(hs, h->out_means_s[sidx], BK * 16, hipMemcpyDeviceToHost, sd)); hs += BK * 16;
+            HIPCHK(h, hipMemcpyAsync(hs, h->out_covs_s[sidx], BK * 64, hipMemcpyDeviceToHost, sd)); hs += BK * 64;
+            HIPCHK(h, hipMemcpyAsync(hs, h->out_counts_s[sidx], BK * C * 4, hipMemcpyDeviceToHost, sd)); hs += BK * C * 4;
+            if (h->parts) { HIPCHK(h, hipMemcpyAsync(hs, h->out_parts_s[sidx], BK * 48 * 4, hipMemcpyDeviceToHost, sd)); hs += BK * 48 * 4; }
+            if (h->cparts) HIPCHK(h, hipMemcpyAsync(hs, h->out_cparts_s[sidx], BK * 4 * 4, hipMemcpyDeviceToHost, sd));
+        }
+        if (h->parts) h->parts_staged[sidx] = true;
+        if (h->cparts) h->cparts_staged[sidx] = true;
     }
     HIPCHK(h, hipEventRecord(h->ev_done[sidx], sd));
     h->done_stream[sidx] = sd;
@@ -2979,7 +2997,7 @@
     HIPCHK(h, hipEventSynchronize(h->ev_done[sidx]));
     const char* hs = h->host_stage[sidx];
     if (num) std::memcpy(num, hs, B * 4);
-    hs += B * 4;
+    hs += h->stage_num() * 4;
     if (scores) std::memcpy(scores, hs, BK * C * 4);
     hs += BK * C * 4;
     if (means) std::memcpy(means, hs, BK * 16);
@@ -2996,7 +3014,7 @@
     if (sidx < 0 || sidx > 1 || !h->parts_staged[sidx]) return h->fail(BOD_ERR_NOT_READY, "bod_collect_parts: slot %d holds no batch of bod_infer_async", sidx);
     const size_t B = (size_t)h->cfg.batch, BK = B * h->cfg.nms_max_output_size, C = h->cfg.num_classes;
     HIPCHK(h, hipEventSynchronize(h->ev_done[sidx]));
-    if (parts) std::memcpy(parts, h->host_stage[sidx] + (B + BK * (2 * C + 20)) * 4, BK * 48 * 4);
+    if (parts) std::memcpy(parts, h->host_stage[sidx] + (h->stage_num() + BK * (2 * C + 20)) * 4, BK * 48 * 4);
     return BOD_OK;
 }
 
@@ -3006,7 +3024,7 @@
     const size_t B = (size_t)h->cfg.batch, K = (size_t)h->cfg.nms_max_output_size, BK = B * K, C = h->cfg.num_classes;
     HIPCHK(h, hipEventSynchronize(h->ev_done[sidx]));
     if (!rows) return BOD_OK;
-    std::memcpy(rows, h->host_stage[sidx] + (B + BK * (2 * C + 20 + (h->parts ? 48 : 0))) * 4, BK * 4 * 4);
+    std::memcpy(rows, h->host_stage[sidx] + (h->stage_num() + BK * (2 * C + 20 + (h->parts ? 48 : 0))) * 4, BK * 4 * 4);
     const int32_t* num = reinterpret_cast<const int32_t*>(h->host_stage[sidx]);
     for (size_t b = 0; b < B; ++b)
         for (size_t k = (size_t)std::max(num[b], 0); k < K; ++k)
@@ -3751,6 +3769,27 @@
     return BOD_OK;
 }
 
+bod_status bod_get_sparse_table(bod_handle h, int32_t table, int32_t cap_tiles, int32_t* tiles, int32_t* rows_per_tile,
+                                int32_t* rows, int32_t* ext) {
+    if (!h || !tiles || !rows_per_tile || table < 0 || table > 1 || cap_tiles < 0) return BOD_ERR_INVALID_ARG;
+    BODCHK(join_overlap(h));
+    const SparseTailArgs& sa = h->sparse;
+    if (!h->plan_sparse || (table == 1 && !h->plan_halo)) return h->fail(BOD_ERR_NOT_READY, "bod_get_sparse_table: the plan has no table %d", table);
+    HIPCHK(h, hipSetDevice(h->cfg.device));
+    HIPCHK(h, hipStreamSynchronize(h->stream));
+    int32_t cnt[2] = {0, 0};
+    HIPCHK(h, hipMemcpy(cnt, sa.tile_count, sizeof cnt, hipMemcpyDeviceToHost));
+    const int R = table == 0 ? sa.tail_rows : 256;
+    *tiles = cnt[table]; *rows_per_tile = R;
+    if (!rows && !ext) return BOD_OK;
+    if (cnt[table] < 0 || cnt[table] > cap_tiles || cnt[table] > sa.cap_tiles)
+        return h->fail(BOD_ERR_INVALID_ARG, "bod_get_sparse_table: %d tiles, room for %d", (int)cnt[table], (int)cap_tiles);
+    const size_t n = (size_t)cnt[table];
+    if (rows && n) HIPCHK(h, hipMemcpy(rows, table == 0 ? sa.rows : sa.halo_rows, n * R * sizeof(RowEnt), hipMemcpyDeviceToHost));
+    if (ext && n) HIPCHK(h, hipMemcpy(ext, table == 0 ? sa.ext : sa.halo_ext, n * XR_EXT_ROWS * sizeof(int2), hipMemcpyDeviceToHost));
+    return BOD_OK;
+}
+
 static bod_status stat_handle(bod_handle h, const char* who) {
     if (!h->cfg.mc_statistics) return h->fail(BOD_ERR_INVALID_ARG, "%s: the handle was not created with mc_statistics = 1", who);
     BODCHK(join_overlap(h));
diff --git a/bayes-od-rc_amd/csrc/kernels.h b/bayes-od-rc_amd/csrc/kernels.h
--- a/bayes-od-rc_amd/csrc/kernels.h
+++ b/bayes-od-rc_amd/csrc/kernels.h
@@ -147,6 +147,7 @@
     SparseLevels lv;
 };
 hipError_t launch_sparse_tail_rows(const SparseTailArgs& a, hipStream_t s);
+hipError_t launch_sparse_tail_rows_split(const SparseTailArgs& a, StQuad* hdr, int img_tiles, hipStream_t s);
 hipError_t launch_joint_entropy_rank(const PostCfg& c, const PostBuffers& b, hipStream_t s);
 hipError_t launch_validation_post(const PostCfg& c, const PostBuffers& b, hipStream_t s);
 
diff --git a/bayes-od-rc_amd/csrc/post_kernels.hip b/bayes-od-rc_amd/csrc/post_kernels.hip
--- a/bayes-od-rc_amd/csrc/post_kernels.hip
+++ b/bayes-od-rc_amd/csrc/post_kernels.hip
@@ -2,6 +2,7 @@
 #include "philox.h"
 #include <algorithm>
 #include <math.h>
+#include <stdlib.h>
 
 #define POST_BLOCK 256
 #define MAXC 16
@@ -140,6 +141,102 @@
         float* dc = pb.d_counts + ((size_t)b * c.A + a) * C;
 #pragma unroll
         for (int j = 0; j < C; ++j) dc[j] = (float)cnt[j];
+    }
+    const int n = __syncthreads_count(keep ? 1 : 0);
+    if (threadIdx.x == 0) pb.block_counts[(size_t)b * nblocks + blockIdx.x] = n;
+}
+
+template <int C>
+__device__ __forceinline__ void post_mean_cdf(const PostCfg& c, const PostBuffers& pb, int b, int a, float (&cdf)[C]) {
+    float mp[C];
+#pragma unroll
+    for (int j = 0; j < C; ++j) mp[j] = 0.f;
+    if (c.aggregated) {
+        const float* l = pb.agg_cls + ((size_t)b * c.A + a) * C;
+#pragma unroll
+        for (int j = 0; j < C; ++j) mp[j] = l[j];
+    }
+    for (int n = 0; n < (c.aggregated ? 0 : c.N); ++n) {
+        const float* l = pb.cls + (((size_t)b * c.N + n) * c.A + a) * C;
+        float v[C];
+        if (C % 4 == 0) {
+#pragma unroll
+            for (int q = 0; q < C / 4; ++q) {
+                const float4 t = reinterpret_cast<const float4*>(l)[q];
+                v[4 * q] = t.x; v[4 * q + 1] = t.y; v[4 * q + 2] = t.z; v[4 * q + 3] = t.w;
+            }
+        } else {
+#pragma unroll
+            for (int j = 0; j < C; ++j) v[j] = l[j];
+        }
+        float mx = v[0];
+#pragma unroll
+        for (int j = 1; j < C; ++j) mx = fmaxf(mx, v[j]);
+        float s = 0.f;
+#pragma unroll
+        for (int j = 0; j < C; ++j) { v[j] = expf(v[j] - mx); s += v[j]; }
+#pragma unroll
+        for (int j = 0; j < C; ++j) mp[j] += v[j] / s;
+    }
+    float accum = 0.f;
+#pragma unroll
+    for (int j = 0; j < C; ++j) { mp[j] = mp[j] / (float)c.N; accum += mp[j]; cdf[j] = accum; }
+}
+
+template <int C>
+__device__ __forceinline__ uint64_t post_draw(const float (&cdf)[C], float total, uint32_t w, uint64_t cnt) {
+    static_assert(C == 4 || C == 8, "the search below is written out for 4 and 8 classes");
+    const float t = (float)(w >> 8) * 5.9604644775390625e-8f * total;
+    int sh;
+    if (C == 8) {
+        sh = cdf[3] <= t ? 32 : 0;
+        sh += (sh ? cdf[5] : cdf[1]) <= t ? 16 : 0;
+        const float lo = (sh & 16) ? cdf[2] : cdf[0], hi = (sh & 16) ? cdf[6] : cdf[4];
+        sh += ((sh & 32) ? hi : lo) <= t ? 8 : 0;
+    } else {
+        sh = cdf[1] <= t ? 16 : 0;
+        sh += (sh ? cdf[2] : cdf[0]) <= t ? 8 : 0;
+    }
+    return cnt + (1ull << sh);
+}
+
+template <int C>
+__global__ __launch_bounds__(POST_BLOCK) void post_sample_packed_kernel(PostCfg c, PostBuffers pb, int nblocks) {
+    const int a = blockIdx.x * POST_BLOCK + threadIdx.x;
+    const int b = blockIdx.y;
+    bool keep = false;
+    if (a < c.A) {
+        float cdf[C];
+        post_mean_cdf<C>(c, pb, b, a, cdf);
+        const float total = cdf[C - 1];
+        uint64_t cnt = 0;
+        const int full = c.draws / 4;
+        for (int g = 0; g < full; ++g) {
+            const Philox4 r = philox4x32_10((uint32_t)a, (uint32_t)g, BOD_CAT_TAG, c.image_base + b, c.seed_lo, c.seed_hi);
+            cnt = post_draw<C>(cdf, total, r.x, cnt);
+            cnt = post_draw<C>(cdf, total, r.y, cnt);
+            cnt = post_draw<C>(cdf, total, r.z, cnt);
+            cnt = post_draw<C>(cdf, total, r.w, cnt);
+        }
+        if (c.draws & 3) {
+            const Philox4 r = philox4x32_10((uint32_t)a, (uint32_t)full, BOD_CAT_TAG, c.image_base + b, c.seed_lo, c.seed_hi);
+            cnt = post_draw<C>(cdf, total, r.x, cnt);
+            if ((c.draws & 3) > 1) cnt = post_draw<C>(cdf, total, r.y, cnt);
+            if ((c.draws & 3) > 2) cnt = post_draw<C>(cdf, total, r.z, cnt);
+        }
+        int best = 0, bestc = (int)(cnt & 0xff);
+#pragma unroll
+        for (int j = 1; j < C; ++j) {
+            const int cj = (int)((cnt >> (8 * j)) & 0xff);
+            if (cj > bestc) { bestc = cj; best = j; }
+        }
+        keep = best != C - 1;
+        pb.keep[(size_t)b * c.A + a] = keep ? 1 : 0;
+        if (keep) {
+            float* dc = pb.d_counts + ((size_t)b * c.A + a) * C;
+#pragma unroll
+            for (int j = 0; j < C; ++j) dc[j] = (float)((cnt >> (8 * j)) & 0xff);
+        }
     }
     const int n = __syncthreads_count(keep ? 1 : 0);
     if (threadIdx.x == 0) pb.block_counts[(size_t)b * nblocks + blockIdx.x] = n;
@@ -487,9 +584,16 @@
 hipError_t launch_posterior_keep(const PostCfg& c, const PostBuffers& b, hipStream_t s) {
     const int nblocks = (c.A + POST_BLOCK - 1) / POST_BLOCK;
     dim3 grid(nblocks, c.B);
-    if (c.C == 8) hipLaunchKernelGGL(post_sample_kernel<8>, grid, dim3(POST_BLOCK), 0, s, c, b, nblocks);
-    else if (c.C == 4) hipLaunchKernelGGL(post_sample_kernel<4>, grid, dim3(POST_BLOCK), 0, s, c, b, nblocks);
-    else return hipErrorInvalidValue;
+    const char* e = getenv("BOD_KEEP_PACKED");
+    const bool packed = (!e || atoi(e) != 0) && c.draws <= 255;
+    if (c.C != 8 && c.C != 4) return hipErrorInvalidValue;
+    if (packed) {
+        if (c.C == 8) hipLaunchKernelGGL(post_sample_packed_kernel<8>, grid, dim3(POST_BLOCK), 0, s, c, b, nblocks);
+        else hipLaunchKernelGGL(post_sample_packed_kernel<4>, grid, dim3(POST_BLOCK), 0, s, c, b, nblocks);
+    } else {
+        if (c.C == 8) hipLaunchKernelGGL(post_sample_kernel<8>, grid, dim3(POST_BLOCK), 0, s, c, b, nblocks);
+        else hipLaunchKernelGGL(post_sample_kernel<4>, grid, dim3(POST_BLOCK), 0, s, c, b, nblocks);
+    }
     hipLaunchKernelGGL(post_scan_kernel, dim3(c.B), dim3(POST_BLOCK), 0, s, b, nblocks);
     return hipGetLastError();
 }
@@ -758,7 +862,8 @@
     return hipGetLastError();
 }
 
-__global__ __launch_bounds__(256) void sparse_tail_rows_kernel(SparseTailArgs a) {
+template <bool kSplit>
+__device__ __forceinline__ void sparse_tail_image(const SparseTailArgs& a, StQuad* __restrict__ hdr) {
     extern __shared__ uint8_t s_flag[];
     __shared__ int s_cnt[2][256];
     __shared__ int s_nrun[2], s_nchunk[2], s_ntile[2], s_base[2];
@@ -828,8 +933,10 @@
         if (lane == 0) {
             s_nchunk[t] = st.nchunk; s_ntile[t] = st.ntile;
             s_base[t] = atomicAdd(a.tile_count + t, st.ntile);
-        }
-    }
+            if (kSplit) hdr[(size_t)t * B + b] = StQuad{st.nchunk, st.ntile, s_base[t], 0};
+        }
+    }
+    if (kSplit) return;
     __syncthreads();
     const RowEnt invalid = st_invalid_row(a.pix[0]);
     for (int t = 0; t < T; ++t) {
@@ -857,6 +964,40 @@
     }
 }
 
+__global__ __launch_bounds__(256) void sparse_tail_rows_kernel(SparseTailArgs a) { sparse_tail_image<false>(a, nullptr); }
+__global__ __launch_bounds__(256) void sparse_tail_pack_kernel(SparseTailArgs a, StQuad* __restrict__ hdr) { sparse_tail_image<true>(a, hdr); }
+
+#define ST_WRITE_TILES 16
+__global__ __launch_bounds__(256) void sparse_tail_write_kernel(SparseTailArgs a, const StQuad* __restrict__ hdr) {
+    const int b = blockIdx.y, t = blockIdx.z, N = a.N, P = a.P;
+    const StQuad h = hdr[(size_t)t * a.B + b];
+    const int nchunk = h.x, ntile = h.y, base = h.z;
+    const int groups = (ntile + ST_WRITE_TILES - 1) / ST_WRITE_TILES;
+    if ((int)blockIdx.x >= groups) return;
+    if (base < 0 || base + ntile > a.cap_tiles) return;
+    const int first = blockIdx.x * 256 + threadIdx.x, step = groups * 256;
+    const int R = t == 0 ? a.tail_rows : 256;
+    RowEnt* rows = t == 0 ? a.rows : a.halo_rows;
+    ExtRow* ext = reinterpret_cast<ExtRow*>(t == 0 ? a.ext : a.halo_ext);
+    const StQuad* chunks = a.chunks + ((size_t)t * a.B + b) * P;
+    const StQuad* tiles = a.tiles + ((size_t)t * a.B + b) * P;
+    const RowEnt invalid = st_invalid_row(a.pix[0]);
+    for (int i = first; i < nchunk * N; i += step) {
+        const int ci = i / N, n = i - ci * N;
+        const StQuad c = chunks[ci];
+        st_write_piece(c, n, b, base + c.y, a.pix, N, P, a.Ppad, rows, ext, R);
+    }
+    for (int i = first; i < ntile * R; i += step) {
+        const int tt = i / R, r = i - tt * R;
+        if (st_pad_row(tiles[tt], r, N)) rows[(size_t)(base + tt) * R + r] = invalid;
+    }
+    for (int i = first; i < ntile * XR_EXT_ROWS; i += step) {
+        const int tt = i / XR_EXT_ROWS, r = i - tt * XR_EXT_ROWS;
+        const StQuad ti = tiles[tt];
+        if (r >= ti.z) ext[(size_t)(base + tt) * XR_EXT_ROWS + r] = st_pad_ext(ti, b, a.pix, N, P, a.Ppad);
+    }
+}
+
 hipError_t launch_sparse_tail_rows(const SparseTailArgs& a, hipStream_t s) {
     if (a.B <= 0 || a.P <= 0 || a.N < 1 || 256 / a.N < 1 || XR_EXT_ROWS / a.N - 2 < 1 || a.P > 65536 || a.lv.n < 1 || a.lv.n > 5)
         return hipErrorInvalidValue;
@@ -864,6 +1005,18 @@
     hipError_t e = hipMemsetAsync(a.tile_count, 0, 2 * sizeof(int32_t), s);
     if (e != hipSuccess) return e;
     hipLaunchKernelGGL(sparse_tail_rows_kernel, dim3(a.B), dim3(256), (size_t)a.P, s, a);
+    return hipGetLastError();
+}
+
+hipError_t launch_sparse_tail_rows_split(const SparseTailArgs& a, StQuad* hdr, int img_tiles, hipStream_t s) {
+    if (a.B <= 0 || a.P <= 0 || a.N < 1 || 256 / a.N < 1 || XR_EXT_ROWS / a.N - 2 < 1 || a.P > 65536 || a.lv.n < 1 || a.lv.n > 5)
+        return hipErrorInvalidValue;
+    if ((a.tail_rows != 192 && a.tail_rows != 256) || a.tail_rows / a.N < 1 || !hdr || img_tiles < 1) return hipErrorInvalidValue;
+    hipError_t e = hipMemsetAsync(a.tile_count, 0, 2 * sizeof(int32_t), s);
+    if (e != hipSuccess) return e;
+    hipLaunchKernelGGL(sparse_tail_pack_kernel, dim3(a.B), dim3(256), (size_t)a.P, s, a, hdr);
+    const dim3 grid((img_tiles + ST_WRITE_TILES - 1) / ST_WRITE_TILES, a.B, a.halo_rows ? 2 : 1);
+    hipLaunchKernelGGL(sparse_tail_write_kernel, grid, dim3(256), 0, s, a, hdr);
     return hipGetLastError();
 }
 
@@ -1385,11 +1538,242 @@
     }
 }
 
+#define CLW_AHEAD 4
+template <int C>
+__global__ __launch_bounds__(64) void cluster_fuse_wave_kernel(ClusterArgs a) {
+    static_assert(2 * C <= 64 && CL_BLOCK == 256, "lane layout of the sums and the tail's stores");
+    const int k = blockIdx.x, b = blockIdx.y, lane = threadIdx.x;
+    const int nsel = a.num_selected[b];
+    const int M = a.num_kept[b];
+    const int centre = a.selected[(size_t)b * a.max_out + k];
+    if (k >= nsel) return;
+    const size_t base = (size_t)b * a.A;
+    const float4* boxes = reinterpret_cast<const float4*>(a.corners) + base;
+    const float4 cbox = boxes[centre];
+    float cs[C];
+    {
+        float sum = 0.f;
+#pragma unroll
+        for (int j = 0; j < C; ++j) { cs[j] = a.counts[(base + centre) * C + j]; sum += cs[j]; }
+#pragma unroll
+        for (int j = 0; j < C; ++j) cs[j] = cs[j] / sum;
+        float s2 = 0.f;
+#pragma unroll
+        for (int j = 0; j < C; ++j) s2 += cs[j];
+#pragma unroll
+        for (int j = 0; j < C; ++j) cs[j] = cs[j] / s2;
+    }
+    auto wsum = [](float v) {
+#pragma unroll
+        for (int o = 32; o > 0; o >>= 1) v += __shfl_xor(v, o, 64);
+        return v;
+    };
+    auto uniform = [](float v, int l) { return __int_as_float(__builtin_amdgcn_readlane(__float_as_int(v), l)); };
+    const float* aff = (a.affinity && b == a.affinity_img) ? a.affinity + (size_t)k * a.A : nullptr;
+    float prev = 0.f, s01 = 0.f, s23 = 0.f;
+    float bk[3] = {INFINITY, INFINITY, INFINITY};
+    int bx[3] = {0x7fffffff, 0x7fffffff, 0x7fffffff};
+    int mem0 = 0, mem1 = 0, mem2 = 0, nmem = 0;
+#pragma unroll 1
+    for (int v = 0; v < 4; ++v) {
+        float psum[10], pmsum[4];
+#pragma unroll
+        for (int q = 0; q < 10; ++q) psum[q] = 0.f;
+#pragma unroll
+        for (int q = 0; q < 4; ++q) pmsum[q] = 0.f;
+        float tk[3] = {INFINITY, INFINITY, INFINITY};
+        int ti[3] = {0x7fffffff, 0x7fffffff, 0x7fffffff};
+        int cnt = 0;
+        for (int i0 = v * 64 + lane; i0 < M; i0 += CL_BLOCK * CLW_AHEAD) {
+            float val[CLW_AHEAD];
+            if (aff) {
+#pragma unroll
+                for (int c = 0; c < CLW_AHEAD; ++c) val[c] = aff[min(i0 + c * CL_BLOCK, M - 1)];
+            } else {
+                float4 bb[CLW_AHEAD];
+#pragma unroll
+                for (int c = 0; c < CLW_AHEAD; ++c) bb[c] = boxes[min(i0 + c * CL_BLOCK, M - 1)];
+#pragma unroll
+                for (int c = 0; c < CLW_AHEAD; ++c) val[c] = iou_plus1(bb[c], cbox);
+            }
+            unsigned member = 0;
+#pragma unroll
+            for (int c = 0; c < CLW_AHEAD; ++c) member |= (i0 + c * CL_BLOCK < M && val[c] > a.thr) ? 1u << c : 0u;
+#pragma unroll 1
+            for (int c = 0; c < CLW_AHEAD; ++c) {
+                if (!(member >> c & 1)) continue;
+                const int i = i0 + c * CL_BLOCK;
+                ++cnt;
+                if (nmem == 0) mem0 = i; else if (nmem == 1) mem1 = i; else if (nmem == 2) mem2 = i;
+                ++nmem;
+                Mat4 cv;
+#pragma unroll
+                for (int r = 0; r < 4; ++r)
+#pragma unroll
+                    for (int q = 0; q < 4; ++q) cv.m[r][q] = a.covs[(base + i) * 16 + r * 4 + q];
+                const Mat4 pr = inv_spd4(cv);
+                int t = 0;
+#pragma unroll
+                for (int r = 0; r < 4; ++r)
+#pragma unroll
+                    for (int q = 0; q <= r; ++q) psum[t++] += pr.m[r][q];
+                float mu[4];
+#pragma unroll
+                for (int r = 0; r < 4; ++r) mu[r] = a.means[(base + i) * 4 + r];
+#pragma unroll
+                for (int r = 0; r < 4; ++r) {
+                    float s = 0.f;
+#pragma unroll
+                    for (int q = 0; q < 4; ++q) s += pr.m[r][q] * mu[q];
+                    pmsum[r] += s;
+                }
+                float row[C], rs = 0.f;
+#pragma unroll
+                for (int j = 0; j < C; ++j) { row[j] = a.counts[(base + i) * C + j]; rs += row[j]; }
+                float kl = 0.f, qs = 0.f;
+                float sc[C];
+#pragma unroll
+                for (int j = 0; j < C; ++j) { sc[j] = row[j] / rs; qs += sc[j]; }
+#pragma unroll
+                for (int j = 0; j < C; ++j) {
+                    const float q = sc[j] / qs;
+                    if (cs[j] > 0.f) kl += (q > 0.f) ? cs[j] * logf(cs[j] / q) : INFINITY;
+                }
+                if (kl < tk[2] || (kl == tk[2] && i < ti[2])) {
+                    tk[2] = kl; ti[2] = i;
+                    if (tk[2] < tk[1] || (tk[2] == tk[1] && ti[2] < ti[1])) {
+                        float f = tk[1]; tk[1] = tk[2]; tk[2] = f; int g = ti[1]; ti[1] = ti[2]; ti[2] = g;
+                        if (tk[1] < tk[0] || (tk[1] == tk[0] && ti[1] < ti[0])) {
+                            f = tk[0]; tk[0] = tk[1]; tk[1] = f; g = ti[0]; ti[0] = ti[1]; ti[1] = g;
+                        }
+                    }
+                }
+            }
+        }
+        float cur = 0.f;
+        if (__any(cnt > 0)) {
+            float vals[15];
+#pragma unroll
+            for (int q = 0; q < 10; ++q) vals[q] = psum[q];
+#pragma unroll
+            for (int q = 0; q < 4; ++q) vals[10 + q] = pmsum[q];
+            vals[14] = (float)cnt;
+#pragma unroll
+            for (int q = 0; q < 15; ++q) {
+                const float r = wsum(vals[q]);
+                cur = lane == q ? r : cur;
+            }
+            int p = 0;
+#pragma unroll
+            for (int r = 0; r < 3; ++r) {
+                const float ck = p == 0 ? tk[0] : p == 1 ? tk[1] : p == 2 ? tk[2] : INFINITY;
+                const int ci = p == 0 ? ti[0] : p == 1 ? ti[1] : p == 2 ? ti[2] : 0x7fffffff;
+                float wk = ck; int wi = ci;
+#pragma unroll
+                for (int o = 32; o > 0; o >>= 1) {
+                    const float ok = __shfl_xor(wk, o, 64);
+                    const int oi = __shfl_xor(wi, o, 64);
+                    if (oi != 0x7fffffff && (wi == 0x7fffffff || ok < wk || (ok == wk && oi < wi))) { wk = ok; wi = oi; }
+                }
+                if (wi != 0x7fffffff && ci == wi) ++p;
+                if (wi == 0x7fffffff) continue;
+                if (wk < bk[2] || (wk == bk[2] && wi < bx[2])) {
+                    bk[2] = wk; bx[2] = wi;
+                    if (bk[2] < bk[1] || (bk[2] == bk[1] && bx[2] < bx[1])) {
+                        float f = bk[1]; bk[1] = bk[2]; bk[2] = f; int g = bx[1]; bx[1] = bx[2]; bx[2] = g;
+                        if (bk[1] < bk[0] || (bk[1] == bk[0] && bx[1] < bx[0])) {
+                            f = bk[0]; bk[0] = bk[1]; bk[1] = f; g = bx[0]; bx[0] = bx[1]; bx[1] = g;
+                        }
+                    }
+                }
+            }
+        }
+        if (v == 1) s01 = prev + cur; else if (v == 3) s23 = prev + cur; else prev = cur;
+    }
+    const float comb = s01 + s23;
+    const int total = (int)uniform(comb, 14);
+    float sv = 0.f;
+    if (total <= 3) {
+        float p01 = 0.f;
+#pragma unroll 1
+        for (int v = 0; v < 4; ++v) {
+            float ssum[C], csum[C];
+#pragma unroll
+            for (int j = 0; j < C; ++j) { ssum[j] = 0.f; csum[j] = 0.f; }
+            bool any = false;
+#pragma unroll
+            for (int e = 0; e < 3; ++e) {
+                const int i = e == 0 ? mem0 : e == 1 ? mem1 : mem2;
+                if (e >= nmem || ((i >> 6) & 3) != v) continue;
+                any = true;
+                float row[C], rs = 0.f;
+#pragma unroll
+                for (int j = 0; j < C; ++j) { row[j] = a.counts[(base + i) * C + j]; rs += row[j]; }
+#pragma unroll
+                for (int j = 0; j < C; ++j) { ssum[j] += row[j] / rs; csum[j] += row[j]; }
+            }
+            float cur = 0.f;
+            if (__any(any)) {
+#pragma unroll
+                for (int j = 0; j < C; ++j) {
+                    const float r0 = wsum(ssum[j]), r1 = wsum(csum[j]);
+                    cur = lane == j ? r0 : lane == C + j ? r1 : cur;
+                }
+            }
+            if (v == 1) p01 = sv + cur; else if (v == 3) sv = p01 + (sv + cur); else sv = cur;
+        }
+    } else {
+        float s = 0.f, cc = 0.f;
+#pragma unroll
+        for (int t = 0; t < 3; ++t) {
+            const float* rowp = a.counts + (base + bx[t]) * C;
+            float rs = 0.f;
+#pragma unroll
+            for (int j = 0; j < C; ++j) rs += rowp[j];
+            const float x = rowp[lane & (C - 1)];
+            s += x / rs; cc += x;
+        }
+        sv = lane < C ? s : cc;
+    }
+    const size_t ob = (size_t)b * a.max_out + k;
+    Mat4 ps;
+    {
+        int t = 0;
+#pragma unroll
+        for (int r = 0; r < 4; ++r)
+#pragma unroll
+            for (int q = 0; q <= r; ++q) { ps.m[r][q] = uniform(comb, t); ps.m[q][r] = ps.m[r][q]; ++t; }
+    }
+    const Mat4 fc = inv_spd4(ps);
+    float ov = 0.f;
+#pragma unroll
+    for (int r = 0; r < 4; ++r) {
+        float s = 0.f;
+#pragma unroll
+        for (int q = 0; q < 4; ++q) s += fc.m[r][q] * uniform(comb, 10 + q);
+        ov = lane == 16 + r ? s : ov;
+#pragma unroll
+        for (int q = 0; q < 4; ++q) ov = lane == r * 4 + q ? fc.m[r][q] * 70.0f : ov;
+    }
+    if (lane < 16) a.out_covs[ob * 16 + lane] = ov;
+    else if (lane < 20) a.out_means[ob * 4 + (lane - 16)] = ov;
+    const float denom = (float)(total > 3 ? 3 : total);
+    if (lane < C) a.out_scores[ob * C + lane] = sv / denom;
+    else if (lane < 2 * C) a.out_counts[ob * C + (lane - C)] = sv;
+}
+
 hipError_t launch_cluster_fuse(const ClusterArgs& a, hipStream_t s) {
     dim3 grid(a.max_out, a.B);
-    if (a.C == 8) hipLaunchKernelGGL(cluster_fuse_kernel<8>, grid, dim3(CL_BLOCK), 0, s, a);
-    else if (a.C == 4) hipLaunchKernelGGL(cluster_fuse_kernel<4>, grid, dim3(CL_BLOCK), 0, s, a);
-    else return hipErrorInvalidValue;
+    const char* e = getenv("BOD_CLUSTER_WAVE");
+    const bool wave = !e || atoi(e) != 0;
+    if (a.C != 8 && a.C != 4) return hipErrorInvalidValue;
+    if (wave) {
+        if (a.C == 8) hipLaunchKernelGGL(cluster_fuse_wave_kernel<8>, grid, dim3(64), 0, s, a);
+        else hipLaunchKernelGGL(cluster_fuse_wave_kernel<4>, grid, dim3(64), 0, s, a);
+    } else {
+        if (a.C == 8) hipLaunchKernelGGL(cluster_fuse_kernel<8>, grid, dim3(CL_BLOCK), 0, s, a);
+        else hipLaunchKernelGGL(cluster_fuse_kernel<4>, grid, dim3(CL_BLOCK), 0, s, a);
+    }
     return hipGetLastError();
 }
 
diff --git a/bayes-od-rc_amd/engine.py b/bayes-od-rc_amd/engine.py
--- a/bayes-od-rc_amd/engine.py
+++ b/bayes-od-rc_amd/engine.py
@@ -699,6 +699,14 @@
                 "fan_out_row_reuse": bool(info[3]), "ops": int(info[4]), "plane_row_reuse_layers": int(info[5]), "tower_mx": bool(info[6]), "tower_mx_format": int(info[6]),
                 "sparse_tail": bool(info[7]), "sparse_halo": bool(info[8]), "sparse_tail_rows": int(info[9])}
 
+    def sparse_table(self, table=0):
+        tiles, height = C.c_int32(0), C.c_int32(0)
+        self._chk(self.lib.bod_get_sparse_table(self.h, table, 0, C.byref(tiles), C.byref(height), None, None))
+        rows = np.empty((tiles.value, height.value, 8), np.int32)
+        ext = np.empty((tiles.value, 320, 2), np.int32)
+        self._chk(self.lib.bod_get_sparse_table(self.h, table, tiles.value, C.byref(tiles), C.byref(height), iptr(rows), iptr(ext)))
+        return rows, ext
+
     @property
     def aggregating(self):
         return self.plan_info()["aggregating"]
diff --git a/include/bayesod.h b/include/bayesod.h
--- a/include/bayesod.h
+++ b/include/bayesod.h
@@ -277,6 +277,8 @@
 
 bod_status bod_plan_info(bod_handle h, int32_t* info8);
 bod_status bod_plan_info_n(bod_handle h, int32_t* info, int32_t n);
+bod_status bod_get_sparse_table(bod_handle h, int32_t table, int32_t cap_tiles, int32_t* tiles, int32_t* rows_per_tile,
+                                int32_t* rows, int32_t* ext);
 
 bod_status bod_stat_reset(bod_handle h);
 bod_status bod_stat_forward(bod_handle h, const float* images, int32_t images_on_device, uint64_t seed, uint32_t first_image_id,
diff --git a/include/bayesod_cdef.h b/include/bayesod_cdef.h
--- a/include/bayesod_cdef.h
+++ b/include/bayesod_cdef.h
@@ -235,6 +235,8 @@
 bod_status bod_device_detection_class_parts(bod_handle h, int32_t slot, void** ptr);
 bod_status bod_plan_info(bod_handle h, int32_t* info8);
 bod_status bod_plan_info_n(bod_handle h, int32_t* info, int32_t n);
+bod_status bod_get_sparse_table(bod_handle h, int32_t table, int32_t cap_tiles, int32_t* tiles, int32_t* rows_per_tile,
+                                int32_t* rows, int32_t* ext);
 bod_status bod_stat_reset(bod_handle h);
 bod_status bod_stat_forward(bod_handle h, const float* images, int32_t images_on_device, uint64_t seed, uint32_t first_image_id,
                             int32_t sample_base);
```

Result: no change. 2284 images/sec, median of 6 (+0.5%).
